# iesl/anncur

Hardware: AMD Instinct MI355X
Metric: queries/sec + Top-k-Recall@100 vs exact, CUR-256 on QxI score matrix (higher is better)
Workload: dtype bf16; 1 GPU; cfg2: Q=10000/GPU x I=100000 bf16 score matrix, 256 anchor items, 512 anchor queries, k=100, k_retvr=100; step = gather C_q + fused S_hat/top-k + exact top-k scan + overlap/recall; Q_per_gpu=10000, I=100000, anchors=256, anchor_queries=512, k=100, k_retvr=100

## Files before the change

### anncur_amd/csrc/common.hpp

```cpp
#pragma once
#include <hip/hip_runtime.h>
#include <stdint.h>
#include <stdarg.h>
#include <stdio.h>
#include "anncur_hip.h"

void anncur_set_error(const char *fmt, ...);
constexpr int LADDER_LEVELS = 8;
int anncur_internal_kth_value(const float *G, int64_t Q, int n, int64_t ldg, int k, float *out, int64_t out_stride, hipStream_t st, int coarse = 0,
							  float *ladder = nullptr, int k2 = 1, float *tau2 = nullptr);
int anncur_internal_approx_error_acc(const void *X, int x_dtype, int64_t ldx, const void *Et, int e_dtype, int64_t lde, const void *Aex, int a_dtype,
									 int64_t lda, int64_t Q, int64_t I, int64_t K, float *err_sq, float *norm_sq, void *stream);

int anncur_ensure_dyn_lds(const void *fn, int bytes);
int anncur_num_cu();
int anncur_event_pool(hipEvent_t **out, int n);
int anncur_internal_scan_rows_in_flight(int dtype);

#define ANNCUR_REQUIRE(cond, code, ...)                 \
	do {                                                \
		if (!(cond)) {                                  \
			anncur_set_error(__VA_ARGS__);              \
			return (code);                              \
		}                                               \
	} while (0)

#define ANNCUR_HIP_OK(expr)                                                              \
	do {                                                                                 \
		hipError_t e__ = (expr);                                                         \
		if (e__ != hipSuccess) {                                                         \
			anncur_set_error("%s failed: %s (%s:%d)", #expr, hipGetErrorString(e__), __FILE__, __LINE__); \
			return ANNCUR_E_HIP;                                                         \
		}                                                                                \
	} while (0)

#define ANNCUR_LAUNCH_OK()                                                               \
	do {                                                                                 \
		hipError_t e__ = hipGetLastError();                                              \
		if (e__ != hipSuccess) {                                                         \
			anncur_set_error("kernel launch failed: %s (%s:%d)", hipGetErrorString(e__), __FILE__, __LINE__); \
			return ANNCUR_E_HIP;                                                         \
		}                                                                                \
	} while (0)

static inline bool dtype_ok(int d) { return d == ANNCUR_F32 || d == ANNCUR_BF16; }
static inline size_t dtype_size(int d) { return d == ANNCUR_F32 ? 4 : 2; }
static inline int64_t ceil_div64(int64_t a, int64_t b) { return (a + b - 1) / b; }

#define WAVE 64

__device__ __forceinline__ float bf16_bits_to_f32(uint32_t b) { return __uint_as_float(b << 16); }

__device__ __forceinline__ uint16_t f32_to_bf16_bits(float f) {
	uint32_t u = __float_as_uint(f);
	if ((u & 0x7fffffffu) > 0x7f800000u) return (uint16_t)((u >> 16) | 0x0040u);
	return (uint16_t)((u + 0x7fffu + ((u >> 16) & 1u)) >> 16);
}

__device__ __forceinline__ uint32_t f32_sortable(float f) {
	const uint32_t u = __float_as_uint(f);
	return u ^ ((uint32_t)((int32_t)u >> 31) | 0x80000000u);
}
__device__ __forceinline__ float f32_unsortable(uint32_t s) {
	uint32_t u = (s & 0x80000000u) ? (s & 0x7fffffffu) : ~s;
	return __uint_as_float(u);
}
__device__ __forceinline__ uint64_t make_key(float v, uint32_t idx) {
	return ((uint64_t)f32_sortable(v) << 32) | (uint64_t)(0xffffffffu - idx);
}
__device__ __forceinline__ float key_val(uint64_t k) { return f32_unsortable((uint32_t)(k >> 32)); }
__device__ __forceinline__ uint32_t key_idx(uint64_t k) { return 0xffffffffu - (uint32_t)k; }

__device__ __forceinline__ int lane_id() { return threadIdx.x & (WAVE - 1); }

template <int CTRL, int ROW_MASK = 0xf, int BANK_MASK = 0xf>
__device__ __forceinline__ uint32_t dpp_mov(uint32_t identity, uint32_t x) {
	return (uint32_t)__builtin_amdgcn_update_dpp((int)identity, (int)x, CTRL, ROW_MASK, BANK_MASK, false);
}
struct DppAdd { static constexpr uint32_t ID = 0u; __device__ static uint32_t op(uint32_t a, uint32_t b) { return a + b; } };
struct DppMin { static constexpr uint32_t ID = 0xffffffffu; __device__ static uint32_t op(uint32_t a, uint32_t b) { return a < b ? a : b; } };
struct DppMax { static constexpr uint32_t ID = 0u; __device__ static uint32_t op(uint32_t a, uint32_t b) { return a > b ? a : b; } };
template <typename OP>
__device__ __forceinline__ uint32_t wave_scan_incl(uint32_t x) {
	uint32_t t = x;
	t = OP::op(t, dpp_mov<0x111>(OP::ID, x));
	t = OP::op(t, dpp_mov<0x112>(OP::ID, x));
	t = OP::op(t, dpp_mov<0x113>(OP::ID, x));
	t = OP::op(t, dpp_mov<0x114, 0xf, 0xe>(OP::ID, t));
	t = OP::op(t, dpp_mov<0x118, 0xf, 0xc>(OP::ID, t));
	t = OP::op(t, dpp_mov<0x142, 0xa, 0xf>(OP::ID, t));
	t = OP::op(t, dpp_mov<0x143, 0xc, 0xf>(OP::ID, t));
	return t;
}
template <typename OP>
__device__ __forceinline__ uint32_t wave_reduce(uint32_t x) {
	return (uint32_t)__builtin_amdgcn_readlane((int)wave_scan_incl<OP>(x), WAVE - 1);
}

__device__ __forceinline__ uint32_t lane_xor(uint32_t x, int stride) {
	if (stride == 1) return dpp_mov<0xB1>(x, x);
	if (stride == 2) return dpp_mov<0x4E>(x, x);
	if (stride == 4) return dpp_mov<0x1B>(x, dpp_mov<0x141>(x, x));
	if (stride == 8) return dpp_mov<0x141>(x, dpp_mov<0x140>(x, x));
	return (uint32_t)__shfl_xor((int)x, stride);
}

template <typename T>
__device__ __forceinline__ float load_as_f32(const T *p);
template <>
__device__ __forceinline__ float load_as_f32<float>(const float *p) { return *p; }
template <>
__device__ __forceinline__ float load_as_f32<uint16_t>(const uint16_t *p) { return bf16_bits_to_f32(*p); }
```

### anncur_amd/csrc/prepass16.hpp

```cpp
#pragma once

template <int KP>
struct Prepass16Cfg {
	static constexpr int NBUF = 3;
	static constexpr int KS32 = KP / 32, K = KP / 16, CPR = KP / 8;
	static constexpr int TILE_BYTES = TILE_I * KP * 2;
	static constexpr int PIECES = TILE_BYTES / 1024 / 4;
	static constexpr int LDS_BYTES = NBUF * TILE_BYTES;
	static constexpr int BQ = 256;
	static_assert(PIECES >= 1 && K >= 4, "a tile holds a 1 KB piece per wave and at least four fragments per lane");
	static_assert(2 * LDS_BYTES <= 160 * 1024, "two workgroups per CU");
};

template <int N>
__device__ __forceinline__ void vm_wait_all_but() {
#if defined(__HIP_DEVICE_COMPILE__)
	asm volatile("s_waitcnt vmcnt(%0)" ::"n"(N) : "memory");
#endif
}

template <int KP, int CUR>
__device__ __forceinline__ void prepass16_tile(const uint32_t (&aoff)[Prepass16Cfg<KP>::K], const bf16x8 (&xb)[4][Prepass16Cfg<KP>::KS32], f32x4 (&acc)[2][4]) {
	using C = Prepass16Cfg<KP>;
	constexpr int K = C::K, AR = 5, DIST = 3, OFF = CUR * C::TILE_BYTES;
	u32x4 ring[AR];
#pragma unroll
	for (int i = 0; i < DIST; ++i) lds_read_frag<OFF>(ring[i], aoff[i]);
#pragma unroll
	for (int ih = 0; ih < 2; ++ih)
#pragma unroll
		for (int t = 0; t < 4; ++t) acc[ih][t] = (f32x4){0.f, 0.f, 0.f, 0.f};
#pragma unroll
	for (int g = 0; g < K; ++g) {
		const int nxt = g + DIST;
		if (nxt < K) lds_read_frag<OFF>(ring[nxt % AR], aoff[nxt]);
#if defined(__HIP_DEVICE_COMPILE__)
		if (g >= 1) asm volatile("" ::"v"(ring[(g - 1) % AR]));
#endif
		const int after = K - 1 - g;
		lds_wait_frag(ring[g % AR], after < DIST ? after : DIST);
		const bf16x8 a = __builtin_bit_cast(bf16x8, ring[g % AR]);
		const int ks = g >> 1, ih = g & 1;
#pragma unroll
		for (int t = 0; t < 4; ++t) acc[ih][t] = __builtin_amdgcn_mfma_f32_16x16x32_bf16(a, xb[t][ks], acc[ih][t], 0, 0, 0);
	}
#if defined(__HIP_DEVICE_COMPILE__)
	asm volatile("s_nop 7\n\ts_nop 2" : "+v"(acc[0][0]), "+v"(acc[0][1]), "+v"(acc[0][2]), "+v"(acc[0][3]), "+v"(acc[1][0]), "+v"(acc[1][1]), "+v"(acc[1][2]), "+v"(acc[1][3]));
#endif
}

template <int KP>
__global__ __launch_bounds__(256, 2) void prepass16_kernel(const FusedParams p) {
	using C = Prepass16Cfg<KP>;
	constexpr int K = C::K, KS32 = C::KS32, CPR = C::CPR;
	extern __shared__ __attribute__((aligned(16))) unsigned char smem[];
	const int tid = threadIdx.x, lane = tid & 63, wave = tid >> 6;
	const int c16 = lane & 15, g4 = lane >> 4;
	zero_ws_header(p);
	const int wid = xcd_remap(blockIdx.x, p.n_wg);
	const int n_rb = (int)((p.Q + C::BQ - 1) / C::BQ);
	const int split = wid / n_rb, rb = wid - split * n_rb;
	const int wave_u = __builtin_amdgcn_readfirstlane(wave);
	const uint32_t lds_base = (uint32_t)__builtin_amdgcn_readfirstlane((int)lds_addr(smem));

	const int j_begin = split * p.st_per_split, j_end = min(j_begin + p.st_per_split, p.n_st);
	int f_tile, f_rem = 0, dq = 1, dr = 0;
	if (p.sample_leading) f_tile = j_begin;
	else {
		const int64_t x = (int64_t)j_begin * p.n_full_tiles;
		f_tile = (int)(x / p.n_st); f_rem = (int)(x % p.n_st);
		dq = p.n_full_tiles / p.n_st; dr = p.n_full_tiles % p.n_st;
	}
	int j_dma = j_begin;
	uint32_t dma_off[C::PIECES];
#pragma unroll
	for (int i = 0; i < C::PIECES; ++i) {
		const int pch = (wave_u * C::PIECES + i) * 64 + lane;
		const int row = pch / CPR, cs = pch % CPR;
		dma_off[i] = (uint32_t)(row * CPR + swz<CPR>(row, cs)) * 16u;
	}
	auto fetch = [&](int buf) {
		const unsigned char *src = reinterpret_cast<const unsigned char *>(p.Et) + (int64_t)f_tile * C::TILE_BYTES;
#if defined(__HIP_DEVICE_COMPILE__)
#pragma unroll
		for (int i = 0; i < C::PIECES; ++i) {
			const uint32_t m0v = lds_base + (uint32_t)(buf * C::TILE_BYTES) + (uint32_t)(wave_u * C::PIECES + i) * 1024u;
			asm volatile("s_mov_b32 m0, %0\n\ts_nop 0\n\tglobal_load_lds_dwordx4 %1, %2" ::"s"(m0v), "v"(dma_off[i]), "s"(src) : "memory", "m0");
		}
#endif
		f_tile += dq; f_rem += dr;
		if (f_rem >= p.n_st) { f_rem -= p.n_st; ++f_tile; }
		++j_dma;
	};
	if (j_dma < j_end) fetch(0);

	bf16x8 xb[4][KS32];
	const int64_t q_wave0 = (int64_t)rb * C::BQ + wave_u * 64;
#pragma unroll
	for (int t = 0; t < 4; ++t) {
		const int64_t q = q_wave0 + 16 * t + c16;
		const bool ok = q < p.Q;
		const u32x4 *src = reinterpret_cast<const u32x4 *>(p.X + (ok ? q : 0) * p.ldx) + g4;
#pragma unroll
		for (int s = 0; s < KS32; ++s) {
			const u32x4 zero = {0u, 0u, 0u, 0u};
			const u32x4 w = ok ? src[4 * s] : zero;
			xb[t][s] = __builtin_bit_cast(bf16x8, w);
		}
	}
	__builtin_amdgcn_s_waitcnt(0x0F70);
	if (j_dma < j_end) fetch(1);
	__builtin_amdgcn_s_barrier();

	const int64_t q_st = q_wave0 + 16 * (lane >> 5) + c16;
	const bool st_ok0 = q_st < p.Q, st_ok1 = q_st + 32 < p.Q;
	float *const gdst = p.gmax + (st_ok0 ? q_st : 0) * p.n_groups + (g4 & 1);
	const int64_t gdst_pair = (int64_t)32 * p.n_groups;
	uint32_t aoff[K];
#pragma unroll
	for (int s = 0; s < K; ++s) {
		const int row = 16 * (s & 1) + c16;
		aoff[s] = lds_addr(smem) + (uint32_t)(row * CPR + swz<CPR>(row, 4 * (s >> 1) + g4)) * 16u;
	}
	__builtin_amdgcn_s_waitcnt(0xC07F);

#define PRE16_STEP(CUR)                                                                                                         \
	do {                                                                                                                        \
		const bool ahead = j_dma < j_end;                                                                        \
		if (ahead) fetch(((CUR) + 2) % C::NBUF);    \
		f32x4 acc[2][4];                                                                                                        \
		prepass16_tile<KP, CUR>(aoff, xb, acc);                                                                                 \
		float m[4];                                                                                                             \
		_Pragma("unroll") for (int t = 0; t < 4; ++t) {                                                                         \
			const f32x4 a0 = acc[0][t], a1 = acc[1][t];                                                                         \
			m[t] = fmaxf(fmaxf(fmaxf(a0[0], a0[1]), fmaxf(a0[2], a0[3])), fmaxf(fmaxf(a1[0], a1[1]), fmaxf(a1[2], a1[3])));     \
		}                                                                                                                       \
		const auto s01 = __builtin_amdgcn_permlane32_swap(__float_as_uint(m[0]), __float_as_uint(m[1]), false, false);          \
		const auto s23 = __builtin_amdgcn_permlane32_swap(__float_as_uint(m[2]), __float_as_uint(m[3]), false, false);          \
		const float v01 = fmaxf(__uint_as_float(s01[0]), __uint_as_float(s01[1]));                                              \
		const float v23 = fmaxf(__uint_as_float(s23[0]), __uint_as_float(s23[1]));                                              \
		                         \
		if (ahead) vm_wait_all_but<C::PIECES>(); else vm_wait_all_but<0>();                                                     \
		if (st_ok0) gdst[2 * (int64_t)j] = v01;                                                                                 \
		if (st_ok1) gdst[gdst_pair + 2 * (int64_t)j] = v23;                                                                     \
		__builtin_amdgcn_s_barrier();                                                                                           \
		++j;                                                                                                                    \
	} while (0)
	ANNCUR_PAD_HERE();
	int j = j_begin;
	while (j < j_end) {
		PRE16_STEP(0);
		if (j >= j_end) break;
		PRE16_STEP(1);
		if (j >= j_end) break;
		PRE16_STEP(2);
	}
#undef PRE16_STEP
}
```

### anncur_amd/csrc/score_fused.hip

```cpp
#include <stdlib.h>
#include <math.h>
#include <type_traits>
#ifdef ANNCUR_PLACEMENT_PAD
#define ANNCUR_PAD_HERE() asm volatile(".rept %0\n\ts_nop 0\n\t.endr" ::"n"(ANNCUR_PLACEMENT_PAD) : "memory")
#else
#define ANNCUR_PAD_HERE() do { } while (0)
#endif
#include "select.hpp"
#include "wave_select.hpp"
#include "select_stream.hpp"

using namespace anncur;

namespace {

typedef __attribute__((ext_vector_type(8))) __bf16 bf16x8;
typedef __attribute__((ext_vector_type(16))) float f32x16;
typedef __attribute__((ext_vector_type(4))) unsigned int u32x4;

constexpr int TILE_I = 32;
constexpr int CHUNK_TILES = 4;

template <int KP, int QTV = ((KP <= 256) ? 2 : 1)>
struct FusedCfg {
	static constexpr int KSTEPS = KP / 16;
	static constexpr int QT = QTV;
	static constexpr int BQ = 4 * 32 * QT;
	static constexpr int CPR = KP / 8;
	static constexpr int TILE_BYTES = TILE_I * KP * 2;
	static constexpr int PASSES = TILE_BYTES / (256 * 16);
	static constexpr int QDEPTH = 8;
	static constexpr int QUEUE_BYTES = QT * QDEPTH * 256 * 8;
	static constexpr int QUEUE_OFF = (2 * TILE_BYTES + 16383) / 16384 * 16384;
	static constexpr int TICKET_OFF = QUEUE_OFF + QUEUE_BYTES;
	static constexpr int LDS_BYTES = TICKET_OFF + (KP >= 512 ? 0 : 16);
	static constexpr int NAOFF = KSTEPS < 8 ? KSTEPS : 8;
};

template <int CPR>
__device__ __forceinline__ int swz(int row, int c) {
	if (CPR >= 16) return c ^ (row & 15);
	return c ^ ((row >> 1) & 7);
}

struct FusedParams {
	const uint16_t *X; int64_t ldx;
	const uint16_t *Et;
	int64_t Q, I;
	int n_tiles, n_full_tiles;
	int S, tiles_per_split;
	int tile_begin, tile_end;
	int tile_step;
	int carry;
	int n_st, S0, st_per_split;
	int sample_leading;
	float *gmax; int n_groups;
	const float *tau; int tau_stride;
	uint2 *cand; uint32_t *seg_cnt; int capg;
	int nseg;
	int rb_major;
	int flush_tiles;
	int debug_nostore;
	int debug_stamp;
	float tau_bias;
	int n_wg;
	int chunk_tiles, n_chunks;
	uint32_t *chunk_ctr;
	uint8_t *chunk_owner;
	int sliced, chunks_per_slice;
	int prio_mode;
	int ladder_on; uint32_t ladder_k, ladder_mask;
	const float *ladder; uint32_t *ladder_cnt; float *tau_final;
	uint32_t *nfb;
	int ring_stagger, ring_spin_sleep;
	uint32_t zero_bytes;
};

__device__ __forceinline__ int xcd_remap(int b, int n) {
	const int q = n >> 3, r = n & 7, x = b & 7, l = b >> 3;
	return (x < r ? x * (q + 1) : r * (q + 1) + (x - r) * q) + l;
}

__device__ __forceinline__ void zero_ws_header(const FusedParams &p) {
	typedef __attribute__((ext_vector_type(4))) unsigned int zvec;
	zvec *const dst = reinterpret_cast<zvec *>(p.nfb);
	const uint32_t n = p.zero_bytes >> 4;
	for (uint32_t i = blockIdx.x * blockDim.x + threadIdx.x; i < n; i += gridDim.x * blockDim.x) dst[i] = (zvec){0u, 0u, 0u, 0u};
}


template <int KP>
__device__ __forceinline__ void tile_dma(const uint16_t *__restrict__ Et, int tile, unsigned char *buf, int wave, int lane) {
	constexpr int CPR = FusedCfg<KP>::CPR;
	constexpr int PER_WAVE = FusedCfg<KP>::TILE_BYTES / 1024 / 4;
	const unsigned char *src = reinterpret_cast<const unsigned char *>(Et + (int64_t)tile * TILE_I * KP);
#pragma unroll
	for (int i = 0; i < PER_WAVE; ++i) {
		const int piece = wave * PER_WAVE + i;
		const int pch = piece * 64 + lane;
		const int row = pch / CPR, cs = pch % CPR;
		const int c = swz<CPR>(row, cs);
		__builtin_amdgcn_global_load_lds((const __attribute__((address_space(1))) void *)(src + (row * CPR + c) * 16),
										 (__attribute__((address_space(3))) void *)(buf + piece * 1024), 16, 0, 0);
	}
}

template <int KP>
__device__ __forceinline__ void tile_dma_offsets(uint32_t (&voff)[FusedCfg<KP>::TILE_BYTES / 4096], int wave_u, int lane) {
	constexpr int CPR = FusedCfg<KP>::CPR, PER_WAVE = FusedCfg<KP>::TILE_BYTES / 4096;
#pragma unroll
	for (int i = 0; i < PER_WAVE; ++i) {
		const int pch = (wave_u * PER_WAVE + i) * 64 + lane;
		const int row = pch / CPR, cs = pch % CPR;
		voff[i] = (uint32_t)(row * CPR + swz<CPR>(row, cs)) * 16u;
	}
}
template <int KP>
__device__ __forceinline__ void tile_dma_s(const uint16_t *__restrict__ Et, int tile, uint32_t lds_buf, int wave_u,
											const uint32_t (&voff)[FusedCfg<KP>::TILE_BYTES / 4096]) {
	constexpr int PER_WAVE = FusedCfg<KP>::TILE_BYTES / 4096;
	const unsigned char *src = reinterpret_cast<const unsigned char *>(Et) + (int64_t)tile * FusedCfg<KP>::TILE_BYTES;
#if defined(__HIP_DEVICE_COMPILE__)
#pragma unroll
	for (int i = 0; i < PER_WAVE; ++i) {
		const uint32_t m0v = lds_buf + (uint32_t)(wave_u * PER_WAVE + i) * 1024u;
		asm volatile("s_mov_b32 m0, %0\n\ts_nop 0\n\tglobal_load_lds_dwordx4 %1, %2" ::"s"(m0v), "v"(voff[i]), "s"(src) : "memory", "m0");
	}
#endif
}

__device__ __forceinline__ uint32_t lds_addr(const void *p) {
	return (uint32_t)(size_t)(__attribute__((address_space(3))) const char *)p;
}
__device__ __forceinline__ void lds_write_u64(uint32_t addr, uint32_t lo, uint32_t hi) {
#if defined(__HIP_DEVICE_COMPILE__)
	const unsigned long long d = ((unsigned long long)hi << 32) | lo;
	asm volatile("ds_write_b64 %0, %1" ::"v"(addr), "v"(d) : "memory");
#endif
}
__device__ __forceinline__ uint2 lds_load_u64(uint32_t addr) {
	unsigned long long d = 0;
#if defined(__HIP_DEVICE_COMPILE__)
	asm volatile("ds_read_b64 %0, %1\n\ts_waitcnt lgkmcnt(0)" : "=&v"(d) : "v"(addr) : "memory");
#endif
	return make_uint2((uint32_t)d, (uint32_t)(d >> 32));
}

__device__ __forceinline__ void lds_write_u32(uint32_t addr, uint32_t v) {
#if defined(__HIP_DEVICE_COMPILE__)
	asm volatile("ds_write_b32 %0, %1" ::"v"(addr), "v"(v) : "memory");
#endif
}
__device__ __forceinline__ uint32_t lds_load_u32_uniform(uint32_t addr) {
	uint32_t d = 0;
#if defined(__HIP_DEVICE_COMPILE__)
	asm volatile("ds_read_b32 %0, %1\n\ts_waitcnt lgkmcnt(0)" : "=&v"(d) : "v"(addr) : "memory");
#endif
	return (uint32_t)__builtin_amdgcn_readfirstlane((int)d);
}
__device__ __forceinline__ void ticket_draw(uint32_t &ticket, uint32_t *ctr) {
#if defined(__HIP_DEVICE_COMPILE__)
	const uint32_t one = 1u;
	asm volatile("global_atomic_add %0, %1, %2, off sc0" : "=v"(ticket) : "v"(ctr), "v"(one) : "memory");
#endif
}
__device__ __forceinline__ void ticket_wait(uint32_t &ticket) {
#if defined(__HIP_DEVICE_COMPILE__)
	asm volatile("s_waitcnt vmcnt(0)" : "+v"(ticket)::"memory");
#endif
}
__device__ __forceinline__ void lds_write_2x32(uint32_t addr, uint32_t lo, uint32_t hi) {
#if defined(__HIP_DEVICE_COMPILE__)
	asm volatile("ds_write2_b32 %0, %1, %2 offset1:1" ::"v"(addr), "v"(lo), "v"(hi) : "memory");
#endif
}

template <int D, bool FILTER_PREDICATED = false, bool INLINE_HIT = false>
__device__ __forceinline__ void filter_one(float v, int e, float tau, uint32_t item0, uint32_t lq, uint32_t &qcnt) {
	static_assert((D & (D - 1)) == 0, "queue depth must be a power of two");
	if (FILTER_PREDICATED) {
		if (v >= tau) {
			lds_write_2x32((qcnt & (uint32_t)((D - 1) << 11)) | lq, __float_as_uint(v), item0 + (uint32_t)((e & 3) + 8 * (e >> 2)));
			qcnt += 2048u;
		}
	} else if (INLINE_HIT) {
		if (__builtin_expect(__ballot(v >= tau) != 0ull, 1)) {
			if (v >= tau) {
				lds_write_2x32((qcnt & (uint32_t)((D - 1) << 11)) | lq, __float_as_uint(v), item0 + (uint32_t)((e & 3) + 8 * (e >> 2)));
				qcnt += 2048u;
			}
		}
	} else if (__builtin_expect(__ballot(v >= tau) != 0ull, 0)) {
		if (v >= tau) {
			lds_write_2x32((qcnt & (uint32_t)((D - 1) << 11)) | lq, __float_as_uint(v), item0 + (uint32_t)((e & 3) + 8 * (e >> 2)));
			qcnt += 2048u;
		}
	}
}

template <int D>
__device__ __forceinline__ void filter_queue(const f32x16 &acc, float tau, uint32_t item0, uint32_t lq, uint32_t &qcnt) {
#pragma unroll
	for (int e = 0; e < 16; ++e) filter_one<D>(acc[e], e, tau, item0, lq, qcnt);
}

constexpr uint32_t RING_RAW = 0x80000000u;
template <int D>
__device__ __forceinline__ void mark_wrapped_raw(const f32x16 &acc, uint32_t lq, uint32_t &qcnt) {
	static_assert(D == 8, "the raw tile (16 floats) fills the ring exactly");
	const bool wrapped = (qcnt >> 11) > (uint32_t)D && qcnt < RING_RAW;
	if (__builtin_expect(__ballot(wrapped) != 0ull, 0)) {
		if (wrapped) {
#pragma unroll
			for (int i = 0; i < D; ++i) lds_write_2x32(lq + (uint32_t)i * 2048u, __float_as_uint(acc[2 * i]), __float_as_uint(acc[2 * i + 1]));
			qcnt = RING_RAW;
		}
	}
}

template <int D, bool BATCH = true>
__device__ __forceinline__ void flush_queue(uint32_t lq, uint32_t &qcnt, uint2 *__restrict__ seg, uint32_t &ncand, uint32_t capg,
											 uint32_t n_items, float tau, uint32_t raw_item0) {
	if (__builtin_expect(__ballot(qcnt >= RING_RAW) != 0ull, 0)) {
		if (qcnt >= RING_RAW) {
			for (int i = 0; i < D; ++i) {
				const uint2 w = lds_load_u64(lq + (uint32_t)i * 2048u);
#pragma unroll
				for (int half = 0; half < 2; ++half) {
// ... 629 lines not shown
		adma(j_begin, 0);
	}
	__builtin_amdgcn_s_waitcnt(0x0F70);
	__syncthreads();
	uint32_t aoff[Cfg::NAOFF];
#pragma unroll
	for (int s = 0; s < Cfg::NAOFF; ++s) aoff[s] = lds_addr(smem) + (uint32_t)(r * CPR + swz<CPR>(r, 2 * s + h)) * 16u;
	__builtin_amdgcn_s_waitcnt(0xC07F);
	static_assert(PA <= 15, "vmcnt immediate");
#define ERRL_STEP(ECUR, ACUR, J)                                                                                                \
	do {                                                                                                                        \
		if ((J) + 1 < j_end) tile_dma_s<KP>(p.Et, (J) + 1, lds_base + ((ECUR) ^ 1) * Cfg::TILE_BYTES, wave_u, dma_off);         \
		const bool ahead = (J) + NAB - 1 < j_end;                                                                \
		if (ahead) adma((J) + NAB - 1, ((ACUR) + NAB - 1) % NAB);                                                               \
		f32x16 acc[QT];                                                                                                         \
		error_mfma_tile<KP, ECUR>(aoff, xb, acc);                                                                               \
		ExactQuad<uint16_t> ex[QT][4];                     \
		_Pragma("unroll") for (int t = 0; t < QT; ++t)                                                                          \
			_Pragma("unroll") for (int g = 0; g < 4; ++g)                                                                       \
				asm volatile("ds_read_b64 %0, %1 offset:%2" : "=v"(ex[t][g].w) : "v"(aread[t] + (((uint32_t)g << 4) ^ asw[t])), "n"((ACUR) * ATILE)); \
		asm volatile("s_waitcnt lgkmcnt(0)" ::: "memory");                                                                      \
		_Pragma("unroll") for (int t = 0; t < QT; ++t)                                                                          \
			_Pragma("unroll") for (int g = 0; g < 4; ++g) asm volatile("" : "+v"(ex[t][g].w));                                  \
		_Pragma("unroll") for (int t = 0; t < QT; ++t)                                                                          \
			_Pragma("unroll") for (int e = 0; e < 16; ++e) {                                                                    \
				const float x = ex[t][e >> 2].get(e & 3);                                                                       \
				const float d = acc[t][e] - x;                                                                                  \
				se[t] = fmaf(d, d, se[t]);                                                                                      \
				sn[t] = fmaf(x, x, sn[t]);                                                                                      \
			}                                                                                                                   \
		        \
		if (NAB == 3 && ahead) asm volatile("s_waitcnt vmcnt(%0)" ::"n"(PA) : "memory");                                        \
		else __builtin_amdgcn_s_waitcnt(0x0F70);                                                                                \
		asm volatile("" ::: "memory");                                                                                          \
		__builtin_amdgcn_s_barrier();                                                                                           \
		asm volatile("" ::: "memory");                                                                                          \
	} while (0)
	for (int j = j_begin; j < j_end; j += 2) {
		ERRL_STEP(0, 0, j);
		if (j + 1 < j_end) ERRL_STEP(1, 1, j + 1);
	}
#undef ERRL_STEP
#pragma unroll
	for (int t = 0; t < QT; ++t)
		if (qv[t] < p.Q) {
			atomicAdd(&err_sq[qv[t]], se[t]);
			atomicAdd(&norm_sq[qv[t]], sn[t]);
		}
}

template <int KP, typename TA>
__global__ __launch_bounds__(256, 2) void error_kernel(const FusedParams p, const TA *__restrict__ Aex, int64_t lda,
														float *__restrict__ err_sq, float *__restrict__ norm_sq) {
	using Cfg = FusedCfg<KP>;
	constexpr int KSTEPS = Cfg::KSTEPS, QT = Cfg::QT, CPR = Cfg::CPR;
	extern __shared__ __attribute__((aligned(16))) unsigned char smem[];
	const int tid = threadIdx.x, lane = tid & 63, wave = tid >> 6;
	const int r = lane & 31, h = lane >> 5;
	const int wid = xcd_remap(blockIdx.x, p.n_wg);
	const int n_rb = (int)((p.Q + Cfg::BQ - 1) / Cfg::BQ);
	const int split = wid / n_rb, rb = wid - split * n_rb;

	bf16x8 xb[QT][KSTEPS];
	int64_t qv[QT];
	const TA *rowp[QT];
#pragma unroll
	for (int t = 0; t < QT; ++t) {
		qv[t] = (int64_t)rb * Cfg::BQ + wave * 32 * QT + 32 * t + r;
		const bool ok = qv[t] < p.Q;
		rowp[t] = Aex + (ok ? qv[t] : 0) * lda + 4 * h;
		const u32x4 *src = reinterpret_cast<const u32x4 *>(p.X + (ok ? qv[t] : 0) * p.ldx) + h;
#pragma unroll
		for (int s = 0; s < KSTEPS; ++s) {
			const u32x4 zero = {0u, 0u, 0u, 0u};
			const u32x4 w = ok ? src[2 * s] : zero;
			xb[t][s] = __builtin_bit_cast(bf16x8, w);
		}
	}
	__builtin_amdgcn_s_waitcnt(0x0F70);

	const int j_begin = split * p.tiles_per_split, j_end = min(j_begin + p.tiles_per_split, p.n_tiles);
	float se[QT], sn[QT];
	ExactQuad<TA> ex[QT][4];
#pragma unroll
	for (int t = 0; t < QT; ++t) { se[t] = 0.f; sn[t] = 0.f; }
	if (j_begin < j_end) {
		tile_dma<KP>(p.Et, j_begin, smem, wave, lane);
#pragma unroll
		for (int t = 0; t < QT; ++t)
#pragma unroll
			for (int g = 0; g < 4; ++g) ex[t][g].load(rowp[t] + (int64_t)j_begin * TILE_I + 8 * g);
	}
	__builtin_amdgcn_s_waitcnt(0x0F70);
	__syncthreads();
	uint32_t aoff[Cfg::NAOFF];
#pragma unroll
	for (int s = 0; s < Cfg::NAOFF; ++s) aoff[s] = lds_addr(smem) + (uint32_t)(r * CPR + swz<CPR>(r, 2 * s + h)) * 16u;
	__builtin_amdgcn_s_waitcnt(0xC07F);
#define ERR_STEP(CUR, J)                                                                                                        \
	do {                                                                                                                        \
		const bool more = (J) + 1 < j_end;                                                                                      \
		if (more) tile_dma<KP>(p.Et, (J) + 1, smem + ((CUR) ^ 1) * Cfg::TILE_BYTES, wave, lane);                                \
		f32x16 acc[QT];                                                                                                         \
		error_mfma_tile<KP, CUR>(aoff, xb, acc);                                                                                \
		 \
		                            \
		_Pragma("unroll") for (int t = 0; t < QT; ++t)                                                                          \
			_Pragma("unroll") for (int g = 0; g < 4; ++g) asm volatile("" : "+v"(ex[t][g].w));                                  \
		_Pragma("unroll") for (int t = 0; t < QT; ++t)                                                                          \
			_Pragma("unroll") for (int e = 0; e < 16; ++e) {                                                                    \
				const float x = ex[t][e >> 2].get(e & 3);                                                                       \
				const float d = acc[t][e] - x;                                                                                  \
				se[t] = fmaf(d, d, se[t]);                                                                                      \
				sn[t] = fmaf(x, x, sn[t]);                                                                                      \
			}                                                                                                                   \
		  \
		                      \
		if (more) {                                                                                                             \
			      \
			       \
			if (QT == 2) asm volatile("" : "+v"(se[0]), "+v"(sn[0]), "+v"(se[QT - 1]), "+v"(sn[QT - 1])::"memory");             \
			else asm volatile("" : "+v"(se[0]), "+v"(sn[0])::"memory");                                                         \
			_Pragma("unroll") for (int t = 0; t < QT; ++t)                                                                      \
				_Pragma("unroll") for (int g = 0; g < 4; ++g) ex[t][g].load(rowp[t] + (int64_t)((J) + 1) * TILE_I + 8 * g);     \
			__builtin_amdgcn_s_waitcnt(QT == 2 ? 0x0F78 : 0x0F74);                                     \
		}                                                                                                                       \
		 \
		 \
		asm volatile("" ::: "memory");                                                                                          \
		__builtin_amdgcn_s_barrier();                                                                                           \
		asm volatile("" ::: "memory");                                                                                          \
	} while (0)
	for (int j = j_begin; j < j_end; j += 2) {
		ERR_STEP(0, j);
		if (j + 1 < j_end) ERR_STEP(1, j + 1);
	}
#undef ERR_STEP
#pragma unroll
	for (int t = 0; t < QT; ++t)
		if (qv[t] < p.Q) {
			atomicAdd(&err_sq[qv[t]], se[t]);
			atomicAdd(&norm_sq[qv[t]], sn[t]);
		}
}

#include "score_evalf.hpp"

struct SweepStages {
	int n, begin[3], end[3], tps[3], stride;
	int chunk, bq, n_chunks[3];
	const uint8_t *owner[3];
};

template <int KMAX>
__global__ __launch_bounds__(SEL_THREADS) void select_candidates_kernel(
	const uint2 *__restrict__ cand, const uint32_t *__restrict__ seg_cnt, int nseg, int S, SweepStages stg, int capg,
	const uint16_t *__restrict__ X, int64_t ldx, const uint16_t *__restrict__ Et, int64_t I, int KP, uint32_t k,
	float *__restrict__ out_val, int32_t *__restrict__ out_idx, uint32_t *__restrict__ n_fallback,
	const int32_t *__restrict__ hard_list, const uint32_t *__restrict__ hard_cnt, const float *__restrict__ tau_in, int tau_stride,
	const int32_t *__restrict__ remap) {
	extern __shared__ __attribute__((aligned(16))) unsigned char smem[];
	const SelState s = sel_carve<KMAX>(smem);
	float *xq = reinterpret_cast<float *>(smem + SelCfg<KMAX>::LDS_BYTES);
	uint32_t *bad = reinterpret_cast<uint32_t *>(xq + KP);
	const int tid = threadIdx.x, lane = tid & 63, wave = tid >> 6;
	auto score_of = [&](int64_t i) {
		float v = 0.f;
		const uint4 *er = reinterpret_cast<const uint4 *>(Et + i * KP);
		for (int c = 0; c < KP / 8; ++c) {
			const uint4 w = er[c];
			const uint32_t ww[4] = {w.x, w.y, w.z, w.w};
#pragma unroll
			for (int d = 0; d < 4; ++d) {
				v = fmaf(__uint_as_float(ww[d] << 16), xq[8 * c + 2 * d], v);
				v = fmaf(__uint_as_float(ww[d] & 0xffff0000u), xq[8 * c + 2 * d + 1], v);
			}
		}
		return v;
	};
	const uint32_t n_work = hard_list ? *hard_cnt : gridDim.x;
	for (uint32_t wi = blockIdx.x; wi < n_work; wi += gridDim.x) {
	__syncthreads();
	sel_init(s);
	if (tid < 8) bad[tid] = 0u;
	__syncthreads();
	const int64_t q = hard_list ? (int64_t)hard_list[wi] : (int64_t)wi;
	const uint32_t *cnts = seg_cnt + q * nseg;
	for (int sg = tid; sg < nseg; sg += SEL_THREADS) {
		const uint32_t c = cnts[sg];
		if (c > (uint32_t)capg) { const int sp = sg % S; atomicOr(&bad[sp >> 5], 1u << (sp & 31)); }
	}
	__syncthreads();
	const bool repair = (bad[0] | bad[1] | bad[2] | bad[3] | bad[4] | bad[5] | bad[6] | bad[7]) != 0u;
	for (int sg = tid; sg < nseg; sg += SEL_THREADS) {
		const int sp = sg % S;
		const uint32_t cc = ((bad[sp >> 5] >> (sp & 31)) & 1u) ? 0u : cnts[sg];
		atomicAdd(&s.scal[9], cc);
		atomicMax(&s.scal[10], cc);
	}
	__syncthreads();
	const uint32_t total = s.scal[9], maxc = s.scal[10];
	float tau = tau_in ? tau_in[q * tau_stride] : -INFINITY;
	uint64_t tau_key = 0;
	bool full = !repair && total < k;
	if (!full) {
		for (int sb = 0; sb < nseg; sb += 4) {
			const int sg = sb + wave;
			const int sp = sg % S;
			const bool use = sg < nseg && !((bad[sp >> 5] >> (sp & 31)) & 1u);
			const uint32_t c = use ? cnts[sg] : 0u;
			const uint2 *sp_ptr = cand + (q * nseg + (sg < nseg ? sg : 0)) * (int64_t)capg;
			for (uint32_t e0 = 0; e0 < maxc; e0 += WAVE) {
				const uint32_t e = e0 + lane;
				const bool in = e < c;
				const uint2 ce = in ? sp_ptr[e] : make_uint2(0, 0);
				sel_offer(s, in, __uint_as_float(ce.x), ce.y, tau, tau_key);
				sel_maybe_compact<KMAX>(s, k, tau, tau_key);
			}
		}
	}
	if (repair || full) {
		if (tid == 0) atomicAdd(n_fallback, 1u);
		for (int c = tid; c < KP; c += SEL_THREADS) xq[c] = bf16_bits_to_f32(X[q * ldx + c]);
		__syncthreads();
	}
	if (repair) {
		for (int sp = 0; sp < S; ++sp) {
			if (!((bad[sp >> 5] >> (sp & 31)) & 1u)) continue;
			for (int g = 0; g < stg.n; ++g) {
				if (stg.chunk > 0) {
					const uint8_t *own = stg.owner[g] + (q / stg.bq) * (int64_t)stg.n_chunks[g];
					int it = 0;
					for (int c = 0; c < stg.n_chunks[g]; ++c) {
						if (own[c] != (uint8_t)sp) continue;
						const int64_t i_beg = (int64_t)(stg.begin[g] + c * stg.chunk) * TILE_I;
						const int64_t i_end = (int64_t)min(stg.begin[g] + (c + 1) * stg.chunk, stg.end[g]) * TILE_I;
						for (int64_t i0 = i_beg; i0 < i_end; i0 += SEL_THREADS, ++it) {
							const int64_t i = i0 + tid;
							const bool in = i < i_end && i < I;
							const float v = in ? score_of(i) : 0.f;
							sel_offer(s, in, v, (uint32_t)i, tau, tau_key);
							if ((it & 15) == 15) sel_maybe_compact<KMAX>(s, k, tau, tau_key);
						}
					}
					sel_maybe_compact<KMAX>(s, k, tau, tau_key);
					continue;
				}
				if (stg.stride > 1) {
					int it = 0;
					for (int tb = stg.begin[g] + sp; tb < stg.end[g]; tb += 8 * stg.stride, ++it) {
						const int tile = tb + (tid >> 5) * stg.stride;
						const int64_t i = (int64_t)tile * TILE_I + (tid & 31);
						const bool in = tile < stg.end[g] && i < I;
						const float v = in ? score_of(i) : 0.f;
						sel_offer(s, in, v, (uint32_t)i, tau, tau_key);
						if ((it & 15) == 15) sel_maybe_compact<KMAX>(s, k, tau, tau_key);
					}
					sel_maybe_compact<KMAX>(s, k, tau, tau_key);
					continue;
				}
				const int t0 = stg.begin[g] + sp * stg.tps[g];
				const int t1 = min(t0 + stg.tps[g], stg.end[g]);
				int it = 0;
				for (int64_t i0 = (int64_t)t0 * TILE_I; i0 < (int64_t)t1 * TILE_I; i0 += SEL_THREADS, ++it) {
					const int64_t i = i0 + tid;
					const bool in = i < (int64_t)t1 * TILE_I && i < I;
					const float v = in ? score_of(i) : 0.f;
					sel_offer(s, in, v, (uint32_t)i, tau, tau_key);
					if ((it & 15) == 15) sel_maybe_compact<KMAX>(s, k, tau, tau_key);
				}
				sel_maybe_compact<KMAX>(s, k, tau, tau_key);
			}
		}
		__syncthreads();
		full = s.scal[0] < k && tau_key == 0;
	}
	if (full) {
		__syncthreads();
		if (tid == 0) s.scal[0] = 0;
		__syncthreads();
		tau = -INFINITY; tau_key = 0;
		int it = 0;
		for (int64_t i0 = 0; i0 < I; i0 += SEL_THREADS, ++it) {
			const int64_t i = i0 + tid;
			const bool in = i < I;
			const float v = in ? score_of(i) : 0.f;
			sel_offer(s, in, v, (uint32_t)i, tau, tau_key);
			if ((it & 15) == 15) sel_maybe_compact<KMAX>(s, k, tau, tau_key);
		}
	}
	sel_finish<KMAX>(s, k, out_val + q * (int64_t)k, out_idx + q * (int64_t)k, remap);
	}
}

template <int KMAX>
__global__ __launch_bounds__(SEL_THREADS) void tau_block_kernel(const uint2 *__restrict__ cand, const uint32_t *__restrict__ seg_cnt, int nseg,
																 int capg, uint32_t k, float *__restrict__ tau_out, int tau_stride, int prefilter) {
	extern __shared__ __attribute__((aligned(16))) unsigned char smem[];
	const SelState s = sel_carve<KMAX>(smem);
	const int tid = threadIdx.x, lane = tid & 63, wave = tid >> 6;
	const int64_t q = blockIdx.x;
	sel_init(s);
	const uint32_t *cnts = seg_cnt + q * nseg;
	for (int sg = tid; sg < nseg; sg += SEL_THREADS) {
		const uint32_t c = cnts[sg];
		if (c > (uint32_t)capg) atomicOr(&s.scal[8], 1u);
		atomicAdd(&s.scal[9], c > (uint32_t)capg ? 0u : c);
		atomicMax(&s.scal[10], c > (uint32_t)capg ? 0u : c);
	}
	__syncthreads();
	if (s.scal[8] != 0u || s.scal[9] <= k) return;
	const uint32_t maxc = s.scal[10];
	float tau = prefilter ? tau_out[q * tau_stride] : -INFINITY;
	uint64_t tau_key = 0;
	for (int sb = 0; sb < nseg; sb += 4) {
		const int sg = sb + wave;
		const uint32_t c = sg < nseg ? cnts[sg] : 0u;
		const uint2 *sp = cand + (q * nseg + (sg < nseg ? sg : 0)) * (int64_t)capg;
		for (uint32_t e0 = 0; e0 < maxc; e0 += WAVE) {
			const uint32_t e = e0 + lane;
			const bool in = e < c;
			const uint2 ce = in ? sp[e] : make_uint2(0, 0);
			sel_offer(s, in, __uint_as_float(ce.x), ce.y, tau, tau_key);
			sel_maybe_compact<KMAX>(s, k, tau, tau_key);
		}
	}
	__syncthreads();
	if (s.scal[0] > k) {
		tau_key = sel_compact<KMAX>(s, k);
		tau = key_val(tau_key);
	}
	if (tid == 0 && tau_key != 0 && s.scal[0] >= k) tau_out[q * tau_stride] = fmaxf(tau_out[q * tau_stride], tau);
}

constexpr int WQ_CAP = 1024;
constexpr int WQ_K2 = 1024;
template <int KW> struct WqCfg { static constexpr int CAP = KW <= 128 ? WQ_CAP : 2048, TRIGGER = CAP - WAVE, E = KW / 64; };

template <bool TAU_ONLY, int KW = 128>
__global__ __launch_bounds__(256) void select_wave_kernel(const uint2 *__restrict__ cand, const uint32_t *__restrict__ seg_cnt, int nseg,
														   int capg, int64_t Q, uint32_t k, float *__restrict__ out_val,
														   int32_t *__restrict__ out_idx, uint32_t *__restrict__ hard_cnt,
														   int32_t *__restrict__ hard_list, float *__restrict__ tau, int tau_stride, int prefilter,
														   const int32_t *__restrict__ remap) {
	extern __shared__ __attribute__((aligned(16))) unsigned char smem[];
	const int lane = lane_id(), wave = threadIdx.x >> 6;
	const int64_t q = (int64_t)blockIdx.x * 4 + wave;
	if (q >= Q) return;
	const uint32_t c = (lane < nseg) ? seg_cnt[q * nseg + lane] : 0u;
	const uint32_t inc = wave_scan_incl<DppAdd>(c);
	const uint32_t total = (uint32_t)__builtin_amdgcn_readlane((int)inc, WAVE - 1), pre = inc - c;
	if (__ballot(c > (uint32_t)capg) != 0ull || total < k) {
		if (!TAU_ONLY && lane == 0) hard_list[atomicAdd(hard_cnt, 1u)] = (int32_t)q;
		return;
	}
	constexpr int CAP = WqCfg<KW>::CAP, TRIGGER = WqCfg<KW>::TRIGGER;
	WaveSel w = wsel_init<CAP>(smem + wave * WaveSelLayout<CAP>::BYTES);
	if (tau && prefilter) w.tau = tau[q * tau_stride];
	const uint2 *qc = cand + q * nseg * (int64_t)capg;
	constexpr int LOAD_U = 8;
	for (uint32_t j0 = 0; j0 < total; j0 += LOAD_U * WAVE) {
		int sg[LOAD_U];
#pragma unroll
		for (int u = 0; u < LOAD_U; ++u) sg[u] = 0;
#pragma unroll
		for (int step = 32; step >= 1; step >>= 1) {
			if (step < nseg) {
				uint32_t pv[LOAD_U];
#pragma unroll
				for (int u = 0; u < LOAD_U; ++u) pv[u] = __shfl(pre, (sg[u] + step) & 63);
#pragma unroll
				for (int u = 0; u < LOAD_U; ++u)
					if (sg[u] + step < nseg && pv[u] <= j0 + (uint32_t)(u * WAVE + lane)) sg[u] += step;
			}
		}
		uint32_t ps[LOAD_U];
#pragma unroll
		for (int u = 0; u < LOAD_U; ++u) ps[u] = __shfl(pre, sg[u]);
		uint2 e[LOAD_U];
#pragma unroll
		for (int u = 0; u < LOAD_U; ++u) {
			const uint32_t j = j0 + (uint32_t)(u * WAVE + lane);
			e[u] = qc[j < total ? (int64_t)sg[u] * capg + (j - ps[u]) : 0];
		}
#pragma unroll
		for (int u = 0; u < LOAD_U; ++u) {
			if (j0 + (uint32_t)(u * WAVE) < total) {
				wsel_offer(w, j0 + (uint32_t)(u * WAVE + lane) < total, __uint_as_float(e[u].x), e[u].y);
				if (w.cnt > (uint32_t)TRIGGER) wsel_compact<4, false, true>(w, k);
			}
		}
	}
	if (TAU_ONLY) {
		if (w.cnt > k) wsel_compact<4, false, true>(w, k);
		if (lane == 0 && w.cnt >= k) tau[q * tau_stride] = fmaxf(tau[q * tau_stride], w.tau);
		return;
	}
	wsel_finish<0, 4, WqCfg<KW>::E, true>(w, k, out_val + q * (int64_t)k, out_idx + q * (int64_t)k, remap);
}

}
namespace {
#include "score_wide.hpp"
}
namespace {

struct FusedPlan {
	bool ok;
	int QT, BQ, n_rb, n_tiles, n_full, S, tiles_per_split, group, n_st, S0, st_per_split, n_groups, capg, kmax, flush_tiles;
	int n_stages, stage_end[3], stage_tps[3], stage_flush[3], stage_pred[3];
	int leading;
	int lg;
	bool body16;
	bool bodyef;
	bool bodyq16;
	int chunk;
	bool ladder;
	int ladder_k2;
	size_t off_lcnt, off_lvl, off_tau2;
	size_t off_gmax, off_tval, off_tidx, off_segcnt, off_cand, off_tau, off_hard, off_ctr, off_owner, total;
};

int num_cu() { return anncur_num_cu(); }

size_t align256(size_t x) { return (x + 255) & ~(size_t)255; }
int next_pow2(int x) { int p = 1; while (p < x) p <<= 1; return p; }

void plan_stages(FusedPlan &P, int64_t Q, int k, double exp_hits, bool staged, double fmin, int unit_items) {
	double frac[3] = {1.0, 1.0, 1.0};
	P.n_stages = 1;
	if (staged) {
		const double H0 = exp_hits, c_hit = 2.4e-11 * (double)Q;
		const double c_stage = k <= WSEL_K ? 25e-6 + 3e-9 * (double)Q : (k <= WQ_K2 ? 25e-6 + 1.2e-8 * (double)Q : 25e-6 + 1.4e-11 * (double)Q * 0.3 * H0);
		auto later = [&](double f) { const double h = 1.2 * k / f; return h < H0 ? h : H0; };
		double best = H0 * c_hit;
		static const double grid[] = {0.02, 0.03, 0.04, 0.06, 0.08, 0.10, 0.12, 0.15, 0.18, 0.22, 0.26, 0.30, 0.35, 0.40, 0.50};
		const int ng = (int)(sizeof(grid) / sizeof(grid[0]));
		for (int i = 0; i < ng; ++i) {
			const double f1 = grid[i];
			if (f1 < fmin) continue;
			const double c2 = (f1 * H0 + (1 - f1) * later(f1)) * c_hit + c_stage;
			if (c2 < best) { best = c2; P.n_stages = 2; frac[0] = f1; frac[1] = 1.0; }
			for (int j = i + 1; j < ng; ++j) {
				const double f2 = grid[j];
				if (f2 - f1 < fmin) continue;
				const double c3 = (f1 * H0 + (f2 - f1) * later(f1) + (1 - f2) * later(f2)) * c_hit + 2 * c_stage;
				if (c3 < best) { best = c3; P.n_stages = 3; frac[0] = f1; frac[1] = f2; }
			}
		}
	}
	if (P.n_stages == 2) {
		const double shrink = P.body16 ? 0.63 : (k <= WSEL_K ? 1.0 : 0.6);
		const double f1 = frac[0] * shrink;
		frac[0] = f1 > fmin ? f1 : (fmin < frac[0] ? fmin : frac[0]);
	}
	double rate = exp_hits / ((double)P.n_tiles * 2.0);
	int prev = 0;
	for (int i = 0; i < P.n_stages; ++i) {
		int end = (int)(frac[i] * P.n_tiles + 0.5);
		if (i == P.n_stages - 1 || end > P.n_tiles) end = P.n_tiles;
		if (end <= prev) end = prev + 1 < P.n_tiles ? prev + 1 : P.n_tiles;
		P.stage_end[i] = end;
		P.stage_tps[i] = (end - prev + P.S - 1) / P.S;
		int ft = (int)(0.35 / (rate > 1e-9 ? rate : 1e-9));
		P.stage_flush[i] = ft < 1 ? 1 : (ft > 8 ? 8 : ft);
		P.stage_pred[i] = (1.0 - exp(-4.0 * rate)) > 0.25 ? 1 : 0;
		rate = (double)k / ((double)end * unit_items) * 16.0 * 1.2;
		prev = end;
	}
}

FusedPlan plan_fused(int64_t Q, int64_t I, int KP, int k, bool leading = false, bool mfma16 = false, bool qt1 = false, bool mfma32 = false, bool evalf = false,
					 bool no_ladder = false) {
	FusedPlan P{};
	P.ok = false;
	P.leading = leading ? 1 : 0;
	if (!(KP == 64 || KP == 128 || KP == 256 || KP == 512)) return P;
	if (k < 1 || k > ANNCUR_MAX_TOPK || Q < 1 || I < 1 || I >= (int64_t)0x7fffffff - 64 || k > I) return P;
	if (evalf && !(KP <= 256 && I < (int64_t)(1 << 26))) return P;
	if (evalf) { qt1 = false; mfma16 = false; mfma32 = false; leading = false; P.leading = 0; }
	P.bodyef = evalf;
	P.QT = (KP <= 256 && !(qt1 && KP >= 128)) ? 2 : 1;
	P.BQ = 128 * P.QT;
	P.n_rb = (int)ceil_div64(Q, P.BQ);
	P.n_tiles = (int)ceil_div64(I, TILE_I);
	P.n_full = (int)(I / TILE_I);
	int target = (4 * k > 512) ? 4 * k : 512;
	int n_st16 = (target + 1) / 2;
	if ((int64_t)n_st16 * 8 <= P.n_full) { P.group = 16; P.n_st = n_st16; }
	else { P.group = 4; P.n_st = (target + 7) / 8; }
	if ((int64_t)P.n_st * 4 > P.n_full) return P;
	P.n_groups = P.n_st * (P.group == 16 ? 2 : 8);
	if (P.n_groups < k) return P;
	int slots = ((P.QT == 1 && KP <= 256) ? 3 : 2) * num_cu();
	P.bodyq16 = KP == 512 && !mfma32 && I < (int64_t)(1 << 26);
	const bool ticketed = (P.QT == 2 || P.bodyq16) && !evalf;
	P.chunk = ticketed ? CHUNK_TILES : 0;
	const bool can16 = KP <= 256 && P.QT == 2 && I < (int64_t)(1 << 26);
	constexpr int BODY16_MAX_K = 384, BODY16_MAX_K_LADDER = 1024;
	int S = P.chunk > 0 ? (slots + P.n_rb - 1) / P.n_rb : slots / P.n_rb;
	if (P.chunk > 0 && k <= WQ_K2 && S > WAVE / 2) S = WAVE / 2;
	if (S < 1) S = 1;
	if (S > 255) S = P.chunk > 0 ? 255 : (S > 256 ? 256 : S);
	if (S > P.n_tiles) S = P.n_tiles;
	P.tiles_per_split = (P.n_tiles + S - 1) / S;
	P.S = (P.n_tiles + P.tiles_per_split - 1) / P.tiles_per_split;
	constexpr int64_t LADDER_WAVE_SLACK = (int64_t)(LADDER_PERIOD + 2) * TILE_I + Fused16Cfg<256>::DRAIN_AT;
	const bool ladder_fits = I < 65536 || (int64_t)k + (int64_t)P.S * LADDER_WAVE_SLACK <= 32768;
	const bool ladder_possible = !no_ladder && ticketed && P.n_groups <= 4096 && ladder_fits;
	P.body16 = can16 && !mfma32 && !evalf && (mfma16 || k <= (ladder_possible ? BODY16_MAX_K_LADDER : BODY16_MAX_K));
	int S0 = slots / P.n_rb;
	if (S0 < 1) S0 = 1;
	if (S0 > P.n_st) S0 = P.n_st;
	P.st_per_split = (P.n_st + S0 - 1) / S0;
	P.S0 = (P.n_st + P.st_per_split - 1) / P.st_per_split;
	P.lg = (P.body16 || P.bodyq16 || P.bodyef) ? 1 : 2;
	const double exp_hits_cap = 1.3 * k * ((double)P.n_tiles / P.n_st);
	const double exp_hits = (leading ? 0.65 : 1.0) * exp_hits_cap;
	const double per_seg = exp_hits_cap / ((double)P.lg * P.S);
	int capg = next_pow2((int)(4.0 * per_seg) + 32);
	if (capg < 64) capg = 64;
	if (capg > 16384) capg = 16384;
	P.capg = capg;
	const double per_lane_tile = exp_hits / ((double)P.n_tiles * 2.0);
	int ft = (int)(0.35 / (per_lane_tile > 1e-9 ? per_lane_tile : 1e-9));
	P.flush_tiles = ft < 1 ? 1 : (ft > 8 ? 8 : ft);
	P.ladder = P.body16 && ladder_possible;
	{
		double r = (double)k * ((double)P.n_st * TILE_I / (double)I) * (leading ? 2.0 : 1.25);
		int k2 = (int)(r + 0.5);
		if (k2 > k / 2) k2 = k / 2;
		if (k2 < 3) k2 = 3;
		if (k2 > k) k2 = k;
		P.ladder_k2 = k2;
	}
	plan_stages(P, Q, k, exp_hits, !P.ladder && (k <= WQ_K2 ? P.lg * P.S <= WAVE : true) && P.n_tiles >= 24 * P.S, 4.0 * P.S / P.n_tiles, TILE_I);
	P.kmax = k <= 128 ? 128 : (k <= 512 ? 512 : 2048);
	size_t off = 256;
	P.off_ctr = off;    off = align256(off + (size_t)P.n_rb * 3 * 4 * N_SLICES);
	P.off_lcnt = off;   off = align256(off + (P.ladder ? (size_t)P.n_rb * P.BQ * 16 : 0));
	P.off_gmax = off;   off = align256(off + (size_t)Q * P.n_groups * 4);
	P.off_tval = off;   off = align256(off + (size_t)Q * k * 4);
	P.off_tidx = off;   off = align256(off + (size_t)Q * k * 4);
	P.off_segcnt = off; off = align256(off + (size_t)Q * P.lg * P.S * 4);
	P.off_tau = off;    off = align256(off + (size_t)Q * 4);
	P.off_hard = off;   off = align256(off + (size_t)Q * 4);
	P.off_owner = off;  off = align256(off + (size_t)3 * P.n_rb * (size_t)(P.n_tiles / (P.chunk > 0 ? P.chunk : P.n_tiles) + 2));
	P.off_lvl = off;    off = align256(off + (P.ladder ? (size_t)P.n_rb * P.BQ * 4 * LADDER_LEVELS : 0));
	P.off_tau2 = off;   off = align256(off + (P.ladder ? (size_t)Q * 4 : 0));
	P.off_cand = off;   off = align256(off + (size_t)Q * P.lg * P.S * (size_t)P.capg * 8);
	P.total = off;
	P.ok = true;
	return P;
}

#define EV(i) do { if (ev) ANNCUR_HIP_OK(hipEventRecord(ev[i], st)); } while (0)

constexpr bool STREAM_SELECT_SMALL = false;

int launch_tau_refine(const uint2 *cand, const uint32_t *seg_cnt, int nseg, int capg, int64_t Q, int k, int kmax, float *tau, int tau_stride,
					  int prefilter, hipStream_t st) {
	int rc;
	if (k <= WQ_K2 && nseg <= WAVE) {
#define LAUNCH_WTAU(KW)                                                                                                           \
		do {                                                                                                                      \
			constexpr int lds = 4 * WaveSelLayout<WqCfg<KW>::CAP>::BYTES;                                                         \
			if ((rc = anncur_ensure_dyn_lds((const void *)select_wave_kernel<true, KW>, lds)) != ANNCUR_OK) return rc;            \
			hipLaunchKernelGGL((select_wave_kernel<true, KW>), dim3((unsigned)ceil_div64(Q, 4)), dim3(256), lds, st, cand, seg_cnt, nseg, capg, Q, \
							   (uint32_t)k, (float *)nullptr, (int32_t *)nullptr, (uint32_t *)nullptr, (int32_t *)nullptr, tau, tau_stride, prefilter, (const int32_t *)nullptr); \
		} while (0)
		if (k <= WSEL_K) LAUNCH_WTAU(128);
		else {
			constexpr int lds = 4 * StreamSelLayout::BYTES;
			hipLaunchKernelGGL((select_stream_kernel<true, 2>), dim3((unsigned)ceil_div64(Q, 4)), dim3(256), lds, st, cand, seg_cnt, nseg, capg, Q,
							   (uint32_t)k, (float *)nullptr, (int32_t *)nullptr, (uint32_t *)nullptr, (int32_t *)nullptr, tau, tau_stride, prefilter, (const int32_t *)nullptr);
		}
#undef LAUNCH_WTAU
	} else {
#define LAUNCH_TAU(KM)                                                                                                        \
		do {                                                                                                                  \
			if ((rc = anncur_ensure_dyn_lds((const void *)tau_block_kernel<KM>, (int)SelCfg<KM>::LDS_BYTES)) != ANNCUR_OK) return rc; \
			hipLaunchKernelGGL((tau_block_kernel<KM>), dim3((unsigned)Q), dim3(SEL_THREADS), SelCfg<KM>::LDS_BYTES, st, cand, seg_cnt, \
							   nseg, capg, (uint32_t)k, tau, tau_stride, prefilter);                                           \
		} while (0)
		if (kmax == 128) LAUNCH_TAU(128); else if (kmax == 512) LAUNCH_TAU(512); else LAUNCH_TAU(2048);
#undef LAUNCH_TAU
	}
	ANNCUR_LAUNCH_OK();
	return ANNCUR_OK;
}

int launch_select(const FusedPlan &P, int nseg, const SweepStages &stages, const uint2 *cand, const uint32_t *seg_cnt, const uint16_t *X, int64_t ldx,
				  const uint16_t *Et, int64_t Q, int64_t I, int KP, int k, float *out_val, int32_t *out_idx, unsigned char *ws, const float *tau,
				  int tau_stride, hipStream_t st, const int32_t *remap = nullptr) {
	int rc;
#define LAUNCH_SELECT(KM)                                                                                              \
	do {                                                                                                               \
		const size_t lds = SelCfg<KM>::LDS_BYTES + (size_t)KP * 4 + 32;                                                \
		if ((rc = anncur_ensure_dyn_lds((const void *)select_candidates_kernel<KM>, (int)lds)) != ANNCUR_OK) return rc; \
		hipLaunchKernelGGL((select_candidates_kernel<KM>), dim3(sel_grid), dim3(SEL_THREADS), lds, st, cand, seg_cnt, nseg, \
						   P.S, stages, P.capg, X, ldx, Et, I, KP, (uint32_t)k, out_val, out_idx, (uint32_t *)ws, hard_list, hard_cnt,      \
						   (P.n_stages > 1 || P.ladder) ? tau : (const float *)nullptr, tau_stride, remap);                              \
	} while (0)
	const int32_t *hard_list = nullptr;
	const uint32_t *hard_cnt = nullptr;
	unsigned sel_grid = (unsigned)Q;
	if (k <= WQ_K2 && nseg <= WAVE) {
		int32_t *hl = (int32_t *)(ws + P.off_hard);
		uint32_t *hc = (uint32_t *)(ws + 4);
#define LAUNCH_WSEL(KW)                                                                                                           \
		do {                                                                                                                      \
			constexpr int lds = 4 * WaveSelLayout<WqCfg<KW>::CAP>::BYTES;                                                         \
			if ((rc = anncur_ensure_dyn_lds((const void *)select_wave_kernel<false, KW>, lds)) != ANNCUR_OK) return rc;           \
			hipLaunchKernelGGL((select_wave_kernel<false, KW>), dim3((unsigned)ceil_div64(Q, 4)), dim3(256), lds, st, cand, seg_cnt, nseg, P.capg, Q, \
							   (uint32_t)k, out_val, out_idx, hc, hl, const_cast<float *>(tau), tau_stride, (P.n_stages > 1 || P.ladder) ? 1 : 0, remap); \
		} while (0)
#define LAUNCH_SSEL(EE)                                                                                                           \
		do {                                                                                                                      \
			constexpr int lds = 4 * StreamSelLayout::BYTES;                                                                       \
			hipLaunchKernelGGL((select_stream_kernel<false, EE>), dim3((unsigned)ceil_div64(Q, 4)), dim3(256), lds, st, cand, seg_cnt, nseg, P.capg, Q, \
							   (uint32_t)k, out_val, out_idx, hc, hl, const_cast<float *>(tau), tau_stride, (P.n_stages > 1 || P.ladder) ? 1 : 0, remap); \
		} while (0)
		if (k <= WSEL_K) { if (STREAM_SELECT_SMALL) LAUNCH_SSEL(2); else LAUNCH_WSEL(128); }
		else if (k <= 256) LAUNCH_SSEL(4);
		else if (k <= 512) LAUNCH_SSEL(8);
		else LAUNCH_SSEL(16);
#undef LAUNCH_SSEL
#undef LAUNCH_WSEL
		ANNCUR_LAUNCH_OK();
		hard_list = hl; hard_cnt = hc;
		sel_grid = (unsigned)(Q < 1024 ? Q : 1024);
	}
	if (P.kmax == 128) LAUNCH_SELECT(128); else if (P.kmax == 512) LAUNCH_SELECT(512); else LAUNCH_SELECT(2048);
#undef LAUNCH_SELECT
	ANNCUR_LAUNCH_OK();
	return ANNCUR_OK;
}

int launch_threshold(const FusedPlan &P, const float *gmax, int64_t Q, int k, unsigned char *ws, const float *&tau, int &tau_stride, hipStream_t st) {
	if (P.n_groups <= 4096) {
		float *t = (float *)(ws + P.off_tau);
		const int rc = P.ladder ? anncur_internal_kth_value(gmax, Q, P.n_groups, P.n_groups, k, t, 1, st, 1, (float *)(ws + P.off_lvl), P.ladder_k2, (float *)(ws + P.off_tau2))
								: anncur_internal_kth_value(gmax, Q, P.n_groups, P.n_groups, k, t, 1, st, 1);
		tau = t; tau_stride = 1;
		return rc;
	}
	float *tval = (float *)(ws + P.off_tval);
	tau = tval + (k - 1); tau_stride = k;
	return anncur_rowwise_topk(gmax, ANNCUR_F32, Q, P.n_groups, P.n_groups, k, tval, (int32_t *)(ws + P.off_tidx), st);
}


struct CoScan {
	hipStream_t aux;
	hipEvent_t *ev;
	const void *A; int a_dtype; int64_t lda, Q, I; int32_t k;
	float *val; int32_t *idx;
	int slots, next;
	int64_t row_end[8];
};

int co_plan(CoScan &co, int slots) {
	if (slots > 8) slots = 8;
	if (slots < 1) slots = 1;
	const int64_t round = anncur_internal_scan_rows_in_flight(co.a_dtype);
	const int64_t rounds = co.Q / round;
	int64_t per = rounds / slots;
	if (per < 1) {
		per = 1;
		slots = rounds >= 1 ? (int)rounds : 1;
	}
	int64_t r = 0;
	for (int i = 0; i < slots; ++i) { r = (i == slots - 1) ? co.Q : r + per * round; co.row_end[i] = r < co.Q ? r : co.Q; }
	co.slots = slots;
	co.next = 0;
	return anncur_event_pool(&co.ev, 2 * slots);
}
int co_fork(CoScan *co, hipStream_t st) {
	if (!co || co->next >= co->slots) return ANNCUR_OK;
	const int i = co->next++;
	const int64_t r0 = i ? co->row_end[i - 1] : 0, r1 = co->row_end[i];
	if (r1 <= r0) return ANNCUR_OK;
	ANNCUR_HIP_OK(hipEventRecord(co->ev[2 * i], st));
	ANNCUR_HIP_OK(hipStreamWaitEvent(co->aux, co->ev[2 * i], 0));
	const char *a = (const char *)co->A + (size_t)r0 * (size_t)co->lda * dtype_size(co->a_dtype);
	const int rc = anncur_rowwise_topk(a, co->a_dtype, r1 - r0, co->I, co->lda, co->k, co->val + r0 * co->k, co->idx + r0 * co->k, co->aux);
	if (rc != ANNCUR_OK) return rc;
	ANNCUR_HIP_OK(hipEventRecord(co->ev[2 * i + 1], co->aux));
	return ANNCUR_OK;
}
int co_join(CoScan *co, hipStream_t st) {
	if (!co || co->next < 1) return ANNCUR_OK;
	const int i = co->next - 1;
	if (co->row_end[i] > (i ? co->row_end[i - 1] : 0)) ANNCUR_HIP_OK(hipStreamWaitEvent(st, co->ev[2 * i + 1], 0));
	return ANNCUR_OK;
}
int co_finish(CoScan *co, hipStream_t st) {
	if (!co) return ANNCUR_OK;
	int rc;
	while (co->next < co->slots) {
		if ((rc = co_fork(co, st)) != ANNCUR_OK) return rc;
		if ((rc = co_join(co, st)) != ANNCUR_OK) return rc;
	}
	return co_join(co, st);
}

void co_abort(CoScan *co, hipStream_t st) {
	if (!co) return;
	for (int i = 0; i < co->next; ++i)
		if (co->row_end[i] > (i ? co->row_end[i - 1] : 0)) (void)hipStreamWaitEvent(st, co->ev[2 * i + 1], 0);
}

bool exact_tile_offsets_fit(int64_t lda, int bq) { return lda >= 0 && (uint64_t)(bq - 1) * (uint64_t)lda * 2u + 64u < ((uint64_t)1 << 32); }

struct EvalArgs { const uint16_t *A; int64_t lda; float *err_sq, *norm_sq; const uint16_t *Et_hint; };

template <int KP, int QTV = FusedCfg<KP>::QT>
int launch_fused(const FusedPlan &P, const void *X, int64_t ldx, const void *Et, int64_t Q, int64_t I, int k, float *out_val,
				 int32_t *out_idx, unsigned char *ws, hipStream_t st, hipEvent_t *ev, CoScan *co = nullptr, const int32_t *item_ids = nullptr,
				 const EvalArgs *ea = nullptr) {
	using Cfg = FusedCfg<KP, QTV>;
	FusedParams p{};
	p.X = (const uint16_t *)X; p.ldx = ldx; p.Et = (const uint16_t *)Et; p.Q = Q; p.I = I;
	p.n_tiles = P.n_tiles; p.n_full_tiles = P.n_full; p.S = P.S; p.tiles_per_split = P.tiles_per_split;
	p.tile_begin = 0; p.tile_end = P.n_tiles; p.carry = 0; p.tile_step = 1;
	p.n_st = P.n_st; p.S0 = P.S0; p.st_per_split = P.st_per_split; p.sample_leading = P.leading;
	p.gmax = (float *)(ws + P.off_gmax); p.n_groups = P.n_groups;
	p.cand = (uint2 *)(ws + P.off_cand); p.seg_cnt = (uint32_t *)(ws + P.off_segcnt); p.capg = P.capg; p.flush_tiles = P.flush_tiles;
	p.tau_bias = 0.f;
	p.chunk_tiles = 0; p.n_chunks = 0; p.chunk_ctr = nullptr; p.chunk_owner = nullptr;
	p.nfb = (uint32_t *)ws;
	p.ring_stagger = 0; p.ring_spin_sleep = 1;
	p.nseg = P.lg * P.S;
	p.prio_mode = 0;
	p.ladder_on = P.ladder ? 1 : 0; p.ladder_k = (uint32_t)k; p.ladder_mask = (uint32_t)(LADDER_PERIOD - 1);
	p.ladder = (const float *)(ws + P.off_lvl); p.ladder_cnt = (uint32_t *)(ws + P.off_lcnt); p.tau_final = (float *)(ws + P.off_tau2);

	const int chunk = (P.chunk > 0 && (Cfg::QT == 2 || P.bodyq16)) ? P.chunk : 0;
	const int owner_stride = P.n_rb * (P.n_tiles / (chunk > 0 ? chunk : P.n_tiles) + 2);
	int rc;
	EV(0);
	p.n_wg = P.n_rb * P.S0;
	{
		FusedParams pp = p;
		pp.zero_bytes = (uint32_t)((chunk > 0 || P.ladder) ? P.off_gmax : 256);
		if (ea && ea->Et_hint) { pp.Et = ea->Et_hint; pp.sample_leading = 1; }
		bool pre16 = false;
		if constexpr (KP <= 256 && QTV == 2) {
			if (P.body16 && P.group == 16) {
				if ((rc = anncur_ensure_dyn_lds((const void *)prepass16_kernel<KP>, Prepass16Cfg<KP>::LDS_BYTES)) != ANNCUR_OK) return rc;
				hipLaunchKernelGGL((prepass16_kernel<KP>), dim3(p.n_wg), dim3(256), Prepass16Cfg<KP>::LDS_BYTES, st, pp);
				pre16 = true;
			}
		}
		if (!pre16 && P.group == 16)
			hipLaunchKernelGGL((score_kernel<KP, 0, 16, false, false, QTV>), dim3(p.n_wg), dim3(256), 2 * Cfg::TILE_BYTES, st, pp);
		else if (!pre16)
			hipLaunchKernelGGL((score_kernel<KP, 0, 4, false, false, QTV>), dim3(p.n_wg), dim3(256), 2 * Cfg::TILE_BYTES, st, pp);
	}
	ANNCUR_LAUNCH_OK();
	EV(1);
	if ((rc = co_fork(co, st)) != ANNCUR_OK) return rc;
	rc = launch_threshold(P, p.gmax, Q, k, ws, p.tau, p.tau_stride, st);
	if (rc != ANNCUR_OK) return rc;
	if ((rc = co_join(co, st)) != ANNCUR_OK) return rc;
	EV(2);
	const int tile_step = (!P.body16 && !P.bodyq16 && !P.bodyef && P.S > 1 && chunk == 0) ? P.S : 1;
	p.n_wg = P.n_rb * P.S;
	if ((rc = anncur_ensure_dyn_lds((const void *)score_kernel<KP, 1, 16, false, false, QTV>, Cfg::LDS_BYTES)) != ANNCUR_OK) return rc;
	for (int stg = 0, prev = 0; stg < P.n_stages; prev = P.stage_end[stg], ++stg) {
		EV(5 + 2 * stg);
		p.tile_begin = prev; p.tile_end = P.stage_end[stg]; p.tiles_per_split = P.stage_tps[stg];
		p.flush_tiles = P.stage_flush[stg]; p.carry = stg > 0;
		p.tile_step = tile_step;
		if (chunk > 0) {
			p.rb_major = 0;
			p.chunk_tiles = chunk; p.n_chunks = (p.tile_end - p.tile_begin + chunk - 1) / chunk;
			p.sliced = P.bodyq16 ? 1 : 0;
			p.chunks_per_slice = (p.n_chunks + N_SLICES - 1) / N_SLICES;
			p.chunk_ctr = (uint32_t *)(ws + P.off_ctr) + (size_t)stg * P.n_rb * N_SLICES;
			p.chunk_owner = (uint8_t *)(ws + P.off_owner) + (size_t)stg * owner_stride;
		}
		bool launched = false;
		if constexpr (KP <= 256 && QTV == 2) {
			if (!launched && P.bodyef) {
				if (!ea) { anncur_set_error("launch_fused: evalf plan without the exact matrix"); return ANNCUR_E_INVALID; }
				if ((rc = anncur_ensure_dyn_lds((const void *)evalf_kernel<KP>, EvalFCfg<KP>::LDS_BYTES)) != ANNCUR_OK) return rc;
				hipLaunchKernelGGL((evalf_kernel<KP>), dim3(p.n_wg), dim3(256), EvalFCfg<KP>::LDS_BYTES, st, p, ea->A, ea->lda, ea->err_sq, ea->norm_sq);
				launched = true;
			}
		}
		if constexpr (KP == 512) {
			if (!launched && P.bodyq16) {
				if ((rc = anncur_ensure_dyn_lds((const void *)scoreq16_kernel<KP>, FusedQ16Cfg<KP>::LDS_BYTES)) != ANNCUR_OK) return rc;
				hipLaunchKernelGGL((scoreq16_kernel<KP>), dim3(p.n_wg), dim3(256), FusedQ16Cfg<KP>::LDS_BYTES, st, p);
				launched = true;
			}
		}
		if constexpr (KP <= 256 && QTV == 2) {
			if (!launched && P.body16) {
				if ((rc = anncur_ensure_dyn_lds((const void *)score16_kernel<KP>, Fused16Cfg<KP>::LDS_BYTES)) != ANNCUR_OK) return rc;
				hipLaunchKernelGGL((score16_kernel<KP>), dim3(p.n_wg), dim3(256), Fused16Cfg<KP>::LDS_BYTES, st, p);
				launched = true;
			}
		}
		if constexpr (Cfg::QT == 2) {
			if (!launched && P.stage_pred[stg]) {
				if ((rc = anncur_ensure_dyn_lds((const void *)score_kernel<KP, 1, 16, true, false, QTV>, Cfg::LDS_BYTES)) != ANNCUR_OK) return rc;
				hipLaunchKernelGGL((score_kernel<KP, 1, 16, true, false, QTV>), dim3(p.n_wg), dim3(256), Cfg::LDS_BYTES, st, p);
				launched = true;
			}
		}
		if (!launched) hipLaunchKernelGGL((score_kernel<KP, 1, 16, false, false, QTV>), dim3(p.n_wg), dim3(256), Cfg::LDS_BYTES, st, p);
		ANNCUR_LAUNCH_OK();
		EV(6 + 2 * stg);
		if (stg + 1 < P.n_stages) {
			if ((rc = co_fork(co, st)) != ANNCUR_OK) return rc;
			if ((rc = launch_tau_refine(p.cand, p.seg_cnt, P.lg * P.S, P.capg, Q, k, P.kmax, const_cast<float *>(p.tau), p.tau_stride, stg > 0 ? 1 : 0, st)) != ANNCUR_OK)
				return rc;
			if ((rc = co_join(co, st)) != ANNCUR_OK) return rc;
		}
	}
	EV(3);
	if ((rc = co_fork(co, st)) != ANNCUR_OK) return rc;
	SweepStages stages{};
	stages.n = P.n_stages;
	stages.stride = tile_step;
	stages.chunk = chunk; stages.bq = P.BQ;
	for (int g = 0, prev = 0; g < P.n_stages; prev = P.stage_end[g], ++g) {
		stages.begin[g] = prev; stages.end[g] = P.stage_end[g]; stages.tps[g] = P.stage_tps[g];
		stages.n_chunks[g] = chunk > 0 ? (P.stage_end[g] - prev + chunk - 1) / chunk : 0;
		stages.owner[g] = (const uint8_t *)(ws + P.off_owner) + (size_t)g * owner_stride;
	}
	if ((rc = launch_select(P, P.lg * P.S, stages, p.cand, p.seg_cnt, p.X, ldx, p.Et, Q, I, KP, k, out_val, out_idx, ws, P.ladder ? p.tau_final : p.tau,
							P.ladder ? 1 : p.tau_stride, st, item_ids)) != ANNCUR_OK) return rc;
	EV(4);
	return ANNCUR_OK;
}

constexpr int WIDE_KP_MAX = 4096;
bool wide_kp(int KP) { return KP > 512 && KP <= WIDE_KP_MAX && (KP % 128) == 0; }

FusedPlan plan_wide(int64_t Q, int64_t I, int KP, int k, bool leading = false) {
	FusedPlan P{};
	P.ok = false;
	P.leading = leading ? 1 : 0;
	if (!wide_kp(KP)) return P;
	if (k < 1 || k > ANNCUR_MAX_TOPK || Q < 1 || I < 1 || I >= (int64_t)0x7fffffff - 512 || k > I) return P;
	P.QT = 2;
	P.BQ = WBN;
	P.n_rb = (int)ceil_div64(Q, WBN);
	P.n_tiles = (int)ceil_div64(I, WBM);
	P.n_full = (int)(I / WBM);
	const int target = (4 * k > 512) ? 4 * k : 512;
	const int n16 = (target + 15) / 16;
	if ((int64_t)n16 * 8 <= P.n_full) { P.group = 16; P.n_st = n16; }
	else { P.group = 4; P.n_st = (target + 63) / 64; }
	if ((int64_t)P.n_st * 2 > P.n_full) return P;
	P.n_groups = P.n_st * (P.group == 16 ? 16 : 64);
	if (P.n_groups < k) return P;
	const int slots = num_cu();
	int S = slots / P.n_rb;
	if (S < 1) S = 1;
	if (S > 64) S = 64;
	if (k <= WQ_K2 && S > 16) S = 16;
	if (S > P.n_tiles) S = P.n_tiles;
	P.tiles_per_split = (P.n_tiles + S - 1) / S;
	P.S = (P.n_tiles + P.tiles_per_split - 1) / P.tiles_per_split;
	int S0 = slots / P.n_rb;
	if (S0 < 1) S0 = 1;
	if (S0 > P.n_st) S0 = P.n_st;
	P.st_per_split = (P.n_st + S0 - 1) / S0;
	P.S0 = (P.n_st + P.st_per_split - 1) / P.st_per_split;
	const double exp_hits_cap = 1.3 * k * ((double)P.n_tiles / P.n_st);
	const double exp_hits = (leading ? 0.65 : 1.0) * exp_hits_cap;
	const double per_seg = exp_hits_cap / (4.0 * P.S);
	int capg = next_pow2((int)(4.0 * per_seg) + 32);
	if (capg < 64) capg = 64;
	if (capg > 16384) capg = 16384;
	while (capg > 64 && (int64_t)capg * 4 * P.S >= (1 << 21)) capg >>= 1;
	P.capg = capg;
	P.flush_tiles = 1;
	plan_stages(P, Q, k, exp_hits, (k <= WQ_K2 ? 4 * P.S <= WAVE : true) && P.n_tiles >= 4 * P.S, 1.0 * P.S / P.n_tiles, WBM);
	P.kmax = k <= 128 ? 128 : (k <= 512 ? 512 : 2048);
	size_t off = 256;
	P.off_gmax = off;   off = align256(off + (size_t)Q * P.n_groups * 4);
	P.off_tval = off;   off = align256(off + (size_t)Q * k * 4);
	P.off_tidx = off;   off = align256(off + (size_t)Q * k * 4);
	P.off_segcnt = off; off = align256(off + (size_t)Q * 4 * P.S * 4);
	P.off_tau = off;    off = align256(off + (size_t)Q * 4);
	P.off_hard = off;   off = align256(off + (size_t)Q * 4);
	P.off_cand = off;   off = align256(off + (size_t)Q * 4 * P.S * (size_t)P.capg * 8);
	P.total = off;
	P.ok = true;
	return P;
}

int launch_wide(const FusedPlan &P, const void *X, int64_t ldx, const void *Et, int64_t Q, int64_t I, int KP, int k, float *out_val,
				int32_t *out_idx, unsigned char *ws, hipStream_t st, hipEvent_t *ev, CoScan *co = nullptr, const int32_t *item_ids = nullptr) {
	WideParams p{};
	p.X = (const uint16_t *)X; p.ldx = ldx; p.Et = (const uint16_t *)Et; p.et_rows = ceil_div64(I, TILE_I) * TILE_I; p.Q = Q; p.I = I; p.Kp = KP;
	p.n_rb = P.n_rb; p.S = P.S;
	p.n_st = P.n_st; p.S0 = P.S0; p.st_per_split = P.st_per_split; p.sample_leading = P.leading; p.n_bt_full = P.n_full;
	p.gmax = (float *)(ws + P.off_gmax); p.n_groups = P.n_groups;
	p.cand = (uint2 *)(ws + P.off_cand); p.seg_cnt = (uint32_t *)(ws + P.off_segcnt); p.capg = P.capg;
	p.tau_bias = 0.f;
	int rc;
	ANNCUR_HIP_OK(hipMemsetAsync(ws, 0, 256, st));
	EV(0);
	p.n_wg = P.n_rb * P.S0;
	if (P.group == 16) {
		if ((rc = anncur_ensure_dyn_lds((const void *)wide_kernel<0, 16>, W_LDS_TOTAL)) != ANNCUR_OK) return rc;
		hipLaunchKernelGGL((wide_kernel<0, 16>), dim3(p.n_wg), dim3(512), W_LDS_TOTAL, st, p);
	} else {
		if ((rc = anncur_ensure_dyn_lds((const void *)wide_kernel<0, 4>, W_LDS_TOTAL)) != ANNCUR_OK) return rc;
		hipLaunchKernelGGL((wide_kernel<0, 4>), dim3(p.n_wg), dim3(512), W_LDS_TOTAL, st, p);
	}
	ANNCUR_LAUNCH_OK();
	EV(1);
	if ((rc = co_fork(co, st)) != ANNCUR_OK) return rc;
	if ((rc = launch_threshold(P, p.gmax, Q, k, ws, p.tau, p.tau_stride, st)) != ANNCUR_OK) return rc;
	if ((rc = co_join(co, st)) != ANNCUR_OK) return rc;
	EV(2);
	p.n_wg = P.n_rb * P.S;
	if ((rc = anncur_ensure_dyn_lds((const void *)wide_kernel<1, 16>, W_LDS_TOTAL)) != ANNCUR_OK) return rc;
	for (int stg = 0, prev = 0; stg < P.n_stages; prev = P.stage_end[stg], ++stg) {
		EV(5 + 2 * stg);
		p.bt_begin = prev; p.bt_end = P.stage_end[stg]; p.bt_per_split = P.stage_tps[stg]; p.carry = stg > 0;
		hipLaunchKernelGGL((wide_kernel<1, 16>), dim3(p.n_wg), dim3(512), W_LDS_TOTAL, st, p);
		ANNCUR_LAUNCH_OK();
		EV(6 + 2 * stg);
		if (stg + 1 < P.n_stages) {
			if ((rc = co_fork(co, st)) != ANNCUR_OK) return rc;
			if ((rc = launch_tau_refine(p.cand, p.seg_cnt, 4 * P.S, P.capg, Q, k, P.kmax, const_cast<float *>(p.tau), p.tau_stride, stg > 0 ? 1 : 0, st)) != ANNCUR_OK)
				return rc;
			if ((rc = co_join(co, st)) != ANNCUR_OK) return rc;
		}
	}
	EV(3);
	if ((rc = co_fork(co, st)) != ANNCUR_OK) return rc;
	SweepStages stages{};
	stages.n = P.n_stages;
	const int n_tiles32 = (int)ceil_div64(I, TILE_I), u = WBM / TILE_I;
	for (int g = 0, prev = 0; g < P.n_stages; prev = P.stage_end[g], ++g) {
		stages.begin[g] = prev * u;
		stages.end[g] = P.stage_end[g] * u < n_tiles32 ? P.stage_end[g] * u : n_tiles32;
		stages.tps[g] = P.stage_tps[g] * u;
	}
	if ((rc = launch_select(P, 4 * P.S, stages, p.cand, p.seg_cnt, p.X, ldx, p.Et, Q, I, KP, k, out_val, out_idx, ws, p.tau, p.tau_stride, st, item_ids)) != ANNCUR_OK) return rc;
	EV(4);
	return ANNCUR_OK;
}
#undef EV

FusedPlan plan_any(int64_t Q, int64_t I, int KP, int k, int flags = 0) {
	const bool leading = (flags & ANNCUR_TOPK_LEADING_SAMPLE) != 0, mfma16 = (flags & ANNCUR_TOPK_MFMA16) != 0, qt1 = (flags & ANNCUR_TOPK_QT1) != 0;
	return wide_kp(KP) ? plan_wide(Q, I, KP, k, leading) : plan_fused(Q, I, KP, k, leading, mfma16 && !qt1, qt1, (flags & ANNCUR_TOPK_MFMA32) != 0, false,
																	  (flags & ANNCUR_TOPK_STAGED) != 0);
}
bool ring_flag_ok(int flags) {
	return (flags & ANNCUR_TOPK_RING) == 0;
}
constexpr int TOPK_FLAGS = ANNCUR_TOPK_LEADING_SAMPLE | ANNCUR_TOPK_MFMA16 | ANNCUR_TOPK_QT1 | ANNCUR_TOPK_MFMA32 | ANNCUR_TOPK_RING | ANNCUR_TOPK_STAGED;

}

extern "C" size_t anncur_score_topk_workspace_bytes(int64_t Q, int64_t I, int32_t Kp, int32_t k) {
	const FusedPlan P = plan_any(Q, I, Kp, k);
	if (!P.ok) return 0;
	size_t t = P.total;
	for (int flags : {ANNCUR_TOPK_MFMA16, ANNCUR_TOPK_MFMA32, ANNCUR_TOPK_QT1, ANNCUR_TOPK_RING, ANNCUR_TOPK_STAGED}) {
		const FusedPlan V = plan_any(Q, I, Kp, k, flags);
		if (V.ok && V.total > t) t = V.total;
	}
	return t;
}

extern "C" int anncur_score_topk_supported(int64_t Q, int64_t I, int32_t Kp, int32_t k) {
	return plan_any(Q, I, Kp, k).ok ? 1 : 0;
}

static int score_topk_impl(const void *X, int64_t ldx, const void *Et, int64_t lde, int64_t Q, int64_t I, int32_t Kp,
						   int32_t k, float *out_val, int32_t *out_idx, void *workspace, size_t workspace_bytes,
						   void *stream, hipEvent_t *ev, int32_t flags = 0, const int32_t *item_ids = nullptr, CoScan *co = nullptr, const EvalArgs *ea = nullptr) {
	ANNCUR_REQUIRE((flags & ~TOPK_FLAGS) == 0, ANNCUR_E_INVALID, "score_topk: unknown flags 0x%x", flags);
	ANNCUR_REQUIRE(ring_flag_ok(flags), ANNCUR_E_UNSUPPORTED, "score_topk: ANNCUR_TOPK_RING (the tile-ring sweep body) is retired: measured slower than the default body");
	const FusedPlan P = ea ? plan_fused(Q, I, Kp, k, false, false, false, false, true) : plan_any(Q, I, Kp, k, flags);
	ANNCUR_REQUIRE(P.ok, ANNCUR_E_UNSUPPORTED,
				   "score_topk: (Q=%lld, I=%lld, Kp=%d, k=%d) is outside the fused path (Kp in {64,128,256,512} or a multiple of 128 up to %d, "
				   "1<=k<=%d, I large enough for a sampled threshold); use anncur_gemm + anncur_rowwise_topk",
				   (long long)Q, (long long)I, Kp, k, WIDE_KP_MAX, ANNCUR_MAX_TOPK);
	ANNCUR_REQUIRE(X && Et && out_val && out_idx, ANNCUR_E_INVALID, "score_topk: null pointer");
	ANNCUR_REQUIRE(lde == Kp, ANNCUR_E_INVALID, "score_topk: Et must be packed (lde == Kp), got lde=%lld", (long long)lde);
	ANNCUR_REQUIRE(ldx >= Kp && (ldx % 8) == 0, ANNCUR_E_INVALID, "score_topk: ldx must be >= Kp and a multiple of 8");
	ANNCUR_REQUIRE(((uintptr_t)X % 16) == 0 && ((uintptr_t)Et % 16) == 0, ANNCUR_E_INVALID, "score_topk: X and Et must be 16-byte aligned");
	ANNCUR_REQUIRE(workspace && workspace_bytes >= P.total && ((uintptr_t)workspace % 256) == 0, ANNCUR_E_WORKSPACE,
				   "score_topk: workspace of %zu bytes (256-byte aligned) required, got %zu", P.total, workspace_bytes);
	hipStream_t st = (hipStream_t)stream;
	unsigned char *ws = (unsigned char *)workspace;
	int rc;
	if (co && (rc = co_plan(*co, P.n_stages + 1)) != ANNCUR_OK) return rc;
	switch (Kp) {
		case 64: rc = launch_fused<64>(P, X, ldx, Et, Q, I, k, out_val, out_idx, ws, st, ev, co, item_ids, ea); break;
		case 128: rc = P.QT == 1 ? launch_fused<128, 1>(P, X, ldx, Et, Q, I, k, out_val, out_idx, ws, st, ev, co, item_ids)
								  : launch_fused<128>(P, X, ldx, Et, Q, I, k, out_val, out_idx, ws, st, ev, co, item_ids, ea); break;
		case 256: rc = P.QT == 1 ? launch_fused<256, 1>(P, X, ldx, Et, Q, I, k, out_val, out_idx, ws, st, ev, co, item_ids)
								  : launch_fused<256>(P, X, ldx, Et, Q, I, k, out_val, out_idx, ws, st, ev, co, item_ids, ea); break;
		case 512: rc = launch_fused<512>(P, X, ldx, Et, Q, I, k, out_val, out_idx, ws, st, ev, co, item_ids); break;
		default: rc = launch_wide(P, X, ldx, Et, Q, I, Kp, k, out_val, out_idx, ws, st, ev, co, item_ids); break;
	}
	if (rc == ANNCUR_OK) rc = co_finish(co, st);
	if (rc != ANNCUR_OK) co_abort(co, st);
	return rc;
}

extern "C" int anncur_score_topk_ex(const void *X, int64_t ldx, const void *Et, int64_t lde, int64_t Q, int64_t I, int32_t Kp,
									int32_t k, float *out_val, int32_t *out_idx, void *workspace, size_t workspace_bytes,
									int32_t flags, const int32_t *item_ids, void *stream) {
	return score_topk_impl(X, ldx, Et, lde, Q, I, Kp, k, out_val, out_idx, workspace, workspace_bytes, stream, nullptr, flags, item_ids);
}

extern "C" int anncur_score_topk(const void *X, int64_t ldx, const void *Et, int64_t lde, int64_t Q, int64_t I, int32_t Kp,
								 int32_t k, float *out_val, int32_t *out_idx, void *workspace, size_t workspace_bytes,
								 void *stream) {
	return score_topk_impl(X, ldx, Et, lde, Q, I, Kp, k, out_val, out_idx, workspace, workspace_bytes, stream, nullptr);
}

extern "C" int anncur_eval_topk(const void *A, int a_dtype, int64_t lda, int32_t k_exact, float *exact_val, int32_t *exact_idx,
								const void *X, int64_t ldx, const void *Et, int64_t lde, int64_t Q, int64_t I, int32_t Kp, int32_t k_retvr,
								float *approx_val, int32_t *approx_idx, void *workspace, size_t workspace_bytes, int32_t flags,
								const int32_t *item_ids, void *stream, void *aux_stream) {
	ANNCUR_REQUIRE(dtype_ok(a_dtype) && A && exact_val && exact_idx && lda >= I && k_exact >= 1 && k_exact <= I && k_exact <= ANNCUR_MAX_TOPK,
				   ANNCUR_E_INVALID, "eval_topk: bad exact-scan arguments");
	if (Q == 0) return ANNCUR_OK;
	if (!aux_stream || aux_stream == stream) {
		const int rc = anncur_rowwise_topk(A, a_dtype, Q, I, lda, k_exact, exact_val, exact_idx, stream);
		if (rc != ANNCUR_OK) return rc;
		return score_topk_impl(X, ldx, Et, lde, Q, I, Kp, k_retvr, approx_val, approx_idx, workspace, workspace_bytes, stream, nullptr, flags, item_ids);
	}
	CoScan co{};
	co.aux = (hipStream_t)aux_stream;
	co.A = A; co.a_dtype = a_dtype; co.lda = lda; co.Q = Q; co.I = I; co.k = k_exact; co.val = exact_val; co.idx = exact_idx;
	return score_topk_impl(X, ldx, Et, lde, Q, I, Kp, k_retvr, approx_val, approx_idx, workspace, workspace_bytes, stream, nullptr, flags, item_ids, &co);
}

extern "C" size_t anncur_eval_fused_workspace_bytes(int64_t Q, int64_t I, int32_t Kp, int32_t k) {
	const FusedPlan P = plan_fused(Q, I, Kp, k, false, false, false, false, true);
	return P.ok ? P.total : 0;
}

extern "C" int anncur_eval_fused_ex(const void *X, int64_t ldx, const void *Et, int64_t lde, const void *Et_hint, const void *A, int a_dtype, int64_t lda,
									int64_t Q, int64_t I, int32_t Kp, int32_t k, float *out_val, int32_t *out_idx, float *err_sq, float *norm_sq,
									void *workspace, size_t workspace_bytes, void *stream);
extern "C" int anncur_eval_fused(const void *X, int64_t ldx, const void *Et, int64_t lde, const void *A, int a_dtype, int64_t lda,
								 int64_t Q, int64_t I, int32_t Kp, int32_t k, float *out_val, int32_t *out_idx, float *err_sq, float *norm_sq,
								 void *workspace, size_t workspace_bytes, void *stream) {
	return anncur_eval_fused_ex(X, ldx, Et, lde, nullptr, A, a_dtype, lda, Q, I, Kp, k, out_val, out_idx, err_sq, norm_sq, workspace, workspace_bytes, stream);
}
extern "C" int anncur_eval_fused_ex(const void *X, int64_t ldx, const void *Et, int64_t lde, const void *Et_hint, const void *A, int a_dtype, int64_t lda,
									int64_t Q, int64_t I, int32_t Kp, int32_t k, float *out_val, int32_t *out_idx, float *err_sq, float *norm_sq,
									void *workspace, size_t workspace_bytes, void *stream) {
	ANNCUR_REQUIRE(Kp == 64 || Kp == 128 || Kp == 256, ANNCUR_E_UNSUPPORTED, "eval_fused: Kp must be 64, 128 or 256 (got %d): use anncur_score_topk + anncur_approx_error_packed", Kp);
	ANNCUR_REQUIRE(a_dtype == ANNCUR_BF16 && A && (lda % 8) == 0 && ((uintptr_t)A % 16) == 0 && lda >= I, ANNCUR_E_UNSUPPORTED,
				   "eval_fused: the exact matrix must be bf16 with 16-byte aligned rows (lda a multiple of 8): use anncur_score_topk + anncur_approx_error(_packed) otherwise");
	ANNCUR_REQUIRE(err_sq && norm_sq, ANNCUR_E_INVALID, "eval_fused: null pointer");
	ANNCUR_REQUIRE(exact_tile_offsets_fit(lda, 256), ANNCUR_E_UNSUPPORTED,
				   "eval_fused: row pitch %lld of the exact matrix is too long for the kernel's 32-bit tile offsets (255 rows x pitch x 2 bytes must stay below 2^32): use anncur_score_topk + anncur_approx_error_packed",
				   (long long)lda);
	ANNCUR_REQUIRE(anncur_eval_fused_workspace_bytes(Q, I, Kp, k) > 0, ANNCUR_E_UNSUPPORTED, "eval_fused: shape (Q=%lld, I=%lld, Kp=%d, k=%d) is outside the fused path",
				   (long long)Q, (long long)I, Kp, k);
	if (Q == 0) return ANNCUR_OK;
	hipStream_t st = (hipStream_t)stream;
	ANNCUR_HIP_OK(hipMemsetAsync(err_sq, 0, (size_t)Q * 4, st));
	ANNCUR_HIP_OK(hipMemsetAsync(norm_sq, 0, (size_t)Q * 4, st));
	const int64_t I_full = I / TILE_I * TILE_I;
	if (I_full < I) {
		const int rc = anncur_internal_approx_error_acc((const uint16_t *)X, ANNCUR_BF16, ldx, (const uint16_t *)Et + I_full * lde, ANNCUR_BF16, lde,
														(const void *)((const uint16_t *)A + I_full), a_dtype, lda, Q, I - I_full, Kp, err_sq, norm_sq, stream);
		if (rc != ANNCUR_OK) return rc;
	}
	const EvalArgs ea{(const uint16_t *)A, lda, err_sq, norm_sq, (const uint16_t *)Et_hint};
	return score_topk_impl(X, ldx, Et, lde, Q, I, Kp, k, out_val, out_idx, workspace, workspace_bytes, stream, nullptr, 0, nullptr, nullptr, &ea);
}

extern "C" int anncur_score_topk_timed(const void *X, int64_t ldx, const void *Et, int64_t lde, int64_t Q, int64_t I, int32_t Kp,
									   int32_t k, float *out_val, int32_t *out_idx, void *workspace, size_t workspace_bytes,
									   int32_t flags, const int32_t *item_ids, void *stream, float *stage_ms) {
	ANNCUR_REQUIRE(stage_ms, ANNCUR_E_INVALID, "score_topk_timed: stage_ms is null");
	constexpr int NEV = 11;
	hipEvent_t ev[NEV];
	for (int i = 0; i < NEV; ++i) ANNCUR_HIP_OK(hipEventCreate(&ev[i]));
	const FusedPlan P = plan_any(Q, I, Kp, k, flags);
	int rc = score_topk_impl(X, ldx, Et, lde, Q, I, Kp, k, out_val, out_idx, workspace, workspace_bytes, stream, ev, flags, item_ids);
	if (rc == ANNCUR_OK) {
		hipError_t e = hipEventSynchronize(ev[4]);
		if (e != hipSuccess) { anncur_set_error("hipEventSynchronize: %s", hipGetErrorString(e)); rc = ANNCUR_E_HIP; }
		for (int i = 0; i < 4 && rc == ANNCUR_OK; ++i)
			if (hipEventElapsedTime(&stage_ms[i], ev[i], ev[i + 1]) != hipSuccess) { anncur_set_error("hipEventElapsedTime failed"); rc = ANNCUR_E_HIP; }
		stage_ms[4] = 0.f;
		stage_ms[6] = stage_ms[7] = stage_ms[8] = 0.f;
		for (int g = 0; g < P.n_stages && rc == ANNCUR_OK; ++g) {
			float ms = 0.f;
			if (hipEventElapsedTime(&ms, ev[5 + 2 * g], ev[6 + 2 * g]) != hipSuccess) { anncur_set_error("hipEventElapsedTime failed"); rc = ANNCUR_E_HIP; }
			stage_ms[4] += ms;
			stage_ms[6 + g] = ms;
		}
		stage_ms[5] = (float)P.n_stages;
	}
	for (int i = 0; i < NEV; ++i) (void)hipEventDestroy(ev[i]);
	return rc;
}


extern "C" int anncur_score_topk_plan(int64_t Q, int64_t I, int32_t Kp, int32_t k, int32_t *out5) {
	const FusedPlan P = plan_any(Q, I, Kp, k);
	ANNCUR_REQUIRE(P.ok && out5, ANNCUR_E_UNSUPPORTED, "score_topk_plan: unsupported shape");
	out5[0] = P.n_st; out5[1] = P.n_tiles; out5[2] = P.S; out5[3] = P.capg; out5[4] = P.group;
	return ANNCUR_OK;
}

static void describe_plan(const FusedPlan &P, bool wide, int32_t (&v)[27]) {
	const int32_t head[8] = {P.n_st, P.n_tiles, P.S, P.capg, P.group, wide ? 4 : P.lg, P.QT, P.n_stages};
	for (int i = 0; i < 27; ++i) v[i] = i < 8 ? head[i] : 0;
	v[17] = (!wide && P.ladder) ? 1 : 0; v[18] = (!wide && P.ladder) ? P.ladder_k2 : 0; v[19] = LADDER_PERIOD;
	v[20] = (int32_t)(P.off_gmax / 256); v[21] = P.n_groups; v[22] = (!wide && P.body16 && P.group == 16) ? 1 : 0; v[23] = P.S0;
	for (int g = 0; g < 3; ++g) {
		const bool on = g < P.n_stages;
		v[8 + g] = on ? P.stage_end[g] : 0; v[11 + g] = on ? (wide ? P.stage_pred[g] : P.bodyef ? 6 : P.body16 ? 2 : P.bodyq16 ? 4 : P.stage_pred[g]) : 0; v[14 + g] = on ? P.stage_flush[g] : 0;
		v[24 + g] = on ? P.stage_tps[g] : 0;
	}
}

extern "C" int anncur_score_topk_plan_ex(int64_t Q, int64_t I, int32_t Kp, int32_t k, int32_t flags, int32_t *out, int32_t n_out) {
	ANNCUR_REQUIRE((flags & ~TOPK_FLAGS) == 0, ANNCUR_E_INVALID, "score_topk_plan_ex: unknown flags 0x%x", flags);
	ANNCUR_REQUIRE(ring_flag_ok(flags), ANNCUR_E_UNSUPPORTED, "score_topk_plan_ex: ANNCUR_TOPK_RING (the tile-ring sweep body) is retired");
	const FusedPlan P = plan_any(Q, I, Kp, k, flags);
	ANNCUR_REQUIRE(P.ok && out && n_out >= 0, ANNCUR_E_UNSUPPORTED, "score_topk_plan_ex: unsupported shape");
	int32_t v[27];
	describe_plan(P, wide_kp(Kp), v);
	for (int i = 0; i < n_out && i < 24; ++i) out[i] = v[i];
	return ANNCUR_OK;
}

extern "C" int anncur_eval_fused_plan(int64_t Q, int64_t I, int32_t Kp, int32_t k, int32_t *out, int32_t n_out) {
	ANNCUR_REQUIRE(Kp == 64 || Kp == 128 || Kp == 256, ANNCUR_E_UNSUPPORTED, "eval_fused_plan: Kp must be 64, 128 or 256 (got %d)", Kp);
	const FusedPlan P = plan_fused(Q, I, Kp, k, false, false, false, false, true);
	ANNCUR_REQUIRE(P.ok && out && n_out >= 0, ANNCUR_E_UNSUPPORTED, "eval_fused_plan: shape (Q=%lld, I=%lld, Kp=%d, k=%d) is outside the fused path",
				   (long long)Q, (long long)I, Kp, k);
	int32_t v[27];
	describe_plan(P, false, v);
	for (int i = 0; i < n_out && i < 27; ++i) out[i] = v[i];
	return ANNCUR_OK;
}

extern "C" int anncur_score_topk_survivors(const void *workspace, int64_t Q, int64_t I, int32_t Kp, int32_t k, int32_t flags, double *mean_per_query,
										   void *stream) {
	ANNCUR_REQUIRE((flags & ~TOPK_FLAGS) == 0 && workspace && mean_per_query, ANNCUR_E_INVALID, "score_topk_survivors: bad arguments");
	const FusedPlan P = plan_any(Q, I, Kp, k, flags);
	ANNCUR_REQUIRE(P.ok, ANNCUR_E_UNSUPPORTED, "score_topk_survivors: unsupported shape");
	const size_t n = (size_t)Q * (wide_kp(Kp) ? 4 : P.lg) * P.S;
	std::vector<uint32_t> h(n);
	ANNCUR_HIP_OK(hipMemcpyAsync(h.data(), (const unsigned char *)workspace + P.off_segcnt, n * 4, hipMemcpyDeviceToHost, (hipStream_t)stream));
	ANNCUR_HIP_OK(hipStreamSynchronize((hipStream_t)stream));
	double tot = 0.0;
	for (size_t i = 0; i < n; ++i) tot += (h[i] & 0x80000000u) ? 0.0 : (double)h[i];
	*mean_per_query = tot / (double)Q;
	return ANNCUR_OK;
}

extern "C" int anncur_score_topk_ladder_state(const void *workspace, int64_t Q, int64_t I, int32_t Kp, int32_t k, int32_t flags, float *levels,
											  uint32_t *counts, float *tau_final, float *tau0, void *stream) {
	ANNCUR_REQUIRE((flags & ~TOPK_FLAGS) == 0 && workspace && levels && counts && tau_final, ANNCUR_E_INVALID, "score_topk_ladder_state: bad arguments");
	ANNCUR_REQUIRE(ring_flag_ok(flags), ANNCUR_E_UNSUPPORTED, "score_topk_ladder_state: ANNCUR_TOPK_RING (the tile-ring sweep body) is retired");
	const FusedPlan P = plan_any(Q, I, Kp, k, flags);
	ANNCUR_REQUIRE(P.ok, ANNCUR_E_UNSUPPORTED, "score_topk_ladder_state: unsupported shape");
	ANNCUR_REQUIRE(!wide_kp(Kp) && P.ladder, ANNCUR_E_UNSUPPORTED, "score_topk_ladder_state: the plan of (Q=%lld, I=%lld, Kp=%d, k=%d, flags 0x%x) has no threshold ladder",
				   (long long)Q, (long long)I, Kp, k, flags);
	const unsigned char *ws = (const unsigned char *)workspace;
	hipStream_t st = (hipStream_t)stream;
	std::vector<uint32_t> words((size_t)Q * 4);
	ANNCUR_HIP_OK(hipMemcpyAsync(levels, ws + P.off_lvl, (size_t)Q * LADDER_LEVELS * 4, hipMemcpyDeviceToHost, st));
	ANNCUR_HIP_OK(hipMemcpyAsync(words.data(), ws + P.off_lcnt, (size_t)Q * 16, hipMemcpyDeviceToHost, st));
	ANNCUR_HIP_OK(hipMemcpyAsync(tau_final, ws + P.off_tau2, (size_t)Q * 4, hipMemcpyDeviceToHost, st));
	if (tau0) ANNCUR_HIP_OK(hipMemcpyAsync(tau0, ws + P.off_tau, (size_t)Q * 4, hipMemcpyDeviceToHost, st));
	ANNCUR_HIP_OK(hipStreamSynchronize(st));
	for (int64_t q = 0; q < Q; ++q)
		for (int j = 0; j < LADDER_LEVELS; ++j) counts[q * LADDER_LEVELS + j] = (words[(size_t)q * 4 + (j >> 1)] >> (16 * (j & 1))) & 0xffffu;
	return ANNCUR_OK;
}

extern "C" int anncur_approx_error_packed(const void *X, int64_t ldx, const void *Et, int64_t lde, const void *A, int a_dtype, int64_t lda,
										  int64_t Q, int64_t I, int32_t Kp, float *err_sq, float *norm_sq, void *stream) {
	ANNCUR_REQUIRE(Kp == 64 || Kp == 128 || Kp == 256 || Kp == 512, ANNCUR_E_UNSUPPORTED, "approx_error_packed: Kp must be 64, 128, 256 or 512 (got %d)", Kp);
	ANNCUR_REQUIRE(dtype_ok(a_dtype), ANNCUR_E_INVALID, "approx_error_packed: bad dtype");
	ANNCUR_REQUIRE(Q >= 0 && I >= 1 && I < (int64_t)0x7fffffff - 64 && lda >= I, ANNCUR_E_INVALID, "approx_error_packed: bad shape");
	ANNCUR_REQUIRE(X && Et && A && err_sq && norm_sq, ANNCUR_E_INVALID, "approx_error_packed: null pointer");
	ANNCUR_REQUIRE(lde == Kp && ldx >= Kp && (ldx % 8) == 0 && ((uintptr_t)X % 16) == 0 && ((uintptr_t)Et % 16) == 0, ANNCUR_E_INVALID,
				   "approx_error_packed: X / Et must be packed bf16 (lde == Kp, ldx multiple of 8, 16-byte aligned)");
	ANNCUR_REQUIRE((lda % 4) == 0 && ((uintptr_t)A % 16) == 0, ANNCUR_E_UNSUPPORTED,
				   "approx_error_packed: the exact matrix must be 16-byte aligned with lda a multiple of 4 (use anncur_approx_error otherwise)");
	if (Q == 0) return ANNCUR_OK;
	hipStream_t st = (hipStream_t)stream;
	ANNCUR_HIP_OK(hipMemsetAsync(err_sq, 0, (size_t)Q * 4, st));
	ANNCUR_HIP_OK(hipMemsetAsync(norm_sq, 0, (size_t)Q * 4, st));
	const int64_t I_full = I / TILE_I * TILE_I;
	if (I_full < I) {
		const int rc = anncur_internal_approx_error_acc((const uint16_t *)X, ANNCUR_BF16, ldx, (const uint16_t *)Et + I_full * lde, ANNCUR_BF16, lde,
														a_dtype == ANNCUR_F32 ? (const void *)((const float *)A + I_full) : (const void *)((const uint16_t *)A + I_full),
														a_dtype, lda, Q, I - I_full, Kp, err_sq, norm_sq, stream);
		if (rc != ANNCUR_OK) return rc;
	}
	if (I_full == 0) return ANNCUR_OK;
	FusedParams p{};
	p.X = (const uint16_t *)X; p.ldx = ldx; p.Et = (const uint16_t *)Et; p.Q = Q; p.I = I_full;
	const int QT = (Kp <= 256) ? 2 : 1, BQ = 128 * QT;
	const int n_rb = (int)ceil_div64(Q, BQ);
	p.n_tiles = (int)(I_full / TILE_I);
	int S = 2 * num_cu() / n_rb;
	if (S < 1) S = 1;
	if (S > p.n_tiles) S = p.n_tiles;
	p.tiles_per_split = (p.n_tiles + S - 1) / S;
	S = (p.n_tiles + p.tiles_per_split - 1) / p.tiles_per_split;
	p.n_wg = n_rb * S;
#define LAUNCH_ERR(KPV, TA)                                                                                                   \
	hipLaunchKernelGGL((error_kernel<KPV, TA>), dim3(p.n_wg), dim3(256), 2 * FusedCfg<KPV>::TILE_BYTES, st, p, (const TA *)A, lda, err_sq, norm_sq)
#define LAUNCH_ERR_K(TA)                                                                                                      \
	do {                                                                                                                      \
		switch (Kp) {                                                                                                         \
			case 64: LAUNCH_ERR(64, TA); break;                                                                               \
			case 128: LAUNCH_ERR(128, TA); break;                                                                             \
			case 256: LAUNCH_ERR(256, TA); break;                                                                             \
			default: LAUNCH_ERR(512, TA); break;                                                                              \
		}                                                                                                                     \
	} while (0)
	const bool lds_exact = a_dtype == ANNCUR_BF16 && (lda % 8) == 0 && ((uintptr_t)A % 16) == 0 && exact_tile_offsets_fit(lda, Kp <= 256 ? 256 : 128);
	if (lds_exact) {
#define LAUNCH_ERRL(KPV)                                                                                                      \
		do {                                                                                                                  \
			const int lds_ = 2 * FusedCfg<KPV>::TILE_BYTES + 2 * FusedCfg<KPV>::BQ * 64;                                      \
			{ const int rc_ = anncur_ensure_dyn_lds((const void *)error_lds_kernel<KPV>, lds_); if (rc_ != ANNCUR_OK) return rc_; } \
			hipLaunchKernelGGL((error_lds_kernel<KPV>), dim3(p.n_wg), dim3(256), lds_, st, p, (const uint16_t *)A, lda, err_sq, norm_sq); \
		} while (0)
		switch (Kp) {
			case 64: LAUNCH_ERRL(64); break;
			case 128: LAUNCH_ERRL(128); break;
			case 256: LAUNCH_ERRL(256); break;
			default: LAUNCH_ERRL(512); break;
		}
#undef LAUNCH_ERRL
	} else if (a_dtype == ANNCUR_F32) LAUNCH_ERR_K(float); else LAUNCH_ERR_K(uint16_t);
#undef LAUNCH_ERR_K
#undef LAUNCH_ERR
	ANNCUR_LAUNCH_OK();
	return ANNCUR_OK;
}
```

### anncur_amd/csrc/topk.hip

```cpp
#include <stdlib.h>
#include <atomic>
#include "select.hpp"
#include "wave_select.hpp"

using namespace anncur;

namespace {

constexpr int SCAN_PASS = 2048;

template <typename T> struct VecOf;
template <> struct VecOf<float> { static constexpr int N = 4; };
template <> struct VecOf<uint16_t> { static constexpr int N = 8; };

typedef uint32_t u32x4 __attribute__((ext_vector_type(4)));

template <typename T>
__device__ __forceinline__ float vec_elem(const u32x4 &r, int e);
template <>
__device__ __forceinline__ float vec_elem<float>(const u32x4 &r, int e) { return __uint_as_float(r[e]); }
template <>
__device__ __forceinline__ float vec_elem<uint16_t>(const u32x4 &r, int e) {
	const uint32_t w = r[e >> 1];
	return __uint_as_float((e & 1) ? (w & 0xffff0000u) : (w << 16));
// ... 285 lines not shown
		uint32_t pmask = 0u;                                                                                                    \
		_Pragma("unroll") for (int e = 0; e < VEC; ++e) {                                                                       \
			const float v = vec_elem_f32<T>(sv, e);                                                                             \
			const bool hit = nothr ? (v == v) : (v > w.tau);                                              \
			pmask |= hit ? (1u << e) : 0u;                                                                                      \
		}                                                                                                                       \
		if (!have) pmask = 0u;                                                                                                  \
		for (;;) {                                                                                                              \
			const bool hit = pmask != 0u;                                                                                       \
			const unsigned long long hm = __ballot(hit);                                                                        \
			if (hm == 0ull) break;                                                                                              \
			const int e = hit ? __builtin_ctz(pmask) : 0;                                                                       \
			wsel_push_mask(w, hm, hit, f32_sortable(vec_elem_f32_dyn<T>(sv, e)), 0xffffffffu - (i0 + (uint32_t)e));             \
			pmask &= pmask - 1u;                                                                                                \
		}                                                                                                                       \
		scnt = 0;                                                                                                               \
		__builtin_amdgcn_wave_barrier();                                                                                        \
		if (w.cnt > trig) wsel_compact_call<WS_CAP, HP, true>(w, k, tie_limit, wsel_base16(w.tau));                             \
	}
#define SCAN_STEP(d, FULL, POS)                                                                                                 \
	{                                                                                                                           \
		const u32x4 cur = pf[d];                                                                                                \
		const uint32_t mcur = GATHER ? pm[GATHER ? (d) : 0] : 0u;                                                               \
		bool pass;                                                                                                              \
		if (POS) pass = sp.any_pos(cur);                                                                                        \
		else pass = sp.any(sp.xform(cur));                                                                                      \
		if (FULL) {              \
			if (GATHER) pm[GATHER ? (d) : 0] = mblk[((d) + WS_PF) * WAVE + lane];                                     \
			if (BUF) pf[d] = __builtin_amdgcn_raw_buffer_load_b128(rs, voff + (uint32_t)(((d) & 3) * 1024), soff + (((d) & 4) ? 4096u : 0u), 2); \
			else pf[d] = __builtin_nontemporal_load(blk + ((d) + WS_PF) * WAVE + lane);                                         \
		} else {                    \
			const int64_t iv = (s0 + (d)) * WAVE + lane;                                                                        \
			const int64_t ivn = iv + (int64_t)WS_PF * WAVE;                                                                     \
			if (GATHER) pm[GATHER ? (d) : 0] = ivn < nvec ? gt.vtab[ivn] : 0u;                                       \
			pf[d] = vp[ivn < nvec ? ivn : vlast];                                                                               \
			pass = pass && iv < nvec;                                                                                           \
		}                                                                                                                       \
		if (GATHER) {                          \
			if (__ballot((mcur & 0xffu) != 0u) != 0ull) {                                                                       \
				if ((mcur & 0xffu) != 0u) {                                                                                     \
					uint32_t pos = mcur >> 8;                                                                                   \
					for (uint32_t mm = mcur & 0xffu; mm != 0u; mm &= mm - 1u) cqrow[pos++] = dyn_elem<T>(cur, __builtin_ctz(mm)); \
				}                                                                                                               \
			}                                                                                                                   \
		}                                                                                                                       \
		const unsigned long long pm = __ballot(pass);                                                                           \
		if (pm != 0ull) {                                                                                                       \
			const uint32_t np = (uint32_t)__popcll(pm);                                                                         \
			if (scnt + np > (uint32_t)WAVE) SCAN_DRAIN()                                                                        \
			if (pass) {                                                                                                         \
				const uint32_t pos = scnt + __builtin_amdgcn_mbcnt_hi((uint32_t)(pm >> 32), __builtin_amdgcn_mbcnt_lo((uint32_t)pm, 0u)); \
				 \
				*reinterpret_cast<__attribute__((address_space(3))) u32x4 *>((uintptr_t)(stage_vec_lds + pos * 16u)) = cur;            \
				*reinterpret_cast<__attribute__((address_space(3))) uint32_t *>((uintptr_t)(stage_idx_lds + pos * 4u)) = (uint32_t)(head + ((s0 + (d)) * WAVE + lane) * VEC); \
			}                                                                                                                   \
			scnt += np;                                                                                                         \
		}                                                                                                                       \
	}
	static_assert(WS_PF == 8, "the block spells out eight steps");
	int64_t s0 = 0;
	for (; (s0 + 2 * WS_PF) * WAVE <= nvec; s0 += WS_PF) {
		sp.set(w.tau);
		const u32x4 *blk = vp + s0 * WAVE;
		const uint32_t *mblk = GATHER ? gt.vtab + s0 * WAVE : nullptr;
		const uint32_t soff = (uint32_t)((s0 + WS_PF) * (WAVE * 16));
		(void)mblk; (void)blk; (void)soff;
		if (sp.pos) {
			SCAN_STEP(0, true, true) SCAN_STEP(1, true, true) SCAN_STEP(2, true, true) SCAN_STEP(3, true, true) SCAN_STEP(4, true, true) SCAN_STEP(5, true, true) SCAN_STEP(6, true, true) SCAN_STEP(7, true, true)
		} else {
			SCAN_STEP(0, true, false) SCAN_STEP(1, true, false) SCAN_STEP(2, true, false) SCAN_STEP(3, true, false) SCAN_STEP(4, true, false) SCAN_STEP(5, true, false) SCAN_STEP(6, true, false) SCAN_STEP(7, true, false)
		}
	}
	for (; s0 < nsteps; s0 += WS_PF) {
		sp.set(w.tau);
		const u32x4 *blk = vp;
		const uint32_t *mblk = nullptr;
		const uint32_t soff = 0u;
		(void)blk; (void)mblk; (void)soff;
		SCAN_STEP(0, false, false) SCAN_STEP(1, false, false) SCAN_STEP(2, false, false) SCAN_STEP(3, false, false) SCAN_STEP(4, false, false) SCAN_STEP(5, false, false) SCAN_STEP(6, false, false) SCAN_STEP(7, false, false)
	}
	if (scnt > 0u) SCAN_DRAIN()
#undef SCAN_STEP
#undef SCAN_DRAIN
	{
		const bool in = lane < I - tail0;
		wsel_offer_inorder(w, in, in ? load_as_f32<T>(row + tail0 + lane) : 0.f, (uint32_t)(tail0 + lane));
	}
	if (GATHER) {
		for (int j = lane; j < gt.n_idx; j += WAVE) {
			const int32_t c = gt.col_idx[j];
			if ((int64_t)c >= tail0 && (int64_t)c < I) cqrow[j] = row[c];
		}
	}
	wsel_finish<WS_CAP, HP, E>(w, k, out_val + q * (int64_t)k, out_idx + q * (int64_t)k, nullptr, wsel_base16(w.tau));
}

template <typename T, int E = 2>
__global__ __launch_bounds__(256) void rowwise_topk_short_kernel(const T *__restrict__ A, int64_t Q, int32_t I, int64_t lda, uint32_t k,
																  float *__restrict__ out_val, int32_t *__restrict__ out_idx) {
	extern __shared__ __attribute__((aligned(16))) unsigned char smem[];
	const int lane = lane_id(), wave = __builtin_amdgcn_readfirstlane((int)(threadIdx.x >> 6));
	const int64_t q = (int64_t)blockIdx.x * 4 + wave;
	if (q >= Q) return;
	WaveSel w = wsel_init<WS_CAP>(smem + wave * WaveSelLayout<WS_CAP>::BYTES);
	constexpr int HP = sizeof(T) == 2 ? 2 : 4;
	const T *row = A + q * lda;
	for (int32_t i0 = 0; i0 < I; i0 += WAVE) {
		const int32_t i = i0 + lane;
		const float v = i < I ? load_as_f32<T>(row + i) : 0.f;
		wsel_push(w, i < I && v == v, f32_sortable(v), 0xffffffffu - (uint32_t)i);
	}
	__builtin_amdgcn_wave_barrier();
	wsel_finish<WS_CAP, HP, E>(w, k, out_val + q * (int64_t)k, out_idx + q * (int64_t)k);
}

constexpr int KTH_MAX_N = 4096;
__device__ __forceinline__ void kth2_coarse(const WaveSel &w, uint32_t *hist2, const uint32_t *key, uint32_t n, uint32_t k, uint32_t k2, uint32_t &T, uint32_t &G) {
	const uint32_t lane = (uint32_t)lane_id();
	uint32_t bin0 = 0, a0 = 0, hb = 0, binG0 = 0, aG0 = 0;
#pragma unroll
	for (int pass = 0; pass < 2; ++pass) {
#pragma unroll
		for (int i = 0; i < 4; ++i) { w.hist[lane * 4 + i] = 0; hist2[lane * 4 + i] = 0; }
		__builtin_amdgcn_wave_barrier();
#pragma unroll 4
		for (uint32_t j0 = 0; j0 < n; j0 += WAVE) {
			const uint32_t j = j0 + lane;
			if (j < n) {
				const uint32_t x = key[j];
				if (pass == 0) atomicAdd(&w.hist[x >> 24], 1u);
				else {
					if ((x >> 24) == bin0) atomicAdd(&w.hist[(x >> 16) & 255u], 1u);
					else if ((x >> 24) == binG0) atomicAdd(&hist2[(x >> 16) & 255u], 1u);
				}
			}
		}
		__builtin_amdgcn_wave_barrier();
		if (pass == 0) {
			wsel_find_bin(w.hist, lane, k, bin0, a0, hb);
			wsel_find_bin(w.hist, lane, k2, binG0, aG0, hb);
		} else {
			uint32_t bin1, a1, binG1 = 0;
			wsel_find_bin(w.hist, lane, k - a0, bin1, a1, hb);
			T = ((bin0 << 8) | bin1) << 16;
			wsel_find_bin(binG0 == bin0 ? w.hist : hist2, lane, k2 - aG0, binG1, a1, hb);
			G = ((binG0 << 8) | binG1) << 16;
		}
		__builtin_amdgcn_wave_barrier();
	}
}

__global__ __launch_bounds__(256) void kth_value_wave_kernel(const float *__restrict__ G, int64_t Q, int n, int64_t ldg, uint32_t k,
															  float *__restrict__ out, int64_t out_stride, int n_pad, int coarse,
															  float *__restrict__ ladder, uint32_t k2, float *__restrict__ tau2) {
	extern __shared__ __attribute__((aligned(16))) unsigned char kth_smem[];
	const uint32_t lane = (uint32_t)lane_id();
	const int wave = threadIdx.x >> 6;
	uint32_t *hist = reinterpret_cast<uint32_t *>(kth_smem) + wave * (256 + n_pad + (ladder ? 256 : 0));
	uint32_t *keys = hist + 256;
	const int64_t q = (int64_t)blockIdx.x * 4 + wave;
	if (q >= Q) return;
	const float *g = G + q * ldg;
	for (uint32_t j = lane; j < (uint32_t)n; j += WAVE) {
		const float v = g[j];
		keys[j] = (v == v) ? f32_sortable(v) : 0u;
	}
	__builtin_amdgcn_wave_barrier();
	WaveSel w;
	w.whi = keys; w.wlo = nullptr; w.sort_buf = nullptr; w.hist = hist;
	w.cnt = (uint32_t)n; w.tau_hi = 0; w.tau_lo = 0; w.tau = 0.f;
	uint32_t need;
	uint32_t kk, gk = 0;
	if (ladder) kth2_coarse(w, hist + 256 + n_pad, w.whi, (uint32_t)n, k, k2 < k ? k2 : k, kk, gk);
	else if (coarse) kk = wsel_kth<false, 2>(w, w.whi, (uint32_t)n, k, need, w.whi, 0u);
	else kk = wsel_kth<false, 4>(w, w.whi, (uint32_t)n, k, need, w.whi, 0u);
	if (lane == 0) out[q * out_stride] = f32_unsortable(kk);
	if (ladder) {
		const float t0 = f32_unsortable(kk), g = f32_unsortable(gk);
		float d = g - t0;
		if (!(d > 0.f) || !(d < INFINITY)) d = 0.f;
		if (lane < (uint32_t)LADDER_LEVELS) ladder[q * LADDER_LEVELS + lane] = t0 + d * ((float)(lane + 1) * (1.0f / LADDER_LEVELS));
		if (lane == 0 && tau2) tau2[q] = t0;
	}
}

template <typename T, int KMAX>
__global__ __launch_bounds__(SEL_THREADS) void rerank_kernel(const T *__restrict__ A, int64_t I, int64_t lda,
															  const int32_t *__restrict__ approx_idx, int64_t ld_idx,
															  uint32_t k_retvr, uint32_t k_out, float *__restrict__ out_val,
															  int32_t *__restrict__ out_idx) {
	extern __shared__ __attribute__((aligned(16))) unsigned char smem[];
	const SelState s = sel_carve<KMAX>(smem);
	sel_init(s);
	const int tid = threadIdx.x;
	const int64_t q = blockIdx.x;
	const T *row = A + q * lda;
	const int32_t *ai = approx_idx + q * ld_idx;
	float tau = -INFINITY;
	uint64_t tau_key = 0;
	for (uint32_t j0 = 0; j0 < k_retvr; j0 += SEL_THREADS) {
		const uint32_t j = j0 + tid;
		int32_t it = (j < k_retvr) ? ai[j] : -1;
		const bool in = it >= 0 && (int64_t)it < I;
		const float v = in ? load_as_f32<T>(row + it) : 0.f;
		sel_offer(s, in, v, (uint32_t)it, tau, tau_key);
	}
	sel_finish<KMAX>(s, k_out, out_val + q * (int64_t)k_out, out_idx + q * (int64_t)k_out);
}

constexpr int OVL_MAX_PAIRS = 64;
struct OvlPairs { int32_t ka[OVL_MAX_PAIRS]; int32_t kb[OVL_MAX_PAIRS]; };

__global__ __launch_bounds__(256) void overlap_kernel(const int32_t *__restrict__ a, int32_t la,
													   const int32_t *__restrict__ b, int32_t lb, int64_t Q,
													   OvlPairs pairs, int32_t n_pairs, int32_t *__restrict__ common) {
	extern __shared__ __attribute__((aligned(16))) unsigned char smem[];
	int32_t *sb = reinterpret_cast<int32_t *>(smem);
	int32_t *spos = sb + lb;
	int32_t *scnt = spos + la;
	const int tid = threadIdx.x;
	const int64_t q = blockIdx.x;
	for (int j = tid; j < lb; j += 256) sb[j] = b[q * lb + j];
	for (int p = tid; p < n_pairs; p += 256) scnt[p] = 0;
	__syncthreads();
	for (int j = tid; j < la; j += 256) {
		const int32_t x = a[q * la + j];
		int32_t pos = lb;
		if (x >= 0) {
			for (int t = 0; t < lb; ++t)
				if (sb[t] == x) { pos = t; break; }
		}
		spos[j] = pos;
	}
	__syncthreads();
	for (int p = 0; p < n_pairs; ++p) {
		const int ka = pairs.ka[p], kb = pairs.kb[p];
		int c = 0;
		for (int j = tid; j < ka; j += 256) c += (spos[j] < kb) ? 1 : 0;
		for (int d = WAVE / 2; d > 0; d >>= 1) c += __shfl_xor(c, d);
		if (lane_id() == 0 && c) atomicAdd(&scnt[p], c);
	}
	__syncthreads();
	for (int p = tid; p < n_pairs; p += 256) common[(int64_t)p * Q + q] = scnt[p];
}

__global__ __launch_bounds__(256) void overlap_wave_kernel(const int32_t *__restrict__ a, int32_t la, const int32_t *__restrict__ b,
															int32_t lb, int64_t Q, OvlPairs pairs, int32_t n_pairs,
															int32_t *__restrict__ common) {
	const int lane = lane_id();
	const int64_t q = (int64_t)blockIdx.x * 4 + (threadIdx.x >> 6);
	if (q >= Q) return;
	int32_t av[2], bv[2], pos[2];
#pragma unroll
	for (int e = 0; e < 2; ++e) {
		const int j = e * WAVE + lane;
		av[e] = j < la ? a[q * la + j] : -1;
		bv[e] = j < lb ? b[q * lb + j] : -2;
		pos[e] = 0x7fffffff;
	}
#pragma unroll
	for (int e = 1; e >= 0; --e) {
		const int lim = min(WAVE, lb - e * WAVE);
		for (int t = lim - 1; t >= 0; --t) {
			const int32_t x = __builtin_amdgcn_readlane(bv[e], t);
			const int p = e * WAVE + t;
			const unsigned long long m0 = __ballot(av[0] == x), m1 = __ballot(av[1] == x);
#if defined(__HIP_DEVICE_COMPILE__)
			if (m0 != 0ull) asm volatile("s_mov_b32 m0, %2\n\ts_nop 0\n\tv_writelane_b32 %0, %1, m0" : "+v"(pos[0]) : "s"(p), "s"((int)__builtin_ctzll(m0)) : "m0");
			if (m1 != 0ull) asm volatile("s_mov_b32 m0, %2\n\ts_nop 0\n\tv_writelane_b32 %0, %1, m0" : "+v"(pos[1]) : "s"(p), "s"((int)__builtin_ctzll(m1)) : "m0");
#endif
		}
	}
	for (int p = 0; p < n_pairs; ++p) {
		const int ka = pairs.ka[p], kb = pairs.kb[p];
		const int c = __popcll(__ballot(lane < ka && av[0] >= 0 && pos[0] < kb)) +
					  __popcll(__ballot(WAVE + lane < ka && av[1] >= 0 && pos[1] < kb));
		if (lane == 0) common[(int64_t)p * Q + q] = c;
	}
}

template <typename TS, typename TD>
__device__ __forceinline__ TD cvt(TS x);
template <> __device__ __forceinline__ float cvt<float, float>(float x) { return x; }
template <> __device__ __forceinline__ uint16_t cvt<uint16_t, uint16_t>(uint16_t x) { return x; }
template <> __device__ __forceinline__ float cvt<uint16_t, float>(uint16_t x) { return bf16_bits_to_f32(x); }
template <> __device__ __forceinline__ uint16_t cvt<float, uint16_t>(float x) { return f32_to_bf16_bits(x); }

template <typename TS, typename TD>
__global__ __launch_bounds__(256) void gather_cols_kernel(const TS *__restrict__ A, int64_t n_rows, int64_t n_cols,
														   int64_t lda, const int32_t *__restrict__ col_idx,
														   int32_t n_idx, TD *__restrict__ out, int64_t ldo) {
	const int64_t r = (int64_t)blockIdx.x * 4 + (threadIdx.x >> 6);
	if (r >= n_rows) return;
	const TS *row = A + r * lda;
	constexpr int U = 4;
	for (int j0 = threadIdx.x & 63; j0 < n_idx; j0 += 64 * U) {
		int32_t c[U];
		TS v[U];
#pragma unroll
		for (int u = 0; u < U; ++u) c[u] = (j0 + 64 * u < n_idx) ? col_idx[j0 + 64 * u] : -1;
#pragma unroll
		for (int u = 0; u < U; ++u) {
			const bool in = c[u] >= 0 && (int64_t)c[u] < n_cols;
			v[u] = in ? row[c[u]] : cvt<float, TS>(0.f);
		}
#pragma unroll
		for (int u = 0; u < U; ++u)
			if (j0 + 64 * u < n_idx) out[r * ldo + j0 + 64 * u] = cvt<TS, TD>(v[u]);
	}
}

template <typename TS, typename TD>
__global__ __launch_bounds__(256) void gather_rows_kernel(const TS *__restrict__ A, int64_t n_rows, int64_t n_cols,
														   int64_t lda, const int32_t *__restrict__ row_idx,
														   TD *__restrict__ out, int64_t ldo) {
	const int64_t j = blockIdx.y;
	const int32_t r = row_idx[j];
	const bool in = r >= 0 && (int64_t)r < n_rows;
	const int64_t c = (int64_t)blockIdx.x * 256 + threadIdx.x;
	if (c < n_cols) out[j * ldo + c] = in ? cvt<TS, TD>(A[(int64_t)r * lda + c]) : cvt<float, TD>(0.f);
}

template <typename TS, typename TD>
__global__ __launch_bounds__(256) void convert_kernel(const TS *__restrict__ src, int64_t lds_, TD *__restrict__ dst,
													   int64_t ldd, int64_t n_rows, int64_t n_cols) {
	const int64_t r = blockIdx.y;
	const int64_t c = (int64_t)blockIdx.x * 256 + threadIdx.x;
	if (c < n_cols) dst[r * ldd + c] = cvt<TS, TD>(src[r * lds_ + c]);
}

__global__ __launch_bounds__(256) void copy_bytes_kernel(const uint4 *__restrict__ src, uint4 *__restrict__ dst, size_t n16,
														  const unsigned char *__restrict__ src_tail, unsigned char *__restrict__ dst_tail, int n_tail) {
	const size_t i = (size_t)blockIdx.x * 256 + threadIdx.x;
	if (i < n16) dst[i] = src[i];
	if (blockIdx.x == 0 && (int)threadIdx.x < n_tail) dst_tail[threadIdx.x] = src_tail[threadIdx.x];
}

template <typename F>
int dispatch2(int sd, int dd, F &&f) {
	if (sd == ANNCUR_F32 && dd == ANNCUR_F32) return f((const float *)nullptr, (float *)nullptr);
	if (sd == ANNCUR_F32 && dd == ANNCUR_BF16) return f((const float *)nullptr, (uint16_t *)nullptr);
	if (sd == ANNCUR_BF16 && dd == ANNCUR_F32) return f((const uint16_t *)nullptr, (float *)nullptr);
	return f((const uint16_t *)nullptr, (uint16_t *)nullptr);
}

int kmax_class(int k) { return k <= 128 ? 128 : (k <= 512 ? 512 : 2048); }

}

int anncur_internal_kth_value(const float *G, int64_t Q, int n, int64_t ldg, int k, float *out, int64_t out_stride, hipStream_t st, int coarse,
							  float *ladder, int k2, float *tau2) {
	ANNCUR_REQUIRE(n >= 1 && n <= KTH_MAX_N && k >= 1 && k <= n, ANNCUR_E_INVALID, "kth_value: need 1 <= k <= n <= 4096");
	const unsigned grid = (unsigned)ceil_div64(Q, 4);
	const int n_pad = (n + 63) & ~63;
	const int lds = 4 * (256 + n_pad + (ladder ? 256 : 0)) * 4;
	int rc;
	if (lds > 64 * 1024 && (rc = anncur_ensure_dyn_lds((const void *)kth_value_wave_kernel, lds)) != ANNCUR_OK) return rc;
	hipLaunchKernelGGL(kth_value_wave_kernel, dim3(grid), dim3(256), lds, st, G, Q, n, ldg, (uint32_t)k, out, out_stride, n_pad, coarse, ladder, (uint32_t)(k2 < 1 ? 1 : k2), tau2);
	ANNCUR_LAUNCH_OK();
	return ANNCUR_OK;
}

int anncur_internal_scan_rows_in_flight(int dtype) {
	constexpr int MAX_DEV = 64;
	static std::atomic<int> cached[MAX_DEV][2];
	int dev = 0;
	if (hipGetDevice(&dev) != hipSuccess) { (void)hipGetLastError(); dev = 0; }
	const int di = dtype == ANNCUR_F32 ? 0 : 1;
	std::atomic<int> *slot = (dev >= 0 && dev < MAX_DEV) ? &cached[dev][di] : nullptr;
	int v = slot ? slot->load(std::memory_order_relaxed) : 0;
	if (v == 0) {
		int occ = 0;
		const size_t lds = 4 * (size_t)WaveSelLayout<WS_CAP>::BYTES;
		const hipError_t e = di == 0 ? hipOccupancyMaxActiveBlocksPerMultiprocessor(&occ, rowwise_topk_wave_kernel<float>, 256, lds)
									 : hipOccupancyMaxActiveBlocksPerMultiprocessor(&occ, rowwise_topk_wave_kernel<uint16_t>, 256, lds);
		if (e != hipSuccess || occ < 1) { (void)hipGetLastError(); occ = 3; }
		v = occ * 4 * anncur_num_cu();
		if (slot) slot->store(v, std::memory_order_relaxed);
	}
	return v;
}

extern "C" int anncur_rowwise_topk(const void *A, int dtype, int64_t Q, int64_t I, int64_t lda, int32_t k,
								   float *out_val, int32_t *out_idx, void *stream) {
	ANNCUR_REQUIRE(dtype_ok(dtype), ANNCUR_E_INVALID, "rowwise_topk: bad dtype %d", dtype);
	ANNCUR_REQUIRE(Q >= 0 && I >= 1 && lda >= I, ANNCUR_E_INVALID, "rowwise_topk: bad shape Q=%lld I=%lld lda=%lld",
				   (long long)Q, (long long)I, (long long)lda);
	ANNCUR_REQUIRE(k >= 1 && k <= ANNCUR_MAX_TOPK && k <= I, ANNCUR_E_INVALID, "rowwise_topk: k=%d out of range (1..min(I,%d))",
				   k, ANNCUR_MAX_TOPK);
	ANNCUR_REQUIRE(I < (int64_t)0x7fffffff, ANNCUR_E_INVALID, "rowwise_topk: I too large for int32 indices");
	ANNCUR_REQUIRE(A && out_val && out_idx, ANNCUR_E_INVALID, "rowwise_topk: null pointer");
	ANNCUR_REQUIRE(((uintptr_t)A % dtype_size(dtype)) == 0, ANNCUR_E_INVALID, "rowwise_topk: misaligned A");
	if (Q == 0) return ANNCUR_OK;
	hipStream_t st = (hipStream_t)stream;
	const int kc = kmax_class(k);
#define LAUNCH_ROWTOPK(T, KM)                                                                                   \
	do {                                                                                                        \
		{ const int rc_ = anncur_ensure_dyn_lds((const void *)rowwise_topk_kernel<T, KM, (KM == 128)>, (int)(SelCfg<KM, SCAN_PASS>::LDS_BYTES)); if (rc_ != ANNCUR_OK) return rc_; } \
		hipLaunchKernelGGL((rowwise_topk_kernel<T, KM, (KM == 128)>), dim3((unsigned)Q), dim3(SEL_THREADS), (SelCfg<KM, SCAN_PASS>::LDS_BYTES), st, \
						   (const T *)A, I, lda, (uint32_t)k, out_val, out_idx);                                \
	} while (0)
	ANNCUR_REQUIRE(Q < (int64_t)0x7fffffff, ANNCUR_E_INVALID, "rowwise_topk: Q too large");
	bool wave_scan = k <= WSEL_K;
	if (wave_scan && I <= (int64_t)WS_CAP) {
		const size_t lds = 4 * (size_t)WaveSelLayout<WS_CAP>::BYTES;
		const unsigned grid = (unsigned)ceil_div64(Q, 4);
		if (dtype == ANNCUR_F32) {
			if (k <= 64) hipLaunchKernelGGL((rowwise_topk_short_kernel<float, 1>), dim3(grid), dim3(256), lds, st, (const float *)A, Q, (int32_t)I, lda, (uint32_t)k, out_val, out_idx);
			else hipLaunchKernelGGL((rowwise_topk_short_kernel<float, 2>), dim3(grid), dim3(256), lds, st, (const float *)A, Q, (int32_t)I, lda, (uint32_t)k, out_val, out_idx);
		} else {
			if (k <= 64) hipLaunchKernelGGL((rowwise_topk_short_kernel<uint16_t, 1>), dim3(grid), dim3(256), lds, st, (const uint16_t *)A, Q, (int32_t)I, lda, (uint32_t)k, out_val, out_idx);
			else hipLaunchKernelGGL((rowwise_topk_short_kernel<uint16_t, 2>), dim3(grid), dim3(256), lds, st, (const uint16_t *)A, Q, (int32_t)I, lda, (uint32_t)k, out_val, out_idx);
		}
		ANNCUR_LAUNCH_OK();
		return ANNCUR_OK;
	}
	if (wave_scan) {
		size_t lds = 4 * (size_t)WaveSelLayout<WS_CAP>::BYTES;
		const unsigned grid = (unsigned)ceil_div64(Q, 4);
		uint32_t trig = ws_trigger((uint32_t)k);
		bool buf = I * (int64_t)dtype_size(dtype) < ((int64_t)1 << 31);
		if (dtype == ANNCUR_F32) {
			if (buf) hipLaunchKernelGGL((rowwise_topk_wave_kernel<float, false, true>), dim3(grid), dim3(256), lds, st, (const float *)A, Q, I, lda, (uint32_t)k, trig, out_val, out_idx);
			else hipLaunchKernelGGL((rowwise_topk_wave_kernel<float, false, false>), dim3(grid), dim3(256), lds, st, (const float *)A, Q, I, lda, (uint32_t)k, trig, out_val, out_idx);
		} else {
			if (buf) hipLaunchKernelGGL((rowwise_topk_wave_kernel<uint16_t, false, true>), dim3(grid), dim3(256), lds, st, (const uint16_t *)A, Q, I, lda, (uint32_t)k, trig, out_val, out_idx);
			else hipLaunchKernelGGL((rowwise_topk_wave_kernel<uint16_t, false, false>), dim3(grid), dim3(256), lds, st, (const uint16_t *)A, Q, I, lda, (uint32_t)k, trig, out_val, out_idx);
		}
		ANNCUR_LAUNCH_OK();
		return ANNCUR_OK;
	}
	if (dtype == ANNCUR_F32) {
		if (kc == 128) LAUNCH_ROWTOPK(float, 128); else if (kc == 512) LAUNCH_ROWTOPK(float, 512); else LAUNCH_ROWTOPK(float, 2048);
	} else {
		if (kc == 128) LAUNCH_ROWTOPK(uint16_t, 128); else if (kc == 512) LAUNCH_ROWTOPK(uint16_t, 512); else LAUNCH_ROWTOPK(uint16_t, 2048);
	}
#undef LAUNCH_ROWTOPK
	ANNCUR_LAUNCH_OK();
	return ANNCUR_OK;
}

extern "C" int anncur_rowwise_topk_ragged(const void *A, int dtype, int64_t Q, int64_t I_max, int64_t lda, const int32_t *row_len, int32_t k,
										  float *out_val, int32_t *out_idx, void *stream) {
	ANNCUR_REQUIRE(dtype_ok(dtype), ANNCUR_E_INVALID, "rowwise_topk_ragged: bad dtype %d", dtype);
	ANNCUR_REQUIRE(Q >= 0 && Q < (int64_t)0x7fffffff && I_max >= 1 && I_max < (int64_t)0x7fffffff && lda >= I_max, ANNCUR_E_INVALID,
				   "rowwise_topk_ragged: bad shape Q=%lld I_max=%lld lda=%lld", (long long)Q, (long long)I_max, (long long)lda);
	ANNCUR_REQUIRE(k >= 1 && k <= I_max, ANNCUR_E_INVALID, "rowwise_topk_ragged: k=%d out of range (1..I_max)", k);
	if (k > WSEL_K) { anncur_set_error("rowwise_topk_ragged: k = %d above the wave-per-row scan's %d", k, WSEL_K); return ANNCUR_E_UNSUPPORTED; }
	if (Q == 0) return ANNCUR_OK;
	ANNCUR_REQUIRE(A && row_len && out_val && out_idx && ((uintptr_t)A % dtype_size(dtype)) == 0, ANNCUR_E_INVALID, "rowwise_topk_ragged: null or misaligned pointer");
	hipStream_t st = (hipStream_t)stream;
	const size_t lds = 4 * (size_t)WaveSelLayout<WS_CAP>::BYTES;
	const unsigned grid = (unsigned)ceil_div64(Q, 4);
	const uint32_t trig = ws_trigger((uint32_t)k);
	const bool buf = I_max * (int64_t)dtype_size(dtype) < ((int64_t)1 << 31);
#define LAUNCH_RAGGED(T, B, EE) hipLaunchKernelGGL((rowwise_topk_wave_kernel<T, false, B, true, EE>), dim3(grid), dim3(256), lds, st, (const T *)A, Q, I_max, lda, (uint32_t)k, trig, out_val, out_idx, ScanGather{}, row_len)
	if (dtype == ANNCUR_F32) {
		if (k <= 64) { if (buf) LAUNCH_RAGGED(float, true, 1); else LAUNCH_RAGGED(float, false, 1); }
		else { if (buf) LAUNCH_RAGGED(float, true, 2); else LAUNCH_RAGGED(float, false, 2); }
	} else {
		if (k <= 64) { if (buf) LAUNCH_RAGGED(uint16_t, true, 1); else LAUNCH_RAGGED(uint16_t, false, 1); }
		else { if (buf) LAUNCH_RAGGED(uint16_t, true, 2); else LAUNCH_RAGGED(uint16_t, false, 2); }
	}
#undef LAUNCH_RAGGED
	ANNCUR_LAUNCH_OK();
	return ANNCUR_OK;
}

extern "C" int anncur_gather_tables(const int32_t *col_idx, int32_t n_idx, int64_t I, int dtype, uint32_t *vec_tab, void *stream) {
	ANNCUR_REQUIRE(dtype_ok(dtype) && col_idx && vec_tab && n_idx >= 1 && n_idx <= 65535 && I >= 1, ANNCUR_E_INVALID, "gather_tables: bad arguments");
	const int vec = dtype == ANNCUR_F32 ? 4 : 8;
	const int64_t n_vec = ceil_div64(I, vec);
	hipLaunchKernelGGL(gather_tables_kernel, dim3((unsigned)ceil_div64(n_vec, 256)), dim3(256), 0, (hipStream_t)stream, col_idx, (int)n_idx, n_vec, vec, vec_tab);
	ANNCUR_LAUNCH_OK();
	return ANNCUR_OK;
}

extern "C" int anncur_rowwise_topk_gather(const void *A, int dtype, int64_t Q, int64_t I, int64_t lda, int32_t k, float *out_val, int32_t *out_idx,
										  const int32_t *col_idx, int32_t n_idx, const uint32_t *vec_tab, void *cq, int64_t ldo, void *stream) {
	ANNCUR_REQUIRE(dtype_ok(dtype), ANNCUR_E_INVALID, "rowwise_topk_gather: bad dtype %d", dtype);
	ANNCUR_REQUIRE(Q >= 0 && I >= 1 && lda >= I && Q < (int64_t)0x7fffffff && I < (int64_t)0x7fffffff, ANNCUR_E_INVALID, "rowwise_topk_gather: bad shape");
	ANNCUR_REQUIRE(k >= 1 && k <= WSEL_K && k <= I, ANNCUR_E_UNSUPPORTED, "rowwise_topk_gather: k=%d outside the wave-level scan (1..%d)", k, WSEL_K);
	ANNCUR_REQUIRE(A && out_val && out_idx && col_idx && vec_tab && cq, ANNCUR_E_INVALID, "rowwise_topk_gather: null pointer");
	ANNCUR_REQUIRE(n_idx >= 1 && n_idx <= 65535 && ldo >= n_idx, ANNCUR_E_INVALID, "rowwise_topk_gather: bad anchor count / output pitch");
	ANNCUR_REQUIRE(((uintptr_t)A % 16) == 0 && (Q == 1 || ((size_t)lda * dtype_size(dtype)) % 16 == 0), ANNCUR_E_UNSUPPORTED,
				   "rowwise_topk_gather: A and its rows must be 16-byte aligned (use anncur_gather_cols + anncur_rowwise_topk)");
	if (Q == 0) return ANNCUR_OK;
	hipStream_t st = (hipStream_t)stream;
	const size_t lds = 4 * (size_t)WaveSelLayout<WS_CAP>::BYTES;
	const unsigned grid = (unsigned)ceil_div64(Q, 4);
	const uint32_t trig = ws_trigger((uint32_t)k);
	ScanGather gt{vec_tab, col_idx, n_idx, cq, ldo};
	if (dtype == ANNCUR_F32)
		hipLaunchKernelGGL((rowwise_topk_wave_kernel<float, true, false>), dim3(grid), dim3(256), lds, st, (const float *)A, Q, I, lda, (uint32_t)k, trig, out_val, out_idx, gt);
	else
		hipLaunchKernelGGL((rowwise_topk_wave_kernel<uint16_t, true, false>), dim3(grid), dim3(256), lds, st, (const uint16_t *)A, Q, I, lda, (uint32_t)k, trig, out_val, out_idx, gt);
	ANNCUR_LAUNCH_OK();
	return ANNCUR_OK;
}

extern "C" int anncur_rerank(const void *A, int dtype, int64_t Q, int64_t I, int64_t lda, const int32_t *approx_idx,
							 int64_t ld_idx, int32_t k_retvr, int32_t k_out, float *rerank_val, int32_t *rerank_idx, void *stream) {
	ANNCUR_REQUIRE(dtype_ok(dtype), ANNCUR_E_INVALID, "rerank: bad dtype %d", dtype);
	ANNCUR_REQUIRE(Q >= 0 && I >= 1 && lda >= I && Q < (int64_t)0x7fffffff, ANNCUR_E_INVALID, "rerank: bad shape");
	ANNCUR_REQUIRE(k_retvr >= 1 && k_retvr <= ANNCUR_MAX_TOPK && k_out >= 1 && k_out <= k_retvr, ANNCUR_E_INVALID,
				   "rerank: need 1 <= k_out <= k_retvr <= %d (got %d, %d)", ANNCUR_MAX_TOPK, k_out, k_retvr);
	ANNCUR_REQUIRE(ld_idx >= k_retvr, ANNCUR_E_INVALID, "rerank: ld_idx < k_retvr");
	ANNCUR_REQUIRE(A && approx_idx && rerank_val && rerank_idx, ANNCUR_E_INVALID, "rerank: null pointer");
	if (Q == 0) return ANNCUR_OK;
	hipStream_t st = (hipStream_t)stream;
	const int kc = kmax_class(k_out);
// ... 116 lines not shown
```

### anncur_amd/ops.py

```python
from collections import namedtuple
import ctypes
import functools
import itertools

import numpy as np
import torch

from . import _lib
from ._lib import F32, BF16, check

TopK = namedtuple("TopK", ["values", "indices"])

_DT = {torch.float32: F32, torch.bfloat16: BF16}


def _dt(t):
	try:
		return _DT[t.dtype]
	except KeyError:
		raise TypeError(f"unsupported dtype {t.dtype}: anncur_amd kernels take float32 or bfloat16") from None


def _dev(*ts):
	for t in ts:
# ... 582 lines not shown


@_on_device
def score_topk_fused(Xp, Etp, I, k, return_fallbacks=False, workspace=None, leading_sample=False, item_ids=None, mfma16=False, qt1=False, mfma32=False, ring=False, staged=False):
	_dev(Xp, Etp)
	if Xp.dtype != torch.bfloat16 or Etp.dtype != torch.bfloat16:
		raise TypeError("score_topk_fused takes bf16 operands")
	Q, Kp = Xp.shape
	if Etp.shape[1] != Kp or not Etp.is_contiguous() or Etp.shape[0] < -(-I // 32) * 32:
		raise ValueError("Et must be packed [ceil(I/32)*32 x Kp]")
	Xp = _rowmajor(Xp)
	lib = _lib.load()
	nbytes = lib.anncur_score_topk_workspace_bytes(Q, I, Kp, k)
	if nbytes == 0:
		raise _lib.AnncurHipError(f"score_topk: shape (Q={Q}, I={I}, Kp={Kp}, k={k}) is outside the fused path")
	if workspace is None and nbytes > FUSED_WS_LIMIT_BYTES and Q > 512 and not return_fallbacks:
		qc = Q
		while qc > 512 and lib.anncur_score_topk_workspace_bytes(qc, I, Kp, k) > FUSED_WS_LIMIT_BYTES:
			qc = max(512, (qc // 2 + 255) // 256 * 256)
		val = torch.empty((Q, k), dtype=torch.float32, device=Xp.device)
		idx = torch.empty((Q, k), dtype=torch.int32, device=Xp.device)
		for q0 in range(0, Q, qc):
			part = score_topk_fused(Xp[q0:q0 + qc], Etp, I, k, leading_sample=leading_sample, item_ids=item_ids, mfma16=mfma16, qt1=qt1, mfma32=mfma32, ring=ring, staged=staged)
			val[q0:q0 + qc], idx[q0:q0 + qc] = part.values, part.indices
		return TopK(val, idx)
	if workspace is None:
		ws = _Workspace.get(nbytes, Xp.device)
	else:
		ws = workspace
		if ws.numel() < nbytes or ws.data_ptr() % 256 != 0 or ws.device != Xp.device:
			raise ValueError("score_topk_fused: workspace too small, misaligned or on another device (use fused_workspace())")
	val = torch.empty((Q, k), dtype=torch.float32, device=Xp.device)
	idx = torch.empty((Q, k), dtype=torch.int32, device=Xp.device)
	ids = _item_ids_arg(item_ids, I, Xp.device)
	check(lib.anncur_score_topk_ex(_p(Xp), _ld(Xp), _p(Etp), Kp, Q, I, Kp, k, _p(val), _p(idx), _p(ws), nbytes,
								   _topk_flags(leading_sample, mfma16, qt1, mfma32, ring, staged), _p(ids) if ids is not None else None, _stream()), "score_topk")
	if return_fallbacks:
		return TopK(val, idx), ws[:4].view(torch.int32)
	return TopK(val, idx)


_aux_streams = {}


def aux_stream(device):
	key = (device.type, device.index if device.index is not None else torch.cuda.current_device())
	if key not in _aux_streams:
		_aux_streams[key] = torch.cuda.Stream(device=device)
	return _aux_streams[key]


_cu_streams = {}


def cu_partition_streams(device, n_scan):
	device = torch.device(device)
	idx = device.index if device.index is not None else torch.cuda.current_device()
	if torch.cuda.current_stream(idx).cuda_stream == 0:
		raise _lib.AnncurHipError("cu_partition_streams: the current stream is the NULL stream, which synchronises implicitly with CU-masked (blocking) streams; "
								  "make a non-default stream current first (with torch.cuda.stream(torch.cuda.Stream()): ...)")
	n_cu = torch.cuda.get_device_properties(idx).multi_processor_count
	n_scan = (int(n_scan) // 32) * 32
	if not (0 < n_scan < n_cu):
		raise ValueError(f"cu_partition_streams: n_scan={n_scan} must leave CUs on both sides of {n_cu}")
	key = (idx, n_scan)
	if key not in _cu_streams:
		hip = ctypes.CDLL("libamdhip64.so")
		fn = hip.hipExtStreamCreateWithCUMask
		fn.argtypes = [ctypes.POINTER(ctypes.c_void_p), ctypes.c_uint32, ctypes.POINTER(ctypes.c_uint32)]
		words = (n_cu + 31) // 32
		def make(lo, hi):
			mask = (ctypes.c_uint32 * words)(*[sum(1 << b for b in range(32) if lo <= 32 * w + b < hi) for w in range(words)])
			h = ctypes.c_void_p()
			with torch.cuda.device(idx):
				rc = fn(ctypes.byref(h), words, mask)
			if rc != 0 or not h.value:
				raise _lib.AnncurHipError(f"hipExtStreamCreateWithCUMask failed (code {rc})")
			return torch.cuda.ExternalStream(h.value, device=torch.device("cuda", idx))
		_cu_streams[key] = (make(n_scan, n_cu), make(0, n_scan))
	return _cu_streams[key]


@_on_device
def eval_topk(A, k, Xp, Etp, I, k_retvr, workspace=None, leading_sample=False, item_ids=None, mfma16=False, qt1=False, aux=None, serial=False, mfma32=False, ring=False, staged=False):
	_dev(A, Xp, Etp)
	if Xp.dtype != torch.bfloat16 or Etp.dtype != torch.bfloat16:
		raise TypeError("eval_topk takes bf16 retrieval operands")
	A = _rowmajor(A)
	Q, Kp = Xp.shape
	if A.shape[0] != Q or A.shape[1] != I or Etp.shape[1] != Kp or not Etp.is_contiguous() or Etp.shape[0] < -(-I // 32) * 32:
		raise ValueError("eval_topk: A must be [Q x I], Et packed [ceil(I/32)*32 x Kp]")
	Xp = _rowmajor(Xp)
	lib = _lib.load()
	nbytes = lib.anncur_score_topk_workspace_bytes(Q, I, Kp, k_retvr)
	if nbytes == 0:
		raise _lib.AnncurHipError(f"eval_topk: shape (Q={Q}, I={I}, Kp={Kp}, k={k_retvr}) is outside the fused path")
	ws = _Workspace.get(nbytes, Xp.device) if workspace is None else workspace
	if ws.numel() < nbytes or ws.data_ptr() % 256 != 0 or ws.device != Xp.device:
		raise ValueError("eval_topk: workspace too small, misaligned or on another device (use fused_workspace())")
	ev = torch.empty((Q, k), dtype=torch.float32, device=A.device)
	ei = torch.empty((Q, k), dtype=torch.int32, device=A.device)
	av = torch.empty((Q, k_retvr), dtype=torch.float32, device=A.device)
	ai = torch.empty((Q, k_retvr), dtype=torch.int32, device=A.device)
	ids = _item_ids_arg(item_ids, I, Xp.device)
	if serial:
		aux_p = None
	else:
		aux = aux or aux_stream(A.device)
		aux_p = ctypes.c_void_p(aux.cuda_stream)
	check(lib.anncur_eval_topk(_p(A), _dt(A), _ld(A), k, _p(ev), _p(ei), _p(Xp), _ld(Xp), _p(Etp), Kp, Q, I, Kp, k_retvr, _p(av), _p(ai), _p(ws), nbytes,
							   _topk_flags(leading_sample, mfma16, qt1, mfma32, ring, staged), _p(ids) if ids is not None else None, _stream(), aux_p), "eval_topk")
	return TopK(ev, ei), TopK(av, ai)


@_on_device
def score_topk_fused_timed(Xp, Etp, I, k, leading_sample=False, item_ids=None, mfma16=False, qt1=False, mfma32=False, ring=False, staged=False):
	_dev(Xp, Etp)
	Q, Kp = Xp.shape
	lib = _lib.load()
	nbytes = lib.anncur_score_topk_workspace_bytes(Q, I, Kp, k)
	if nbytes == 0:
		raise _lib.AnncurHipError("score_topk_timed: unsupported shape")
	ws = _Workspace.get(nbytes, Xp.device)
	val = torch.empty((Q, k), dtype=torch.float32, device=Xp.device)
	idx = torch.empty((Q, k), dtype=torch.int32, device=Xp.device)
	ms = (ctypes.c_float * 9)()
	ids = _item_ids_arg(item_ids, I, Xp.device)
	check(lib.anncur_score_topk_timed(_p(Xp), _ld(Xp), _p(Etp), Kp, Q, I, Kp, k, _p(val), _p(idx), _p(ws), nbytes,
									  _topk_flags(leading_sample, mfma16, qt1, mfma32, ring, staged), _p(ids) if ids is not None else None, _stream(), ms),
		  "score_topk_timed")
	return TopK(val, idx), [float(x) for x in ms]


@_on_device
def fused_survivors(workspace, Q, I, Kp, k, leading_sample=False, mfma16=False, qt1=False, mfma32=False, ring=False, staged=False):
	out = ctypes.c_double()
	check(_lib.load().anncur_score_topk_survivors(_p(workspace), Q, I, Kp, k, _topk_flags(leading_sample, mfma16, qt1, mfma32, ring, staged), ctypes.byref(out), _stream()),
		  "score_topk_survivors")
	return out.value


@_on_device
def fused_ladder_state(workspace, Q, I, Kp, k, leading_sample=False, mfma16=False, qt1=False, mfma32=False, ring=False, staged=False):
	levels = np.zeros((Q, 8), dtype=np.float32)
	counts = np.zeros((Q, 8), dtype=np.uint32)
	tau_final = np.zeros(Q, dtype=np.float32)
	tau0 = np.zeros(Q, dtype=np.float32)
	check(_lib.load().anncur_score_topk_ladder_state(_p(workspace), Q, I, Kp, k, _topk_flags(leading_sample, mfma16, qt1, mfma32, ring, staged),
													  levels.ctypes.data, counts.ctypes.data, tau_final.ctypes.data, tau0.ctypes.data, _stream()),
		  "score_topk_ladder_state")
	return {"levels": levels, "counts": counts, "tau_final": tau_final, "tau0": tau0}


def fused_plan(Q, I, Kp, k, leading_sample=False, mfma16=False, qt1=False, mfma32=False, ring=False, staged=False):
	out = (ctypes.c_int32 * 20)()
	check(_lib.load().anncur_score_topk_plan_ex(Q, I, Kp, k, _topk_flags(leading_sample, mfma16, qt1, mfma32, ring, staged), out, 20), "score_topk_plan_ex")
	v = [int(x) for x in out]
	plan = dict(zip(("n_sample_tiles", "n_tiles", "splits", "segment_capacity", "group", "lg", "QT", "n_stages"), v[:8]))
	n = plan["n_stages"]
	plan["stage_end"], plan["stage_pred"], plan["stage_flush"] = v[8:8 + n], v[11:11 + n], v[14:14 + n]
	plan["ladder"], plan["ladder_top_rank"] = bool(v[17]), v[18]
	plan["ladder_period"] = v[19]
	return plan


def eval_fused_plan(Q, I, Kp, k):
	out = (ctypes.c_int32 * 27)()
	check(_lib.load().anncur_eval_fused_plan(Q, I, Kp, k, out, 27), "eval_fused_plan")
	v = [int(x) for x in out]
	plan = dict(zip(("n_sample_tiles", "n_tiles", "splits", "segment_capacity", "group", "lg", "QT", "n_stages"), v[:8]))
	n = plan["n_stages"]
	plan["stage_end"], plan["stage_pred"], plan["stage_flush"], plan["stage_tiles_per_split"] = v[8:8 + n], v[11:11 + n], v[14:14 + n], v[24:24 + n]
	return plan


def fused_group_maxima(workspace, Q, I, Kp, k, leading_sample=False, mfma16=False, qt1=False, mfma32=False, ring=False, staged=False):
	out = (ctypes.c_int32 * 24)()
	check(_lib.load().anncur_score_topk_plan_ex(Q, I, Kp, k, _topk_flags(leading_sample, mfma16, qt1, mfma32, ring, staged), out, 24), "score_topk_plan_ex")
	off, n_groups = int(out[20]) * 256, int(out[21])
	gmax = workspace[off:off + Q * n_groups * 4].view(torch.float32).view(Q, n_groups)
	return gmax, {"prepass16": bool(out[22]), "prepass_splits": int(out[23]), "n_groups": n_groups}


def _dense_scores(X, Et):
	return gemm(X, Et.t())


@_on_device
def score_topk_dense(X, Et, k, max_bytes=2 << 30):
	_dev(X, Et)
	Q, I = X.shape[0], Et.shape[0]
	val = torch.empty((Q, k), dtype=torch.float32, device=X.device)
	idx = torch.empty((Q, k), dtype=torch.int32, device=X.device)
	rows = max(1, min(Q, max_bytes // max(4 * I, 1)))
	for q0 in range(0, Q, rows):
		q1 = min(Q, q0 + rows)
		S = _dense_scores(X[q0:q1], Et)
		v, i = rowwise_topk(S, k)
		val[q0:q1], idx[q0:q1] = v, i
	return TopK(val, idx)


@_on_device
def rerank(A, approx_idx, k_retvr, k_out):
	_dev(A, approx_idx)
	A = _rowmajor(A)
	if approx_idx.dtype != torch.int32 or approx_idx.stride(1) != 1:
		approx_idx = approx_idx.to(torch.int32).contiguous()
	Q, I = A.shape
	val = torch.empty((Q, k_out), dtype=torch.float32, device=A.device)
	idx = torch.empty((Q, k_out), dtype=torch.int32, device=A.device)
	check(_lib.load().anncur_rerank(_p(A), _dt(A), Q, I, _ld(A), _p(approx_idx), _ld(approx_idx), k_retvr, k_out, _p(val), _p(idx),
									_stream()), "rerank")
	return TopK(val, idx)


@_on_device
def overlap_counts(a, b, pairs, mapped_host_out=None):
	_dev(a, b)
	a = a.to(torch.int32).contiguous()
	b = b.to(torch.int32).contiguous()
	Q = a.shape[0]
	if mapped_host_out is not None:
		out = mapped_host_out
		if out.is_cuda or not out.is_pinned() or not out.is_contiguous() or out.dtype != torch.int32 or tuple(out.shape) != (len(pairs), Q):
			raise ValueError("overlap_counts: mapped_host_out must be a contiguous pinned int32 host tensor [n_pairs, Q]")
	else:
		out = torch.empty((len(pairs), Q), dtype=torch.int32, device=a.device)
	lib = _lib.load()
	for s in range(0, len(pairs), 64):
		chunk = pairs[s:s + 64]
		ka = (ctypes.c_int32 * len(chunk))(*[int(p[0]) for p in chunk])
		kb = (ctypes.c_int32 * len(chunk))(*[int(p[1]) for p in chunk])
		check(lib.anncur_overlap_counts(_p(a), a.shape[1], _p(b), b.shape[1], Q, ka, kb, len(chunk), _p(out[s:s + len(chunk)]), _stream()),
			  "overlap_counts")
	return out


@_on_device
def ivf_build_lists(assign, nlist):
	_dev(assign)
	assign = assign.to(torch.int32).contiguous()
	n = assign.numel()
	counts = torch.empty(nlist, dtype=torch.int32, device=assign.device)
	offsets = torch.empty(nlist + 1, dtype=torch.int32, device=assign.device)
	ids = torch.empty(n, dtype=torch.int32, device=assign.device)
	check(_lib.load().anncur_ivf_build_lists(_p(assign), n, nlist, _p(counts), _p(offsets), _p(ids), _stream()), "ivf_build_lists")
	return counts, offsets, ids


@_on_device
def descending_norm_order(M, n_buckets=256):
	_dev(M)
	M = _rowmajor(M)
	if M.dtype != torch.float32:
		raise TypeError("descending_norm_order takes fp32")
	n = M.shape[0]
	norms = torch.empty(n, dtype=torch.float32, device=M.device)
	mm = torch.empty(2, dtype=torch.int32, device=M.device)
	bucket = torch.empty(n, dtype=torch.int32, device=M.device)
	check(_lib.load().anncur_norm_buckets(_p(M), n, M.shape[1], _ld(M), n_buckets, _p(norms), _p(mm), _p(bucket), _stream()), "norm_buckets")
	return ivf_build_lists(bucket, n_buckets)[2]


@_on_device
def ivf_list_means(Xs, offsets, centroids):
	_dev(Xs, offsets, centroids)
	Xs = _rowmajor(Xs)
	if Xs.dtype != torch.float32 or centroids.dtype != torch.float32 or centroids.stride(1) != 1:
		raise TypeError("ivf_list_means takes fp32 row-major tensors")
	check(_lib.load().anncur_ivf_list_means(_p(Xs), _ld(Xs), centroids.shape[1], _p(offsets), centroids.shape[0], _p(centroids), _ld(centroids), _stream()),
		  "ivf_list_means")
	return centroids


@_on_device
def renorm_rows(M):
	_dev(M)
	if M.dtype != torch.float32 or M.dim() != 2 or (M.shape[1] > 1 and M.stride(1) != 1):
		raise TypeError("renorm_rows takes a row-major fp32 matrix")
	check(_lib.load().anncur_renorm_rows(_p(M), M.shape[0], M.shape[1], _ld(M), _stream()), "renorm_rows")
	return M


@_on_device
def ivf_scan(Xs, offsets, ids, Q, probe, k):
	_dev(Xs, offsets, ids, Q, probe)
	nq, dp = Q.shape
	probe = probe.to(torch.int32).contiguous()
	val = torch.empty((nq, k), dtype=torch.float32, device=Q.device)
	idx = torch.empty((nq, k), dtype=torch.int32, device=Q.device)
	check(_lib.load().anncur_ivf_scan(_p(Xs), _ld(Xs), dp, _p(offsets), _p(ids), _p(Q), _ld(Q), nq, _p(probe), probe.shape[1], k, _p(val), _p(idx), _stream()),
		  "ivf_scan")
	return TopK(val, idx)


@_on_device
def ivf_scan_grouped(Xs, offsets, ids, sizes_host, Q, probe, k, max_bytes=8 << 30, lists_bf16=None, profile=None):
	_dev(Xs, offsets, ids, Q, probe)
	lib = _lib.load()
	nq_all, dp = Q.shape
	probe = probe.to(torch.int32).contiguous()
	nprobe, nlist = probe.shape[1], sizes_host.shape[0]
	lmax = int(max(int(sizes_host.max()), 1))
	lmax = -(-lmax // 8) * 8
	k_eff = min(k, nprobe * lmax)
	val = torch.empty((nq_all, k), dtype=torch.float32, device=Q.device)
	idx = torch.empty((nq_all, k), dtype=torch.int32, device=Q.device)
	step = max(64, min(nq_all, max_bytes // (nprobe * lmax * 4)))
	vt = -(-sizes_host // 64)
	vt_sum, vt_max = int(vt.sum()), int(max(int(vt.max()), 1))
	for q0 in range(0, nq_all, step):
		q1 = min(nq_all, q0 + step)
		nq = q1 - q0
		pr = probe[q0:q1].contiguous()
		cnt, poff, pair_ids = ivf_build_lists(pr.reshape(-1).clamp(min=0), nlist)
# ... 101 lines not shown
```

Measured before the change: 11.99 million queries/s.

## Skip re-sweeping sample tiles by reusing prepass top-2 group maxima

The prepass now records, per 8-item group, the second-largest score and the argmax position alongside the group maximum. With the leading-sample plan, the main sweep begins after the sample tiles. Candidates from the sample region are taken directly from the group maxima when only the max clears tau, and groups where the second value also clears it are rescored with a small MFMA. The kth-value kernel also computes per-level seed counts for the ladder. This removes the recomputation of scores for sample tiles, at the cost of extra prepass stores, workspace, and per-query rescoring work in the select kernels.

```diff
diff --git a/anncur_amd/csrc/common.hpp b/anncur_amd/csrc/common.hpp
--- a/anncur_amd/csrc/common.hpp
+++ b/anncur_amd/csrc/common.hpp
@@ -8,7 +8,7 @@
 void anncur_set_error(const char *fmt, ...);
 constexpr int LADDER_LEVELS = 8;
 int anncur_internal_kth_value(const float *G, int64_t Q, int n, int64_t ldg, int k, float *out, int64_t out_stride, hipStream_t st, int coarse = 0,
-							  float *ladder = nullptr, int k2 = 1, float *tau2 = nullptr);
+							  float *ladder = nullptr, int k2 = 1, float *tau2 = nullptr, uint32_t *seed_cnt = nullptr);
 int anncur_internal_approx_error_acc(const void *X, int x_dtype, int64_t ldx, const void *Et, int e_dtype, int64_t lde, const void *Aex, int a_dtype,
 									 int64_t lda, int64_t Q, int64_t I, int64_t K, float *err_sq, float *norm_sq, void *stream);
 
diff --git a/anncur_amd/csrc/prepass16.hpp b/anncur_amd/csrc/prepass16.hpp
--- a/anncur_amd/csrc/prepass16.hpp
+++ b/anncur_amd/csrc/prepass16.hpp
@@ -47,6 +47,28 @@
 #if defined(__HIP_DEVICE_COMPILE__)
 	asm volatile("s_nop 7\n\ts_nop 2" : "+v"(acc[0][0]), "+v"(acc[0][1]), "+v"(acc[0][2]), "+v"(acc[0][3]), "+v"(acc[1][0]), "+v"(acc[1][1]), "+v"(acc[1][2]), "+v"(acc[1][3]));
 #endif
+}
+
+__device__ __forceinline__ void prepass16_top2(const f32x4 &a0, const f32x4 &a1, float &m1, float &m2, uint32_t &pos) {
+	m1 = -INFINITY; m2 = -INFINITY; pos = 0u;
+#pragma unroll
+	for (int e = 0; e < 8; ++e) {
+		const float v = e < 4 ? a0[e] : a1[e - 4];
+		const bool gt = v > m1;
+		m2 = gt ? m1 : fmaxf(m2, v);
+		pos = gt ? (uint32_t)(8 * (e >> 2) + (e & 3)) : pos;
+		m1 = gt ? v : m1;
+	}
+}
+__device__ __forceinline__ void prepass16_merge2(float a1, float a2, uint32_t ap, float b1, float b2, uint32_t bp, float &second, uint32_t &pos) {
+	const auto s1 = __builtin_amdgcn_permlane32_swap(__float_as_uint(a1), __float_as_uint(b1), false, false);
+	const auto s2 = __builtin_amdgcn_permlane32_swap(__float_as_uint(a2), __float_as_uint(b2), false, false);
+	const auto sp = __builtin_amdgcn_permlane32_swap(ap, bp, false, false);
+	const float l1 = __uint_as_float(s1[0]), u1 = __uint_as_float(s1[1]), l2 = __uint_as_float(s2[0]), u2 = __uint_as_float(s2[1]);
+	const uint32_t lp = sp[0], up = sp[1] + 4u;
+	const bool low = l1 > u1 || (l1 == u1 && lp < up);
+	second = low ? fmaxf(l2, u1) : fmaxf(u2, l1);
+	pos = low ? lp : up;
 }
 
 template <int KP>
@@ -116,6 +138,9 @@
 	const bool st_ok0 = q_st < p.Q, st_ok1 = q_st + 32 < p.Q;
 	float *const gdst = p.gmax + (st_ok0 ? q_st : 0) * p.n_groups + (g4 & 1);
 	const int64_t gdst_pair = (int64_t)32 * p.n_groups;
+	const bool top2 = p.gmax2 != nullptr;
+	float *const g2dst = p.gmax2 + (st_ok0 ? q_st : 0) * p.n_groups + (g4 & 1);
+	uint8_t *const gpdst = p.gpos + (st_ok0 ? q_st : 0) * p.n_groups + (g4 & 1);
 	uint32_t aoff[K];
 #pragma unroll
 	for (int s = 0; s < K; ++s) {
@@ -139,10 +164,23 @@
 		const auto s23 = __builtin_amdgcn_permlane32_swap(__float_as_uint(m[2]), __float_as_uint(m[3]), false, false);          \
 		const float v01 = fmaxf(__uint_as_float(s01[0]), __uint_as_float(s01[1]));                                              \
 		const float v23 = fmaxf(__uint_as_float(s23[0]), __uint_as_float(s23[1]));                                              \
+		float w01 = 0.f, w23 = 0.f;                                                                                             \
+		uint32_t p01 = 0u, p23 = 0u;                                                                                            \
+		if (top2) {                     \
+			float b1[4], b2[4];                                                                                                 \
+			uint32_t bp[4];                                                                                                     \
+			_Pragma("unroll") for (int t = 0; t < 4; ++t) prepass16_top2(acc[0][t], acc[1][t], b1[t], b2[t], bp[t]);            \
+			prepass16_merge2(b1[0], b2[0], bp[0], b1[1], b2[1], bp[1], w01, p01);                                               \
+			prepass16_merge2(b1[2], b2[2], bp[2], b1[3], b2[3], bp[3], w23, p23);                                               \
+		}                                                                                                                       \
 		                         \
 		if (ahead) vm_wait_all_but<C::PIECES>(); else vm_wait_all_but<0>();                                                     \
 		if (st_ok0) gdst[2 * (int64_t)j] = v01;                                                                                 \
 		if (st_ok1) gdst[gdst_pair + 2 * (int64_t)j] = v23;                                                                     \
+		if (top2) {                                                                                                             \
+			if (st_ok0) { g2dst[2 * (int64_t)j] = w01; gpdst[2 * (int64_t)j] = (uint8_t)p01; }                                  \
+			if (st_ok1) { g2dst[gdst_pair + 2 * (int64_t)j] = w23; gpdst[gdst_pair + 2 * (int64_t)j] = (uint8_t)p23; }          \
+		}                                                                                                                       \
 		__builtin_amdgcn_s_barrier();                                                                                           \
 		++j;                                                                                                                    \
 	} while (0)
diff --git a/anncur_amd/csrc/score_fused.hip b/anncur_amd/csrc/score_fused.hip
--- a/anncur_amd/csrc/score_fused.hip
+++ b/anncur_amd/csrc/score_fused.hip
@@ -74,6 +74,7 @@
 	uint32_t *nfb;
 	int ring_stagger, ring_spin_sleep;
 	uint32_t zero_bytes;
+	float *gmax2; uint8_t *gpos;
 };
 
 __device__ __forceinline__ int xcd_remap(int b, int n) {
@@ -1009,13 +1010,63 @@
 	const uint8_t *owner[3];
 };
 
+struct SampleArgs {
+	const float *gmax, *gmax2;
+	const uint8_t *gpos;
+	int n_groups;
+	const uint16_t *X; int64_t ldx; const uint16_t *Et; int KP;
+	uint32_t *n_rescored;
+};
+
+__device__ __forceinline__ void sample_rescore16(const SampleArgs &sa, int64_t q, int gi, int lane, float (&out)[4]) {
+	typedef __attribute__((ext_vector_type(4))) float v4f;
+	const int c16 = lane & 15, g4 = lane >> 4;
+	const int64_t row = (int64_t)(gi >> 1) * TILE_I + 8 * (c16 >> 2) + 4 * (gi & 1) + (c16 & 3);
+	const u32x4 *a = reinterpret_cast<const u32x4 *>(sa.Et + row * sa.KP) + g4;
+	const u32x4 *b = reinterpret_cast<const u32x4 *>(sa.X + q * sa.ldx) + g4;
+	v4f acc = {0.f, 0.f, 0.f, 0.f};
+	for (int ks = 0; ks < sa.KP / 32; ++ks)
+		acc = __builtin_amdgcn_mfma_f32_16x16x32_bf16(__builtin_bit_cast(bf16x8, a[4 * ks]), __builtin_bit_cast(bf16x8, b[4 * ks]), acc, 0, 0, 0);
+	out[0] = acc[0]; out[1] = acc[1]; out[2] = acc[2]; out[3] = acc[3];
+}
+
+template <typename Offer>
+__device__ __forceinline__ uint32_t sample_collect64(const SampleArgs &sa, int64_t q, int g0, float tau, int lane, Offer &&offer) {
+	const int gi = g0 + lane;
+	const bool in = gi < sa.n_groups;
+	const int64_t at = q * sa.n_groups + (in ? gi : 0);
+	const float m1 = in ? sa.gmax[at] : -INFINITY, m2 = in ? sa.gmax2[at] : -INFINITY;
+	const uint32_t pos = in ? (uint32_t)sa.gpos[at] : 0u;
+	const bool hit = in && m1 >= tau;
+	const bool again = hit && (m2 >= tau || m1 == 0.f || m1 == -INFINITY);
+	const bool direct = hit && !again;
+	uint32_t n = (uint32_t)__popcll(__ballot(direct));
+	offer(direct, m1, (uint32_t)((gi >> 1) * TILE_I + 8 * (int)(pos >> 2) + 4 * (gi & 1) + (int)(pos & 3u)));
+	unsigned long long rm = __ballot(again);
+	if (rm != 0ull && lane == 0 && sa.n_rescored) atomicAdd(sa.n_rescored, (uint32_t)__popcll(rm));
+	while (rm != 0ull) {
+		const int gs = g0 + (__ffsll((long long)rm) - 1);
+		rm &= rm - 1ull;
+		float sc[4];
+		sample_rescore16(sa, q, gs, lane, sc);
+		const uint32_t item0 = (uint32_t)((gs >> 1) * TILE_I + 8 * (lane >> 4) + 4 * (gs & 1));
+		const bool mine = (lane & 15) == 0;
+#pragma unroll
+		for (int r = 0; r < 4; ++r) {
+			n += (uint32_t)__popcll(__ballot(mine && sc[r] >= tau));
+			offer(mine, sc[r], item0 + (uint32_t)r);
+		}
+	}
+	return n;
+}
+
 template <int KMAX>
 __global__ __launch_bounds__(SEL_THREADS) void select_candidates_kernel(
 	const uint2 *__restrict__ cand, const uint32_t *__restrict__ seg_cnt, int nseg, int S, SweepStages stg, int capg,
 	const uint16_t *__restrict__ X, int64_t ldx, const uint16_t *__restrict__ Et, int64_t I, int KP, uint32_t k,
 	float *__restrict__ out_val, int32_t *__restrict__ out_idx, uint32_t *__restrict__ n_fallback,
 	const int32_t *__restrict__ hard_list, const uint32_t *__restrict__ hard_cnt, const float *__restrict__ tau_in, int tau_stride,
-	const int32_t *__restrict__ remap) {
+	const int32_t *__restrict__ remap, const SampleArgs sa) {
 	extern __shared__ __attribute__((aligned(16))) unsigned char smem[];
 	const SelState s = sel_carve<KMAX>(smem);
 	float *xq = reinterpret_cast<float *>(smem + SelCfg<KMAX>::LDS_BYTES);
@@ -1059,7 +1110,17 @@
 	const uint32_t total = s.scal[9], maxc = s.scal[10];
 	float tau = tau_in ? tau_in[q * tau_stride] : -INFINITY;
 	uint64_t tau_key = 0;
-	bool full = !repair && total < k;
+	uint32_t n_sample = 0;
+	if (sa.gmax) {
+		for (int g0 = 0; g0 < sa.n_groups; g0 += SEL_THREADS) {
+			const uint32_t n = sample_collect64(sa, q, g0 + wave * WAVE, tau, lane, [&](bool ok, float v, uint32_t it) { sel_offer(s, ok, v, it, tau, tau_key); });
+			if (lane == 0 && n) atomicAdd(&s.scal[11], n);
+			sel_maybe_compact<KMAX>(s, k, tau, tau_key);
+		}
+		__syncthreads();
+		n_sample = s.scal[11];
+	}
+	bool full = !repair && total + n_sample < k && tau_key == 0;
 	if (!full) {
 		for (int sb = 0; sb < nseg; sb += 4) {
 			const int sg = sb + wave;
@@ -1199,7 +1260,7 @@
 														   int capg, int64_t Q, uint32_t k, float *__restrict__ out_val,
 														   int32_t *__restrict__ out_idx, uint32_t *__restrict__ hard_cnt,
 														   int32_t *__restrict__ hard_list, float *__restrict__ tau, int tau_stride, int prefilter,
-														   const int32_t *__restrict__ remap) {
+														   const int32_t *__restrict__ remap, const SampleArgs sa) {
 	extern __shared__ __attribute__((aligned(16))) unsigned char smem[];
 	const int lane = lane_id(), wave = threadIdx.x >> 6;
 	const int64_t q = (int64_t)blockIdx.x * 4 + wave;
@@ -1207,13 +1268,27 @@
 	const uint32_t c = (lane < nseg) ? seg_cnt[q * nseg + lane] : 0u;
 	const uint32_t inc = wave_scan_incl<DppAdd>(c);
 	const uint32_t total = (uint32_t)__builtin_amdgcn_readlane((int)inc, WAVE - 1), pre = inc - c;
-	if (__ballot(c > (uint32_t)capg) != 0ull || total < k) {
+	const bool with_sample = !TAU_ONLY && sa.gmax != nullptr;
+	if (__ballot(c > (uint32_t)capg) != 0ull || (!with_sample && total < k)) {
 		if (!TAU_ONLY && lane == 0) hard_list[atomicAdd(hard_cnt, 1u)] = (int32_t)q;
 		return;
 	}
 	constexpr int CAP = WqCfg<KW>::CAP, TRIGGER = WqCfg<KW>::TRIGGER;
 	WaveSel w = wsel_init<CAP>(smem + wave * WaveSelLayout<CAP>::BYTES);
 	if (tau && prefilter) w.tau = tau[q * tau_stride];
+	if (with_sample) {
+		const float tau_f = w.tau;
+		uint32_t n_sample = 0;
+		for (int g0 = 0; g0 < sa.n_groups; g0 += WAVE)
+			n_sample += sample_collect64(sa, q, g0, tau_f, lane, [&](bool ok, float v, uint32_t it) {
+				wsel_offer(w, ok, v, it);
+				if (w.cnt > (uint32_t)TRIGGER) wsel_compact<4, false, true>(w, k);
+			});
+		if (total + n_sample < k) {
+			if (lane == 0) hard_list[atomicAdd(hard_cnt, 1u)] = (int32_t)q;
+			return;
+		}
+	}
 	const uint2 *qc = cand + q * nseg * (int64_t)capg;
 	constexpr int LOAD_U = 8;
 	for (uint32_t j0 = 0; j0 < total; j0 += LOAD_U * WAVE) {
@@ -1274,6 +1349,9 @@
 	int chunk;
 	bool ladder;
 	int ladder_k2;
+	bool sample_skip;
+	int sweep_begin;
+	size_t off_gmax2, off_gpos;
 	size_t off_lcnt, off_lvl, off_tau2;
 	size_t off_gmax, off_tval, off_tidx, off_segcnt, off_cand, off_tau, off_hard, off_ctr, off_owner, total;
 };
@@ -1328,7 +1406,7 @@
 }
 
 FusedPlan plan_fused(int64_t Q, int64_t I, int KP, int k, bool leading = false, bool mfma16 = false, bool qt1 = false, bool mfma32 = false, bool evalf = false,
-					 bool no_ladder = false) {
+					 bool no_ladder = false, bool no_sample_skip = false) {
 	FusedPlan P{};
 	P.ok = false;
 	P.leading = leading ? 1 : 0;
@@ -1392,6 +1470,9 @@
 		P.ladder_k2 = k2;
 	}
 	plan_stages(P, Q, k, exp_hits, !P.ladder && (k <= WQ_K2 ? P.lg * P.S <= WAVE : true) && P.n_tiles >= 24 * P.S, 4.0 * P.S / P.n_tiles, TILE_I);
+	P.sample_skip = P.ladder && leading && P.group == 16 && k <= WSEL_K && P.lg * P.S <= WAVE && P.n_st < P.n_tiles && P.n_stages == 1 && !no_sample_skip;
+	P.sweep_begin = P.sample_skip ? P.n_st : 0;
+	if (P.sample_skip) P.stage_tps[0] = (P.n_tiles - P.n_st + P.S - 1) / P.S;
 	P.kmax = k <= 128 ? 128 : (k <= 512 ? 512 : 2048);
 	size_t off = 256;
 	P.off_ctr = off;    off = align256(off + (size_t)P.n_rb * 3 * 4 * N_SLICES);
@@ -1406,6 +1487,8 @@
 	P.off_lvl = off;    off = align256(off + (P.ladder ? (size_t)P.n_rb * P.BQ * 4 * LADDER_LEVELS : 0));
 	P.off_tau2 = off;   off = align256(off + (P.ladder ? (size_t)Q * 4 : 0));
 	P.off_cand = off;   off = align256(off + (size_t)Q * P.lg * P.S * (size_t)P.capg * 8);
+	P.off_gmax2 = off;  off = align256(off + (P.sample_skip ? (size_t)Q * P.n_groups * 4 : 0));
+	P.off_gpos = off;   off = align256(off + (P.sample_skip ? (size_t)Q * P.n_groups : 0));
 	P.total = off;
 	P.ok = true;
 	return P;
@@ -1424,7 +1507,7 @@
 			constexpr int lds = 4 * WaveSelLayout<WqCfg<KW>::CAP>::BYTES;                                                         \
 			if ((rc = anncur_ensure_dyn_lds((const void *)select_wave_kernel<true, KW>, lds)) != ANNCUR_OK) return rc;            \
 			hipLaunchKernelGGL((select_wave_kernel<true, KW>), dim3((unsigned)ceil_div64(Q, 4)), dim3(256), lds, st, cand, seg_cnt, nseg, capg, Q, \
-							   (uint32_t)k, (float *)nullptr, (int32_t *)nullptr, (uint32_t *)nullptr, (int32_t *)nullptr, tau, tau_stride, prefilter, (const int32_t *)nullptr); \
+							   (uint32_t)k, (float *)nullptr, (int32_t *)nullptr, (uint32_t *)nullptr, (int32_t *)nullptr, tau, tau_stride, prefilter, (const int32_t *)nullptr, SampleArgs{}); \
 		} while (0)
 		if (k <= WSEL_K) LAUNCH_WTAU(128);
 		else {
@@ -1449,7 +1532,7 @@
 
 int launch_select(const FusedPlan &P, int nseg, const SweepStages &stages, const uint2 *cand, const uint32_t *seg_cnt, const uint16_t *X, int64_t ldx,
 				  const uint16_t *Et, int64_t Q, int64_t I, int KP, int k, float *out_val, int32_t *out_idx, unsigned char *ws, const float *tau,
-				  int tau_stride, hipStream_t st, const int32_t *remap = nullptr) {
+				  int tau_stride, hipStream_t st, const int32_t *remap = nullptr, const SampleArgs sa = SampleArgs{}) {
 	int rc;
 #define LAUNCH_SELECT(KM)                                                                                              \
 	do {                                                                                                               \
@@ -1457,7 +1540,7 @@
 		if ((rc = anncur_ensure_dyn_lds((const void *)select_candidates_kernel<KM>, (int)lds)) != ANNCUR_OK) return rc; \
 		hipLaunchKernelGGL((select_candidates_kernel<KM>), dim3(sel_grid), dim3(SEL_THREADS), lds, st, cand, seg_cnt, nseg, \
 						   P.S, stages, P.capg, X, ldx, Et, I, KP, (uint32_t)k, out_val, out_idx, (uint32_t *)ws, hard_list, hard_cnt,      \
-						   (P.n_stages > 1 || P.ladder) ? tau : (const float *)nullptr, tau_stride, remap);                              \
+						   (P.n_stages > 1 || P.ladder) ? tau : (const float *)nullptr, tau_stride, remap, sa);                           \
 	} while (0)
 	const int32_t *hard_list = nullptr;
 	const uint32_t *hard_cnt = nullptr;
@@ -1470,7 +1553,7 @@
 			constexpr int lds = 4 * WaveSelLayout<WqCfg<KW>::CAP>::BYTES;                                                         \
 			if ((rc = anncur_ensure_dyn_lds((const void *)select_wave_kernel<false, KW>, lds)) != ANNCUR_OK) return rc;           \
 			hipLaunchKernelGGL((select_wave_kernel<false, KW>), dim3((unsigned)ceil_div64(Q, 4)), dim3(256), lds, st, cand, seg_cnt, nseg, P.capg, Q, \
-							   (uint32_t)k, out_val, out_idx, hc, hl, const_cast<float *>(tau), tau_stride, (P.n_stages > 1 || P.ladder) ? 1 : 0, remap); \
+							   (uint32_t)k, out_val, out_idx, hc, hl, const_cast<float *>(tau), tau_stride, (P.n_stages > 1 || P.ladder) ? 1 : 0, remap, sa); \
 		} while (0)
 #define LAUNCH_SSEL(EE)                                                                                                           \
 		do {                                                                                                                      \
@@ -1497,7 +1580,8 @@
 int launch_threshold(const FusedPlan &P, const float *gmax, int64_t Q, int k, unsigned char *ws, const float *&tau, int &tau_stride, hipStream_t st) {
 	if (P.n_groups <= 4096) {
 		float *t = (float *)(ws + P.off_tau);
-		const int rc = P.ladder ? anncur_internal_kth_value(gmax, Q, P.n_groups, P.n_groups, k, t, 1, st, 1, (float *)(ws + P.off_lvl), P.ladder_k2, (float *)(ws + P.off_tau2))
+		const int rc = P.ladder ? anncur_internal_kth_value(gmax, Q, P.n_groups, P.n_groups, k, t, 1, st, 1, (float *)(ws + P.off_lvl), P.ladder_k2, (float *)(ws + P.off_tau2),
+															P.sample_skip ? (uint32_t *)(ws + P.off_lcnt) : nullptr)
 								: anncur_internal_kth_value(gmax, Q, P.n_groups, P.n_groups, k, t, 1, st, 1);
 		tau = t; tau_stride = 1;
 		return rc;
@@ -1592,6 +1676,7 @@
 	p.prio_mode = 0;
 	p.ladder_on = P.ladder ? 1 : 0; p.ladder_k = (uint32_t)k; p.ladder_mask = (uint32_t)(LADDER_PERIOD - 1);
 	p.ladder = (const float *)(ws + P.off_lvl); p.ladder_cnt = (uint32_t *)(ws + P.off_lcnt); p.tau_final = (float *)(ws + P.off_tau2);
+	p.gmax2 = P.sample_skip ? (float *)(ws + P.off_gmax2) : nullptr; p.gpos = P.sample_skip ? (uint8_t *)(ws + P.off_gpos) : nullptr;
 
 	const int chunk = (P.chunk > 0 && (Cfg::QT == 2 || P.bodyq16)) ? P.chunk : 0;
 	const int owner_stride = P.n_rb * (P.n_tiles / (chunk > 0 ? chunk : P.n_tiles) + 2);
@@ -1625,7 +1710,7 @@
 	const int tile_step = (!P.body16 && !P.bodyq16 && !P.bodyef && P.S > 1 && chunk == 0) ? P.S : 1;
 	p.n_wg = P.n_rb * P.S;
 	if ((rc = anncur_ensure_dyn_lds((const void *)score_kernel<KP, 1, 16, false, false, QTV>, Cfg::LDS_BYTES)) != ANNCUR_OK) return rc;
-	for (int stg = 0, prev = 0; stg < P.n_stages; prev = P.stage_end[stg], ++stg) {
+	for (int stg = 0, prev = P.sweep_begin; stg < P.n_stages; prev = P.stage_end[stg], ++stg) {
 		EV(5 + 2 * stg);
 		p.tile_begin = prev; p.tile_end = P.stage_end[stg]; p.tiles_per_split = P.stage_tps[stg];
 		p.flush_tiles = P.stage_flush[stg]; p.carry = stg > 0;
@@ -1684,13 +1769,15 @@
 	stages.n = P.n_stages;
 	stages.stride = tile_step;
 	stages.chunk = chunk; stages.bq = P.BQ;
-	for (int g = 0, prev = 0; g < P.n_stages; prev = P.stage_end[g], ++g) {
+	for (int g = 0, prev = P.sweep_begin; g < P.n_stages; prev = P.stage_end[g], ++g) {
 		stages.begin[g] = prev; stages.end[g] = P.stage_end[g]; stages.tps[g] = P.stage_tps[g];
 		stages.n_chunks[g] = chunk > 0 ? (P.stage_end[g] - prev + chunk - 1) / chunk : 0;
 		stages.owner[g] = (const uint8_t *)(ws + P.off_owner) + (size_t)g * owner_stride;
 	}
+	SampleArgs sa{};
+	if (P.sample_skip) sa = SampleArgs{p.gmax, p.gmax2, p.gpos, P.n_groups, p.X, ldx, p.Et, KP, (uint32_t *)(ws + 8)};
 	if ((rc = launch_select(P, P.lg * P.S, stages, p.cand, p.seg_cnt, p.X, ldx, p.Et, Q, I, KP, k, out_val, out_idx, ws, P.ladder ? p.tau_final : p.tau,
-							P.ladder ? 1 : p.tau_stride, st, item_ids)) != ANNCUR_OK) return rc;
+							P.ladder ? 1 : p.tau_stride, st, item_ids, sa)) != ANNCUR_OK) return rc;
 	EV(4);
 	return ANNCUR_OK;
 }
@@ -1830,6 +1917,10 @@
 		const FusedPlan V = plan_any(Q, I, Kp, k, flags);
 		if (V.ok && V.total > t) t = V.total;
 	}
+	for (int flags : {0, ANNCUR_TOPK_MFMA16}) {
+		const FusedPlan V = plan_any(Q, I, Kp, k, flags | ANNCUR_TOPK_LEADING_SAMPLE);
+		if (V.ok && V.total > t) t = V.total;
+	}
 	return t;
 }
 
@@ -1976,9 +2067,10 @@
 	return ANNCUR_OK;
 }
 
-static void describe_plan(const FusedPlan &P, bool wide, int32_t (&v)[27]) {
+static void describe_plan(const FusedPlan &P, bool wide, int32_t (&v)[28]) {
 	const int32_t head[8] = {P.n_st, P.n_tiles, P.S, P.capg, P.group, wide ? 4 : P.lg, P.QT, P.n_stages};
-	for (int i = 0; i < 27; ++i) v[i] = i < 8 ? head[i] : 0;
+	for (int i = 0; i < 28; ++i) v[i] = i < 8 ? head[i] : 0;
+	v[27] = (!wide && P.sample_skip) ? 1 : 0;
 	v[17] = (!wide && P.ladder) ? 1 : 0; v[18] = (!wide && P.ladder) ? P.ladder_k2 : 0; v[19] = LADDER_PERIOD;
 	v[20] = (int32_t)(P.off_gmax / 256); v[21] = P.n_groups; v[22] = (!wide && P.body16 && P.group == 16) ? 1 : 0; v[23] = P.S0;
 	for (int g = 0; g < 3; ++g) {
@@ -1993,9 +2085,9 @@
 	ANNCUR_REQUIRE(ring_flag_ok(flags), ANNCUR_E_UNSUPPORTED, "score_topk_plan_ex: ANNCUR_TOPK_RING (the tile-ring sweep body) is retired");
 	const FusedPlan P = plan_any(Q, I, Kp, k, flags);
 	ANNCUR_REQUIRE(P.ok && out && n_out >= 0, ANNCUR_E_UNSUPPORTED, "score_topk_plan_ex: unsupported shape");
-	int32_t v[27];
+	int32_t v[28];
 	describe_plan(P, wide_kp(Kp), v);
-	for (int i = 0; i < n_out && i < 24; ++i) out[i] = v[i];
+	for (int i = 0; i < n_out && i < 28; ++i) out[i] = (i < 24 || i == 27) ? v[i] : 0;
 	return ANNCUR_OK;
 }
 
@@ -2004,7 +2096,7 @@
 	const FusedPlan P = plan_fused(Q, I, Kp, k, false, false, false, false, true);
 	ANNCUR_REQUIRE(P.ok && out && n_out >= 0, ANNCUR_E_UNSUPPORTED, "eval_fused_plan: shape (Q=%lld, I=%lld, Kp=%d, k=%d) is outside the fused path",
 				   (long long)Q, (long long)I, Kp, k);
-	int32_t v[27];
+	int32_t v[28];
 	describe_plan(P, false, v);
 	for (int i = 0; i < n_out && i < 27; ++i) out[i] = v[i];
 	return ANNCUR_OK;
diff --git a/anncur_amd/csrc/topk.hip b/anncur_amd/csrc/topk.hip
--- a/anncur_amd/csrc/topk.hip
+++ b/anncur_amd/csrc/topk.hip
@@ -461,7 +461,7 @@
 
 __global__ __launch_bounds__(256) void kth_value_wave_kernel(const float *__restrict__ G, int64_t Q, int n, int64_t ldg, uint32_t k,
 															  float *__restrict__ out, int64_t out_stride, int n_pad, int coarse,
-															  float *__restrict__ ladder, uint32_t k2, float *__restrict__ tau2) {
+															  float *__restrict__ ladder, uint32_t k2, float *__restrict__ tau2, uint32_t *__restrict__ seed_cnt) {
 	extern __shared__ __attribute__((aligned(16))) unsigned char kth_smem[];
 	const uint32_t lane = (uint32_t)lane_id();
 	const int wave = threadIdx.x >> 6;
@@ -488,8 +488,36 @@
 		const float t0 = f32_unsortable(kk), g = f32_unsortable(gk);
 		float d = g - t0;
 		if (!(d > 0.f) || !(d < INFINITY)) d = 0.f;
-		if (lane < (uint32_t)LADDER_LEVELS) ladder[q * LADDER_LEVELS + lane] = t0 + d * ((float)(lane + 1) * (1.0f / LADDER_LEVELS));
+		const float lvl_lane = t0 + d * ((float)(lane + 1) * (1.0f / LADDER_LEVELS));
+		if (lane < (uint32_t)LADDER_LEVELS) ladder[q * LADDER_LEVELS + lane] = lvl_lane;
 		if (lane == 0 && tau2) tau2[q] = t0;
+		if (seed_cnt) {
+			const float *gq = G + q * ldg;
+			float lv[LADDER_LEVELS];
+#pragma unroll
+			for (int j = 0; j < LADDER_LEVELS; ++j) lv[j] = __shfl(lvl_lane, j);
+			uint32_t c[LADDER_LEVELS];
+#pragma unroll
+			for (int j = 0; j < LADDER_LEVELS; ++j) c[j] = 0u;
+			for (uint32_t j0 = 0; j0 < (uint32_t)n; j0 += WAVE) {
+				const uint32_t j = j0 + lane;
+				const float v = j < (uint32_t)n ? gq[j] : -INFINITY;
+				uint32_t r = 0;
+#pragma unroll
+				for (int i = 0; i < LADDER_LEVELS; ++i) r += (uint32_t)(v >= lv[i]);
+				if (j >= (uint32_t)n) r = 0;
+#pragma unroll
+				for (int i = 0; i < LADDER_LEVELS; ++i) c[i] += (uint32_t)__popcll(__ballot(r == (uint32_t)(i + 1)));
+			}
+#pragma unroll
+			for (int i = 0; i < LADDER_LEVELS; ++i) c[i] = c[i] < k ? c[i] : k;
+			if (lane < 4u) {
+				uint32_t wlo = 0, whi = 0;
+#pragma unroll
+				for (int i = 0; i < 4; ++i) { if (lane == (uint32_t)i) { wlo = c[2 * i]; whi = c[2 * i + 1]; } }
+				seed_cnt[q * 4 + lane] = wlo | (whi << 16);
+			}
+		}
 	}
 }
 
@@ -658,14 +686,15 @@
 }
 
 int anncur_internal_kth_value(const float *G, int64_t Q, int n, int64_t ldg, int k, float *out, int64_t out_stride, hipStream_t st, int coarse,
-							  float *ladder, int k2, float *tau2) {
+							  float *ladder, int k2, float *tau2, uint32_t *seed_cnt) {
 	ANNCUR_REQUIRE(n >= 1 && n <= KTH_MAX_N && k >= 1 && k <= n, ANNCUR_E_INVALID, "kth_value: need 1 <= k <= n <= 4096");
 	const unsigned grid = (unsigned)ceil_div64(Q, 4);
 	const int n_pad = (n + 63) & ~63;
 	const int lds = 4 * (256 + n_pad + (ladder ? 256 : 0)) * 4;
 	int rc;
 	if (lds > 64 * 1024 && (rc = anncur_ensure_dyn_lds((const void *)kth_value_wave_kernel, lds)) != ANNCUR_OK) return rc;
-	hipLaunchKernelGGL(kth_value_wave_kernel, dim3(grid), dim3(256), lds, st, G, Q, n, ldg, (uint32_t)k, out, out_stride, n_pad, coarse, ladder, (uint32_t)(k2 < 1 ? 1 : k2), tau2);
+	hipLaunchKernelGGL(kth_value_wave_kernel, dim3(grid), dim3(256), lds, st, G, Q, n, ldg, (uint32_t)k, out, out_stride, n_pad, coarse, ladder, (uint32_t)(k2 < 1 ? 1 : k2), tau2,
+					   ladder ? seed_cnt : (uint32_t *)nullptr);
 	ANNCUR_LAUNCH_OK();
 	return ANNCUR_OK;
 }
diff --git a/anncur_amd/ops.py b/anncur_amd/ops.py
--- a/anncur_amd/ops.py
+++ b/anncur_amd/ops.py
@@ -758,16 +758,26 @@
 	return {"levels": levels, "counts": counts, "tau_final": tau_final, "tau0": tau0}
 
 
+class FusedPlanInfo(dict):
+	sample_skip = False
+
+
 def fused_plan(Q, I, Kp, k, leading_sample=False, mfma16=False, qt1=False, mfma32=False, ring=False, staged=False):
-	out = (ctypes.c_int32 * 20)()
-	check(_lib.load().anncur_score_topk_plan_ex(Q, I, Kp, k, _topk_flags(leading_sample, mfma16, qt1, mfma32, ring, staged), out, 20), "score_topk_plan_ex")
+	out = (ctypes.c_int32 * 28)()
+	check(_lib.load().anncur_score_topk_plan_ex(Q, I, Kp, k, _topk_flags(leading_sample, mfma16, qt1, mfma32, ring, staged), out, 28), "score_topk_plan_ex")
 	v = [int(x) for x in out]
 	plan = dict(zip(("n_sample_tiles", "n_tiles", "splits", "segment_capacity", "group", "lg", "QT", "n_stages"), v[:8]))
 	n = plan["n_stages"]
 	plan["stage_end"], plan["stage_pred"], plan["stage_flush"] = v[8:8 + n], v[11:11 + n], v[14:14 + n]
 	plan["ladder"], plan["ladder_top_rank"] = bool(v[17]), v[18]
 	plan["ladder_period"] = v[19]
+	plan = FusedPlanInfo(plan)
+	plan.sample_skip = bool(v[27])
 	return plan
+
+
+def fused_rescored_groups(workspace):
+	return int(workspace[8:12].view(torch.int32).item())
 
 
 def eval_fused_plan(Q, I, Kp, k):
```

Measured after the change: 11.47 million queries/s. -4.4%, worse.
